# TravisWheelerLab/BATH

Hardware: AMD Instinct MI355X
Metric: DP Gcells/s + residues/s through bathsearch pipeline at 1/2/4/8 MI355X (higher is better)
Workload: dtype u8/i16 integer scores (SSV: exact binary16), f32 Forward

## Files before the change

### bath_amd/__init__.py

```python
import ctypes as C
import os
import subprocess

import numpy as np

_HERE = os.path.dirname(os.path.abspath(__file__))
_ROOT = os.path.dirname(_HERE)
LIB_PATH = os.environ.get("BATH_HIP_LIBRARY") or os.path.join(_HERE, "libbathhip.so")

OK, EINVAL, ERANGE, ENORESULT = 0, 11, 16, 19
KP, K, NEVPARAM = 29, 20, 8
LOGSUM_TABLE, LOGSUM_EXACT, LOGSUM_TABLE_SERIAL, LOGSUM_CONTEXT = 0, 1, 2, 3
LOGSUM_ODDS = 4
ENSEMBLE_SERIAL, ENSEMBLE_STREAMS_HOST, ENSEMBLE_STREAMS_DEVICE = 0, 1, 2
ENSEMBLE_MODES = {"serial": ENSEMBLE_SERIAL, "streams": ENSEMBLE_STREAMS_HOST, "device": ENSEMBLE_STREAMS_DEVICE}
ENS_SAMPLES = 200
ARITH_STRICT, ARITH_ODDS3, ARITH_ODDS = 0, 1, 2
ARITH_MODES = {"strict": ARITH_STRICT, "odds3": ARITH_ODDS3, "odds": ARITH_ODDS}
ENS_OK, ENS_IMPOSSIBLE, ENS_STEP_CAP, ENS_SEG_OVERFLOW = 0, 1, 2, 3
ENS_REGION_OK, ENS_REGION_NO_TRACES = 0, 1

DNA_SYMS = "ACGT-RYMKSWHBVDN*~"
AMINO_SYMS = "ACDEFGHIKLMNPQRSTVWY-BJZOUX*~"

# ... 28 lines not shown
class _FsProfile(C.Structure):
    _fields_ = [("M", C.c_int32), ("L", C.c_int32), ("max_length", C.c_int32), ("codon_lengths", C.c_int32),
                ("maxcodons", C.c_int32), ("nj", C.c_float), ("fsprob", C.c_float),
                ("tsc", C.POINTER(C.c_float)), ("rsc", C.POINTER(C.c_float)),
                ("codons", C.POINTER(C.c_uint8)), ("indel_pos", C.POINTER(C.c_uint8)),
                ("xsc", (C.c_float * 2) * 4), ("evparam", C.c_float * NEVPARAM), ("compo", C.c_float * K)]


class OProfileScalars(C.Structure):
    _fields_ = [("tbm_b", C.c_uint8), ("tec_b", C.c_uint8), ("tjb_b", C.c_uint8), ("base_b", C.c_uint8), ("bias_b", C.c_uint8),
                ("scale_b", C.c_float), ("xw", (C.c_int16 * 2) * 4), ("scale_w", C.c_float),
                ("base_w", C.c_int16), ("ddbound_w", C.c_int16), ("xf", (C.c_float * 2) * 4)]


class PipelineParams(C.Structure):
    _fields_ = [("F1", C.c_double), ("F2", C.c_double), ("F3", C.c_double), ("F4", C.c_double),
                ("do_biasfilter", C.c_int32), ("fs_pipe", C.c_int32), ("min_orf_len", C.c_int32), ("ncbi_table", C.c_int32),
                ("nres_before", C.c_int64),
                ("do_null2", C.c_int32), ("std_pipe", C.c_int32), ("strands", C.c_int32), ("initiator", C.c_int32),
                ("inc_by_E", C.c_int32), ("seed", C.c_int32), ("T", C.c_double)]


STRAND_BOTH, STRAND_TOPONLY, STRAND_BOTTOMONLY = 0, 1, 2
INIT_ANY, INIT_TABLE, INIT_AUG = 0, 1, 2


class OrfResult(C.Structure):
    _fields_ = [("window", C.c_int64), ("strand", C.c_int32), ("frame", C.c_int32), ("start", C.c_int32), ("end", C.c_int32),
                ("n", C.c_int32), ("stage", C.c_int32), ("msv_status", C.c_int32), ("vit_status", C.c_int32),
                ("usc", C.c_float), ("nullsc", C.c_float), ("filtersc", C.c_float), ("vfsc", C.c_float), ("fwdsc", C.c_float),
                ("P", C.c_double)]


ORF_RESULT_DTYPE = np.dtype([("window", "<i8"), ("strand", "<i4"), ("frame", "<i4"), ("start", "<i4"), ("end", "<i4"),
                             ("n", "<i4"), ("stage", "<i4"), ("msv_status", "<i4"), ("vit_status", "<i4"),
                             ("usc", "<f4"), ("nullsc", "<f4"), ("filtersc", "<f4"), ("vfsc", "<f4"), ("fwdsc", "<f4"),
                             ("P", "<f8")], align=True)


class PipelineStats(C.Structure):
    _fields_ = [(n, C.c_int64) for n in ("nres", "n_orfs", "n_past_msv", "n_past_bias", "n_past_vit", "n_past_fwd",
                                          "pos_past_msv", "pos_past_bias", "pos_past_vit", "pos_past_fwd",
                                          "cells_msv", "cells_vit", "cells_fwd")]


class Orf(C.Structure):
    _fields_ = [("window", C.c_int64), ("strand", C.c_int32), ("frame", C.c_int32), ("start", C.c_int32), ("end", C.c_int32),
                ("n", C.c_int32), ("aa_off", C.c_int64)]


class FsWindow(C.Structure):
    _fields_ = [("window", C.c_int64), ("strand", C.c_int32), ("n", C.c_int32), ("length", C.c_int32),
                ("orf_cnt", C.c_int32), ("k_min", C.c_int32), ("k_max", C.c_int32),
                ("tot_orfsc", C.c_float), ("nullsc", C.c_float), ("filtersc", C.c_float), ("fwdsc", C.c_float),
                ("P_tot", C.c_double), ("P_min", C.c_double), ("P_fs", C.c_double), ("P_null", C.c_double),
                ("branch", C.c_int32)]


class FsDomain(C.Structure):
    _fields_ = [("window", C.c_int64), ("strand", C.c_int32), ("fs_window", C.c_int32),
                ("ienv", C.c_int32), ("jenv", C.c_int32), ("iali", C.c_int32), ("jali", C.c_int32), ("ihmm", C.c_int32), ("jhmm", C.c_int32),
                ("envsc", C.c_float), ("oasc", C.c_float), ("domcorrection", C.c_float), ("dombias", C.c_float),
                ("bitscore", C.c_float), ("pre_score", C.c_float), ("lnP", C.c_double), ("reported", C.c_int32), ("n_shifted_codons", C.c_int32),
                ("n_stops", C.c_int32), ("pid", C.c_float), ("ali_columns", C.c_int32), ("cigar_off", C.c_int64)]
    cigar = ""


_DTYPES = {}


class DomainTrace(C.Structure):
    _fields_ = [("off", C.c_int64), ("N", C.c_int32), ("win_start", C.c_int32), ("orf_start", C.c_int32), ("frameshift", C.c_int32)]


class AliDisplayOpts(C.Structure):
    _fields_ = [("hmm_name", C.c_char_p), ("seq_name", C.c_char_p), ("consensus", C.c_char_p), ("rf", C.c_char_p), ("cs", C.c_char_p),
                ("M", C.c_int32), ("sqfrom", C.c_int64), ("sqto", C.c_int64), ("textw", C.c_int32), ("show_frameline", C.c_int32),
                ("initiator", C.c_int32)]


class FsRow(C.Structure):
    _fields_ = [("type", C.c_char), ("length", C.c_int32), ("ali_start", C.c_int32), ("seq_start", C.c_int64)]


class DistItem(C.Structure):
    _fields_ = [("query", C.c_int32), ("lo", C.c_int64), ("hi", C.c_int64)]


T_M, T_D, T_I = 1, 2, 3


def _np_dtype(T):
    d = _DTYPES.get(T)
    if d is None:
        d = _DTYPES[T] = np.dtype(T)
    return d


FS_DOMAIN_DTYPE = _np_dtype(FsDomain)


class KernelTime(C.Structure):
    _fields_ = [("name", C.c_char_p), ("ms", C.c_float), ("launches", C.c_int64), ("cells", C.c_double), ("bytes", C.c_double)]


class HmmWindow(C.Structure):
    _fields_ = [("target", C.c_int64), ("n", C.c_int32), ("k", C.c_int32), ("length", C.c_int32), ("score", C.c_float)]


class StdResult(C.Structure):
    _fields_ = [("fwdsc", C.c_float), ("bcksc", C.c_float), ("oasc", C.c_float), ("fwd_status", C.c_int32), ("bck_status", C.c_int32),
                ("ok", C.c_int32), ("null2", C.c_float * KP)]


class Fs5Result(C.Structure):
    _fields_ = [("fwdsc", C.c_float), ("bcksc", C.c_float), ("oasc", C.c_float), ("null2", C.c_float * KP)]


_CALIB_SCORE_FN = C.CFUNCTYPE(C.c_int, C.c_void_p, C.POINTER(C.c_uint8), C.c_int, C.c_int, C.POINTER(C.c_float))

_vp, _u8p, _f32p, _i32p, _i64p = C.c_void_p, C.POINTER(C.c_uint8), C.POINTER(C.c_float), C.POINTER(C.c_int32), C.POINTER(C.c_int64)
ABI = {
    "bath_hmmfile_count": (C.c_int, [C.c_char_p]),
    "bath_hmmfile_read": (C.c_int, [C.c_char_p, C.c_int, C.POINTER(C.POINTER(_Hmm))]),
    "bath_hmm_destroy": (None, [C.POINTER(_Hmm)]),
    "bath_gencode_basic": (C.c_int, [C.c_int, _u8p]),
    "bath_profile_config": (C.c_int, [C.POINTER(_Hmm), C.c_int, C.POINTER(C.POINTER(_Profile))]),
    "bath_profile_destroy": (None, [C.POINTER(_Profile)]),
    "bath_fs_profile_config": (C.c_int, [C.POINTER(_Hmm), _u8p, C.c_int, C.c_int, C.POINTER(C.POINTER(_FsProfile))]),
    "bath_fs_profile_destroy": (None, [C.POINTER(_FsProfile)]),
    "bath_hip_init": (C.c_int, [C.c_int, C.POINTER(_vp)]),
    "bath_hip_finalize": (None, [_vp]),
    "bath_hip_last_error": (C.c_char_p, [_vp]),
    "bath_hip_synchronize": (C.c_int, [_vp]),
    "bath_hip_stream": (_vp, [_vp]),
    "bath_hip_set_fs_strict": (C.c_int, [_vp, C.c_int]),
    "bath_hip_set_fs_serial": (C.c_int, [_vp, C.c_int]),
    "bath_hip_set_fs_odds": (C.c_int, [_vp, C.c_int]),
    "bath_hip_set_fs5_odds": (C.c_int, [_vp, C.c_int]),
    "bath_hip_set_fs_ensemble": (C.c_int, [_vp, C.c_int]),
    "bath_hip_fs_ensemble_counters": (C.c_int, [_vp, _i64p, _i64p, _i64p]),
    "bath_hip_set_std_ensemble": (C.c_int, [_vp, C.c_int]),
    "bath_hip_std_ensemble_counters": (C.c_int, [_vp, _i64p, _i64p, _i64p]),
    "bath_hip_std_region_ensembles": (C.c_int, [_vp, _vp, _vp, _i32p, C.c_uint32, _i32p, _i32p, _i32p, C.c_int64, _i64p, _i32p, _f32p, C.c_int64, _i64p]),
    "bath_selftest_std_ensemble": (C.c_int, [C.c_int, C.c_int, _f32p, _f32p, C.c_float, C.c_float, C.c_float, _u8p, C.c_int, _f32p, _f32p, C.c_uint32, _i32p, _i32p,
                                             _i32p, C.c_int, _i32p, _f32p, _i32p, C.c_int, _i32p]),
    "bath_selftest_std_ens_walk": (C.c_int, [C.c_int, _f32p, C.c_float, C.c_float, C.c_float, C.c_int, _f32p, _f32p, C.c_uint32, _i32p, _i32p, C.c_int, _i32p]),
    "bath_hip_fs5_region_ensembles": (C.c_int, [_vp, _vp, _vp, C.c_uint32, _i32p, _i32p, _i32p, C.c_int64, _i64p, _i32p, C.c_int64, _i64p]),
    "bath_selftest_fs_ensemble_seeded": (C.c_int, [C.c_int, _f32p, C.c_float, C.c_float, C.c_float, C.c_int, C.c_int, _f32p, _f32p, C.c_uint32, _i32p, C.c_int, _i32p]),
    "bath_selftest_fs_ensemble_streams": (C.c_int, [C.c_int, _f32p, C.c_float, C.c_float, C.c_float, C.c_int, C.c_int, _f32p, _f32p, C.c_uint32,
                                                    _i32p, _i32p, _i32p, C.c_int, _i32p, _i32p, C.c_int, _i32p]),
    "bath_selftest_rng_jump": (C.c_int, [C.c_uint32, C.c_uint64, C.POINTER(C.c_uint32)]),
    "bath_selftest_ens_explog": (C.c_int, [C.c_int, _f32p, _f32p, _f32p]),
    "bath_hip_trim": (C.c_int, [_vp]),
    "bath_hip_kernel_times": (C.c_int, [_vp, C.c_int, C.POINTER(KernelTime)]),
    "bath_hip_oprofile_convert": (C.c_int, [_vp, C.POINTER(_Profile), C.POINTER(_vp)]),
    "bath_hip_oprofile_destroy": (None, [_vp]),
    "bath_hip_oprofile_M": (C.c_int, [_vp]),
    "bath_hip_oprofile_scalars": (C.c_int, [_vp, C.c_int, C.POINTER(OProfileScalars)]),
    "bath_hip_oprofile_get_ssv_scores": (C.c_int, [_vp, _u8p]),
    "bath_hip_oprofile_get_vit": (C.c_int, [_vp, C.POINTER(C.c_int16), C.POINTER(C.c_int16)]),
    "bath_hip_oprofile_get_fwd": (C.c_int, [_vp, _f32p, _f32p]),
    "bath_hip_seqs_create": (C.c_int, [_vp, _u8p, _i64p, C.c_int64, C.POINTER(_vp)]),
    "bath_hip_seqs_destroy": (None, [_vp]),
    "bath_hip_seqs_count": (C.c_int64, [_vp]),
    "bath_hip_seqs_read": (C.c_int64, [_vp, _u8p, C.c_int64, _i64p, _i32p, _i32p]),
    "bath_hip_seqs_set_context": (C.c_int, [_vp, C.POINTER(C.c_int32)]),
    "bath_hip_host_alloc": (C.c_void_p, [C.c_size_t]),
    "bath_hip_host_free": (None, [C.c_void_p]),
    "bath_hip_seqs_create_packed": (C.c_int, [_vp, _i64p, C.c_int64, C.POINTER(_vp)]),
    "bath_hip_seqs_upload_packed": (C.c_int, [_vp, C.c_void_p, _i64p, _i32p, _u8p, C.c_int64]),
    "bath_hip_seqs_upload_wait": (C.c_int, [_vp]),
    "bath_hip_fasta_create": (C.c_int, [_vp, C.POINTER(_vp)]),
    "bath_hip_fasta_destroy": (None, [_vp]),
    "bath_hip_fasta_feed": (C.c_int, [_vp, C.c_void_p, C.c_int64]),
    "bath_hip_fasta_finish": (C.c_int, [_vp]),
    "bath_hip_fasta_count": (C.c_int64, [_vp]),
    "bath_hip_fasta_symbols": (C.c_int64, [_vp]),
    "bath_hip_fasta_records": (C.c_int, [_vp, C.c_int64, C.c_int64, C.c_void_p]),
    "bath_hip_fasta_error": (C.c_int, [_vp, _i64p, _i64p, _i64p, _i32p]),
    "bath_hip_fasta_windows": (C.c_int64, [_vp, C.c_int64, C.c_int64, C.c_int32, C.c_int32, C.c_void_p, C.c_int64]),
    "bath_hip_fasta_seqs": (C.c_int, [_vp, C.c_void_p, C.c_int64, C.POINTER(_vp)]),
    "bath_hip_fasta_seqs_for": (C.c_int, [_vp, _vp, C.c_void_p, C.c_int64, C.POINTER(_vp)]),
    "bath_hip_fasta_codes": (C.c_int, [_vp, C.c_int64, C.c_int64, C.c_int64, _u8p]),
    "bath_hip_fasta_release": (C.c_int, [_vp, C.c_int64]),
    "bath_hip_ssvfilter": (C.c_int, [_vp, _vp, _vp, _f32p, _i32p]),
    "bath_hip_msvfilter": (C.c_int, [_vp, _vp, _vp, _f32p, _i32p]),
    "bath_hip_vitfilter": (C.c_int, [_vp, _vp, _vp, _f32p, _i32p]),
    "bath_hip_forward_parser": (C.c_int, [_vp, _vp, _vp, _f32p, _i32p]),
    "bath_hip_bias_filter": (C.c_int, [_vp, _vp, _vp, _f32p, _f32p]),
    "bath_hip_fwdback_parser": (C.c_int, [_vp, _vp, _vp, _i64p, _f32p, _f32p, _i32p, _i32p, _f32p, _f32p]),
    "bath_hip_translate_orfs": (C.c_int, [_vp, _vp, C.c_int, C.c_int, C.POINTER(C.POINTER(Orf)), _i64p, C.POINTER(_u8p)]),
    "bath_hip_translate_orfs_opts": (C.c_int, [_vp, _vp, C.c_int, C.c_int, C.c_int, C.c_int, C.POINTER(C.POINTER(Orf)), _i64p, C.POINTER(_u8p)]),
    "bath_hip_orf_worklist": (C.c_int, [_vp, C.c_void_p, _i64p]),
    "bath_gencode_initiators": (C.c_int, [C.c_int, C.c_int, _u8p]),
    "bath_tophits_set_score_thresholds": (None, [_vp, C.c_int, C.c_double, C.c_int, C.c_double]),
    "bath_search_space_residues": (C.c_int64, [C.c_int, C.c_double, C.c_int, C.c_int64]),
    "bath_pipeline_params_default": (None, [C.POINTER(PipelineParams), C.c_int]),
    "bath_hip_pipeline_filters": (C.c_int, [_vp, _vp, _vp, C.POINTER(PipelineParams), C.POINTER(PipelineStats),
                                            C.POINTER(C.POINTER(OrfResult)), _i64p]),
    "bath_hip_pipeline_frameshift": (C.c_int, [_vp, _vp, _vp, _vp, C.POINTER(PipelineParams), C.POINTER(PipelineStats),
                                              C.POINTER(C.POINTER(OrfResult)), _i64p, C.POINTER(C.POINTER(FsWindow)), _i64p]),
    "bath_hip_oprofile_set_consensus": (C.c_int, [_vp, C.c_char_p]),
    "bath_hip_domain_cigars": (C.c_void_p, [_vp]),
    "bath_hip_domain_traces": (C.c_int, [_vp, C.POINTER(C.POINTER(DomainTrace)), _i64p, C.POINTER(C.POINTER(C.c_int8)), C.POINTER(_i32p),
                                         C.POINTER(_i32p), C.POINTER(C.POINTER(C.c_int8)), C.POINTER(_f32p)]),
    "bath_alidisplay_print": (C.c_int64, [C.POINTER(DomainTrace), C.POINTER(C.c_int8), _i32p, _i32p, C.POINTER(C.c_int8), _f32p,
                                          _u8p, C.c_int32, C.POINTER(_FsProfile), C.POINTER(_Profile), _u8p, C.POINTER(AliDisplayOpts),
                                          C.c_char_p, C.c_int64]),
    "bath_selftest_rng_stream": (C.c_int, [C.c_uint32, C.c_int, C.POINTER(C.c_double)]),
    "bath_selftest_fchoose": (C.c_int, [C.c_uint32, _f32p, C.c_int, C.c_int, _i32p]),
    "bath_hits_serialize": (C.c_int64, [C.c_void_p, C.c_int64, C.c_char_p, C.POINTER(DomainTrace), C.POINTER(C.c_int8), _i32p, _i32p, C.POINTER(C.c_int8), _f32p,
                                        C.c_void_p, C.c_int64]),
    "bath_hits_deserialize": (C.c_int, [C.c_void_p, C.c_int64, C.POINTER(_vp)]),
    "bath_hits_stream_size": (C.c_int64, [C.c_void_p, C.c_int64]),
    "bath_hits_destroy": (None, [_vp]),
    "bath_hits_count": (C.c_int64, [_vp]),
    "bath_hits_domains": (C.POINTER(FsDomain), [_vp]),
    "bath_hits_cigars": (C.c_void_p, [_vp, _i64p]),
    "bath_hits_traces": (C.c_int, [_vp, C.POINTER(C.POINTER(DomainTrace)), C.POINTER(C.POINTER(C.c_int8)), C.POINTER(_i32p), C.POINTER(_i32p),
                                   C.POINTER(C.POINTER(C.c_int8)), C.POINTER(_f32p)]),
    "bath_tophits_add_serialized": (C.c_int, [_vp, C.c_void_p, C.c_int64, C.c_int64, C.c_int64, C.c_int64, C.POINTER(C.c_char_p), C.POINTER(C.c_char_p),
                                              C.POINTER(C.c_char_p), C.POINTER(C.c_int64)]),
    "bath_dist_shard_range": (None, [C.c_int64, C.c_int, C.c_int, _i64p, _i64p]),
    "bath_dist_items": (C.c_int64, [_i64p, C.POINTER(C.c_double), C.c_int, C.c_int, C.c_int, C.POINTER(DistItem), C.c_int64]),
    "bath_dist_deal": (C.c_int, [C.POINTER(C.c_double), C.c_int64, C.c_int, _i32p]),
    "bath_selftest_cluster_segments": (C.c_int, [C.c_int, _i32p, _i32p, _i32p, _i32p, _i32p, C.c_int, C.c_int, _i32p, C.c_int, _i32p]),
    "bath_selftest_fs_ensemble": (C.c_int, [C.c_int, _f32p, C.c_float, C.c_float, C.c_float, C.c_int, C.c_int, _f32p, _f32p, _i32p, C.c_int, _i32p]),
    "bath_tophits_create": (_vp, []),
    "bath_tophits_destroy": (None, [_vp]),
    "bath_tophits_add": (C.c_int, [_vp, C.POINTER(FsDomain), C.c_int64, C.c_void_p, C.c_int64, C.POINTER(C.c_char_p), C.POINTER(C.c_char_p),
                                   C.POINTER(C.c_char_p), C.POINTER(C.c_int64)]),
    "bath_tophits_finalize": (C.c_int, [_vp, C.c_int64, C.c_int, C.c_double]),
    "bath_tophits_count": (C.c_int64, [_vp]),
    "bath_tophits_reported": (C.c_int64, [_vp]),
    "bath_tophits_get": (C.c_int, [_vp, C.c_int64, C.POINTER(FsDomain), C.POINTER(C.c_int64), C.POINTER(C.c_int32)]),
    "bath_tophits_targets": (C.c_int64, [_vp, C.c_int, C.c_int, C.c_char_p, C.c_int64]),
    "bath_tophits_domain_annotation": (C.c_int64, [_vp, C.c_int64, C.c_int, C.c_int, C.c_char_p, C.c_int64]),
    "bath_tophits_pipeline_statistics": (C.c_int64, [_vp, C.POINTER(PipelineStats), C.POINTER(PipelineParams), C.c_int64, C.c_int64, C.c_int64, C.c_char_p, C.c_int64]),
    "bath_tophits_set_inclusion": (None, [_vp, C.c_double]),
    "bath_tophits_tabular_targets": (C.c_int64, [_vp, C.c_char_p, C.c_char_p, C.c_int, C.c_int, C.c_int, C.c_int, C.c_char_p, C.c_int64]),
    "bath_trace_frameshift_rows": (C.c_int64, [C.POINTER(DomainTrace), C.POINTER(C.c_int8), _i32p, _i32p, C.POINTER(C.c_int8), _u8p, C.c_int32,
                                               C.POINTER(_FsProfile), C.c_int64, C.c_int64, C.POINTER(FsRow), C.c_int64]),
    "bath_tophits_tabular_frameshifts": (C.c_int64, [_vp, C.c_char_p, C.c_char_p, C.POINTER(FsRow), _i64p, C.c_int64, C.c_int, C.c_char_p, C.c_int64]),
    "bath_hip_pipeline_hits": (C.c_int, [_vp, _vp, _vp, C.POINTER(PipelineParams), C.c_double, C.POINTER(PipelineStats),
                                         C.POINTER(C.POINTER(FsDomain)), C.POINTER(C.c_int64), C.POINTER(C.c_int64)]),
    "bath_hip_pipeline_frameshift_domains": (C.c_int, [_vp, _vp, _vp, _vp, _vp, C.POINTER(PipelineParams), C.c_double, C.POINTER(PipelineStats),
                                                      C.POINTER(C.POINTER(FsWindow)), _i64p, C.POINTER(C.POINTER(FsDomain)), _i64p, _i64p]),
    "bath_hip_pipeline_timings": (C.c_int, [_vp, C.c_int, C.POINTER(C.c_char_p), _f32p, _i64p]),
    "bath_hip_fsprofile_convert": (C.c_int, [_vp, C.POINTER(_FsProfile), C.POINTER(_vp)]),
    "bath_hip_fsprofile_destroy": (None, [_vp]),
    "bath_hip_fs3_forward_parser": (C.c_int, [_vp, _vp, _vp, C.c_int, _f32p, _f32p, _i64p]),
    "bath_hip_fs3_backward_parser": (C.c_int, [_vp, _vp, _vp, C.c_int, _f32p, _f32p, _i64p]),
    "bath_hip_vitfilter_bath": (C.c_int, [_vp, _vp, _vp, _f32p, C.c_double, _f32p, _i32p, C.POINTER(C.POINTER(HmmWindow)), _i64p]),
    "bath_hip_ssvfilter_bath": (C.c_int, [_vp, _vp, _vp, C.c_double, C.POINTER(C.POINTER(HmmWindow)), _i64p]),
    "bath_hip_forward_full": (C.c_int, [_vp, _vp, _vp, _i32p, C.c_int, _f32p, _i32p, _f32p, _f32p]),
    "bath_hip_std_envelopes": (C.c_int, [_vp, _vp, _vp, C.POINTER(StdResult), _f32p, _f32p, _f32p, _f32p]),
    "bath_hip_std_envelopes_fill": (C.c_int, [_vp, _vp, _vp, C.POINTER(StdResult), _f32p, _f32p, _f32p, _f32p, C.c_int]),
    "bath_hip_fs5_envelopes_x": (C.c_int, [_vp, _vp, _vp, C.c_int, C.c_int, C.POINTER(Fs5Result), _f32p, _f32p, _f32p, _f32p]),
    "bath_hip_fs5_forward_full": (C.c_int, [_vp, _vp, _vp, C.c_int, _f32p, _f32p, _f32p]),
    "bath_hip_fs5_envelopes": (C.c_int, [_vp, _vp, _vp, C.c_int, C.c_int, C.POINTER(Fs5Result), _f32p, _i64p, _f32p, _i64p]),
    "bath_hip_fs5_forward_parser": (C.c_int, [_vp, _vp, _vp, C.c_int, _f32p]),
    "bath_hip_fs5_forward_parser_odds": (C.c_int, [_vp, _vp, _vp, C.c_int, _f32p]),
    "bath_calib_fit_scores": (C.c_int, [C.POINTER(C.c_uint32), _f32p, C.c_int, C.c_int, C.c_int, _CALIB_SCORE_FN, C.c_void_p, C.c_float,
                                        C.POINTER(C.c_double), C.POINTER(C.c_int)]),
    "bath_hip_calibrate_fs_arith": (C.c_int, [_vp, C.POINTER(_Hmm), C.c_int, C.POINTER(C.c_uint32), C.c_int, C.c_int, C.c_double,
                                              C.POINTER(C.c_double), C.POINTER(C.c_double), C.POINTER(C.c_double), C.POINTER(C.c_double),
                                              C.c_int, C.POINTER(C.c_int)]),
    "bath_calib_sample": (C.c_int, [C.POINTER(C.c_uint32), _f32p, C.c_int, C.c_int, C.c_int, _u8p]),
    "bath_gumbel_fit_complete": (C.c_int, [C.POINTER(C.c_double), C.c_int, C.POINTER(C.c_double), C.POINTER(C.c_double)]),
    "bath_gumbel_invcdf": (C.c_double, [C.c_double, C.c_double, C.c_double]),
    "bath_calib_tau": (C.c_int, [C.POINTER(C.c_double), C.c_int, C.c_double, C.c_double, C.POINTER(C.c_double)]),
    "bath_bg_fs_nullone": (C.c_float, [C.c_int]),
    "bath_hmm_max_length": (C.c_int, [C.POINTER(_Hmm), C.c_double]),
    "bath_hip_calibrate_fs": (C.c_int, [_vp, C.POINTER(_Hmm), C.c_int, C.POINTER(C.c_uint32), C.c_int, C.c_int, C.c_double,
                                        C.POINTER(C.c_double), C.POINTER(C.c_double), C.POINTER(C.c_double), C.POINTER(C.c_double)]),
    "bath_scorematrix_builtin": (C.c_char_p, [C.c_char_p]),
    "bath_scoresystem_create": (C.c_int, [C.c_char_p, C.c_char_p, C.c_double, C.c_double, C.POINTER(_vp), C.c_char_p, C.c_int]),
    "bath_scoresystem_destroy": (None, [_vp]),
    "bath_scoresystem_lambda": (C.c_double, [_vp]),
    "bath_scoresystem_conditionals": (C.c_int, [_vp, C.POINTER(C.c_double)]),
    "bath_hmm_from_sequence": (C.c_int, [_vp, _u8p, C.c_int, C.c_char_p, C.c_int, C.POINTER(C.POINTER(_Hmm))]),
    "bath_hmm_mean_match_relent": (C.c_double, [C.POINTER(_Hmm)]),
    "bath_hmm_lambda": (C.c_double, [C.POINTER(_Hmm)]),
    "bath_hmm_write_ascii": (C.c_int64, [C.POINTER(_Hmm), C.c_int, C.c_double, C.c_char_p, C.c_char_p, C.c_char_p, C.c_char_p, C.c_int64]),
    "bath_calib_sample_amino": (C.c_int, [C.POINTER(C.c_uint32), _f32p, C.c_int, C.c_int, _u8p]),
    "bath_gumbel_fit_complete_loc": (C.c_int, [C.POINTER(C.c_double), C.c_int, C.c_double, C.POINTER(C.c_double)]),
    "bath_hip_calib_samples_create": (C.c_int, [_vp, C.POINTER(C.c_uint32), C.c_int, C.c_int, C.c_int, C.c_int, C.c_int, C.c_int, C.POINTER(_vp)]),
    "bath_hip_calib_samples_destroy": (None, [_vp]),
    "bath_hip_calibrate": (C.c_int, [_vp, C.POINTER(_Hmm), C.c_int, C.POINTER(C.c_uint32), _vp, C.c_int, C.c_int, C.c_int, C.c_int, C.c_int, C.c_int,
                                     C.c_double, C.c_int, C.POINTER(C.c_double), C.POINTER(C.c_int)]),
}

_lib = None


def lib():
    global _lib
    if _lib is None:
        if not os.path.exists(LIB_PATH):
            raise BathError("libbathhip.so not built: run `python -c 'import __graft_entry__ as g; g.build()'` "
                            "(or `make -C bath_amd/csrc`). There is no CPU fallback.")
        L = C.CDLL(LIB_PATH)
        for name, (res, args) in ABI.items():
            fn = getattr(L, name)
            fn.restype, fn.argtypes = res, args
# ... 1359 lines not shown
```

### bath_amd/csrc/bath_common.hpp

```cpp
#pragma once
#include <set>
#include <atomic>
#include <hip/hip_runtime.h>

#include <cstdint>
#include <chrono>
#include <cstdio>
#include <cstdlib>
#include <cstring>
#include <condition_variable>
#include <functional>
#include <mutex>
#include <string>
#include <thread>
#include <vector>

#include "bath_hip.h"
#include "bath_tilings.hpp"

namespace bath {

inline hipError_t allow_max_lds(const void *fn) {
  static std::mutex mu;
  static std::set<std::pair<int, const void *>> done;
// ... 151 lines not shown
    if (hipMemcpyAsync(dst, stage[slot].p, n * sizeof(T), hipMemcpyHostToDevice, s) != hipSuccess) { set_error("staging upload failed"); return BATH_EFAIL; }
    return BATH_OK;
  }
  bath::HostBuf pinned[4];
  bath::HostBuf results_pinned;
  bath_orf_result *d_records = nullptr;
  int64_t n_records = 0;
  std::vector<bath_orf> orfs;
  std::vector<bath_fs_window> fs_windows;
  bool keep_fwd_rows = false;
  const float *fwd_rows_kept = nullptr;
  const int64_t *fwd_rows_off = nullptr;
  bool fs_want_regions = false;
  std::vector<int64_t> fs_keep_xoff;
  std::vector<int32_t> fs_regions_all;
  std::vector<bath_fs_domain> fs_domains;
  std::string cigars;
  struct TraceRec { int64_t col_off; int32_t ncol, k1, i_first, win_start, orf_start, frameshift, d_i; };
  std::vector<TraceRec> tr_recs;
  std::vector<uint16_t> tr_codes;
  std::vector<float> tr_pp;
  void traces_clear() { tr_recs.clear(); tr_codes.clear(); tr_pp.clear(); tr_valid = false; }
  void trace_push(const uint16_t *codes, const float *pp, int ncol, int k1, int i_first, int win_start, int orf_start, int frameshift, int d_i) {
    tr_recs.push_back(TraceRec{(int64_t)tr_codes.size(), ncol, k1, i_first, win_start, orf_start, frameshift, d_i});
    tr_codes.insert(tr_codes.end(), codes, codes + ncol);
    if (pp) tr_pp.insert(tr_pp.end(), pp, pp + ncol); else tr_pp.insert(tr_pp.end(), (size_t)ncol, 0.0f);
    tr_valid = false;
  }
  bool tr_valid = false;
  std::vector<bath_domain_trace> tr_out;
  std::vector<int8_t> tr_st, tr_c;
  std::vector<int32_t> tr_k, tr_i;
  std::vector<bath::PipelineSurvivor> fs_std_orfs;
  const uint8_t *fs_std_pool = nullptr;
  std::vector<uint8_t> orf_aa;
  std::vector<bath_orf_work> orf_work;
  std::vector<bath_hmm_window> hmm_windows;
  std::vector<bath::StageTiming> timings;
  std::vector<hipEvent_t> ev_pool;
  std::vector<bath::KernelSpan> spans;
  std::vector<hipEvent_t> span_events;
  size_t span_events_used = 0;
  void spans_reset() { spans.clear(); span_events_used = 0; }
  int span_begin(const char *name, hipStream_t s, double cells, double bytes) {
    auto get = [&]() -> hipEvent_t {
      if (span_events_used == span_events.size()) { hipEvent_t e; if (hipEventCreate(&e) != hipSuccess) return nullptr; span_events.push_back(e); }
      return span_events[span_events_used++];
    };
    bath::KernelSpan k{name, get(), get(), cells, bytes};
    if (!k.a || !k.b) return -1;
    (void)hipEventRecord(k.a, s);
    spans.push_back(k);
    return (int)spans.size() - 1;
  }
  void span_end(int idx, hipStream_t s) { if (idx >= 0) (void)hipEventRecord(spans[(size_t)idx].b, s); }
  std::vector<bath_hip_ctx *> lanes;
  bath::LanePool *lane_pool = nullptr;
  hipEvent_t ev_lanes = nullptr;
  bath_hip_ctx *aux = nullptr;
  bath_hip_ctx *aux2 = nullptr;
  bath_hip_ctx *aux3 = nullptr;
  bool internal = false;
};

namespace bath {
inline void mark_internal(bath_hip_ctx *c) { if (c && !c->internal) { c->internal = true; g_ctx_internal.fetch_add(1); } }
}

struct SeqView {
  const uint8_t *data;
  const int64_t *off;
  const int32_t *len;
  int64_t n;
  const int32_t *context;
};

struct bath_hip_seqs {
  bath_hip_ctx *ctx = nullptr;
  int64_t n = 0;
  int64_t total = 0;
  int64_t total_aligned = 0;
  mutable int64_t cache_minlen = -1, cache_nres = 0, cache_max_orfs = 0;
  mutable int64_t ntiles = -1;
  mutable void *d_tile_desc = nullptr;
  mutable int32_t *d_tile_first = nullptr;
  bool is_part = false;
  int64_t first_window = 0;
  mutable std::vector<bath_hip_seqs *> parts;
  int32_t maxlen = 0;
  uint8_t *d_data = nullptr;
  int64_t *d_off = nullptr;
  int32_t *d_len = nullptr;
  int32_t *d_context = nullptr;
  uint8_t *d_packed = nullptr;
  int64_t *d_poff = nullptr;
  int64_t packed_bytes = 0;
  void *d_exc = nullptr;
  int64_t exc_cap = 0, n_exc = 0;
  hipEvent_t ev_upload = nullptr;
  bool upload_pending = false;
  std::vector<int64_t> h_off;
  std::vector<int32_t> h_len;
  std::vector<int32_t> h_context;
  SeqView view() const { return SeqView{d_data, d_off, d_len, n, d_context}; }
};

struct LenTables {
  int32_t maxL = -1;
  uint8_t *d_tjb = nullptr;
  int16_t *d_xwmove = nullptr;
  float   *d_pmove = nullptr;
  float   *d_nullsc = nullptr;
  float   *d_lt1 = nullptr;
  float   *d_lt2 = nullptr;
  float   *d_p1 = nullptr;
  std::vector<uint8_t> h_tjb;
  std::vector<int16_t> h_xwmove;
  std::vector<float> h_pmove, h_nullsc;
};

struct bath_hip_oprofile {
  bath_hip_ctx *ctx = nullptr;
  uint64_t uid = 0;
  int M = 0, max_length = 0, L0 = 0;
  float nj = 1.f;
  float evparam[BATH_NEVPARAM];
  float compo[BATH_K_AMINO];
  std::vector<uint8_t> rb;
  std::vector<int16_t> rw;
  std::vector<int16_t> tw;
  std::vector<float> rf, tf;
  uint8_t tbm_b = 0, tec_b = 0, base_b = 0, bias_b = 0;
  float scale_b = 0;
  int16_t xw_E[2] = {0, 0};
  float scale_w = 0;
  int16_t base_w = 0, ddbound_w = 0;
  float xf_E[2] = {0, 0};
  std::string consensus;
  std::vector<uint8_t> cons_digital;
  uint8_t *d_cons = nullptr;
  std::vector<float> prefix_lengths, suffix_lengths;
  int NR = 0, G = 1;
  int ssv_row_bytes = 0;
  int16_t *d_ssv = nullptr;
  int16_t *d_msv = nullptr;
  uint8_t *d_rb = nullptr;
  int rb_stride = 0;
  int16_t *d_rw = nullptr;
  int16_t *d_tw = nullptr;
  float *d_rf = nullptr, *d_tf = nullptr;
  float *d_rfb = nullptr, *d_tfb = nullptr;
  float *d_msc = nullptr, *d_tsc = nullptr;
  float *d_bias_eo = nullptr;
  int vit_NR = 0, vit_rw_pitch = 0;
  int16_t *d_vit_rw = nullptr; uint32_t *d_vit_tw2 = nullptr; int16_t *d_vit_rank = nullptr;
  mutable LenTables lt;
  mutable std::mutex grow_mu;
  mutable std::vector<void *> retired;
  mutable int16_t *d_emit = nullptr;
  mutable double emit_F1 = -1.0;
  mutable int emit_maxlen = -1;
  int ensure_len_tables(int maxL) const;
};

namespace bath {
int build_len_tables(const bath_hip_oprofile *om, int maxL);
void bias_filter_eo(const float *compo, float eo[kKp][2]);
double gumbel_surv(double x, double mu, double lambda);
double gumbel_invsurv(double p, double mu, double lambda);
double exp_surv(double x, double mu, double lambda);
struct StageClock {
  bool on; std::chrono::steady_clock::time_point t;
  StageClock() { const char *e = std::getenv("BATH_HIP_TIMING"); on = e && e[0] == '1'; t = std::chrono::steady_clock::now(); }
  void lap(const char *what) {
    if (!on) return;
    const auto n = std::chrono::steady_clock::now();
    std::fprintf(stderr, "[bath timing] %-34s %8.2f ms\n", what, std::chrono::duration<double, std::milli>(n - t).count());
    t = n;
  }
};

}
```

### bath_amd/csrc/bath_pipeline.hip

```cpp
#include <algorithm>
#include <cmath>
#include <cstring>
#include <cstdlib>
#include <map>
#include <thread>

#include "bath_common.hpp"
#include "bath_kernels.hpp"
#include "bath_launch.hpp"
#include "host_model.hpp"

using namespace bath;

namespace bath {

static const double kLog2 = 0.69314718055994529;

enum { FLAG_VIT_RUN = 1, FLAG_HAS_WIN = 2 };

struct Counters {
  int cand_count, todo_msv, todo_vit, todo_ssvb, todo_vit2, todo_fwd, win_count, overflow;
  int todo_lb, pad_;
  unsigned long long n_orfs, orf_res;
  unsigned long long n_past_msv, n_past_bias, n_past_vit, n_past_fwd;
  unsigned long long pos_past_msv, pos_past_bias, pos_past_vit, pos_past_fwd;
  unsigned long long res_vit, res_fwd;
  unsigned long long res_seen;
};

struct Params {
  double F1, F2, F3, F4;
  int do_bias, fs_pipe, minlen;
  float evparam[BATH_NEVPARAM];
};

template <int NR, int G>
__global__ __launch_bounds__(256, NR <= 76 ? 4 : 1) void ssv_orf_kernel(const uint8_t *__restrict__ aa, const OrfRec *__restrict__ orfs, const int *__restrict__ n_orfs_dev,
                                                      SeqView dna, const int16_t *__restrict__ cost_tab, int row_bytes,
                                                      const int16_t *__restrict__ emit_thresh, int thresh_max,
                                                      Cand cand, int cand_cap, Counters *__restrict__ ctr, int chunk) {
  extern __shared__ __attribute__((aligned(16))) char lds[];
  if (chunk > 0 && (int64_t)blockIdx.x * (blockDim.x >> 6) * chunk * (64 / G) >= (int64_t)*n_orfs_dev) return;
  {
    const int n32 = kSsvRows * row_bytes / 4;
    const uint32_t *src = reinterpret_cast<const uint32_t *>(cost_tab);
    uint32_t *dst = reinterpret_cast<uint32_t *>(lds);
    for (int i = threadIdx.x; i < n32; i += blockDim.x) dst[i] = src[i];
  }
  __syncthreads();
  constexpr int TPW = 64 / G;
  const int64_t n_orfs = *n_orfs_dev;
  const int lane = threadIdx.x & 63;
  const int grank = SsvGroups<G>::rank(lane);
  const char *tile = lds + grank * (4 * NR);
  const unsigned tile_addr = (unsigned)(size_t)(__attribute__((address_space(3))) const char *)tile;
  const int64_t wave0 = ((int64_t)blockIdx.x * blockDim.x + threadIdx.x) >> 6;
  const int64_t nwaves = ((int64_t)gridDim.x * blockDim.x) >> 6;
  const s16x2 fl = {0, 0};
  const int64_t tb_first = chunk > 0 ? wave0 * chunk * TPW : wave0 * TPW, tb_step = chunk > 0 ? TPW : nwaves * TPW;
  const int64_t tb_end = chunk > 0 ? (tb_first + (int64_t)chunk * TPW < n_orfs ? tb_first + (int64_t)chunk * TPW : n_orfs) : n_orfs;
  for (int64_t tb = tb_first; tb < tb_end; tb += tb_step) {
    const int64_t t = tb + SsvGroups<G>::slot(lane);
    const bool live = t < n_orfs;
    OrfRec rec{0, 0, 0};
    if (live) rec = orfs[t];
    const int L = rec.len_sf & 0x0fffffff;
#ifdef BATH_SSV_POOL_PROBE
    const uint8_t *s = aa + ((size_t)(tb / TPW) * 8192) % ((size_t)1 << 27) + (size_t)lane * 8;
#define BATH_SSV_RES(i8) (s + (size_t)(i8) * 64)
#else
    const uint8_t *s = aa + rec.aa_off;
#define BATH_SSV_RES(i8) (s + (i8))
#endif
    const int Lw = wave_max_i32(L);
    s16x2 reg[NR];
#pragma unroll
    for (int r = 0; r < NR; r++) reg[r] = fl;
    s16x2 xE = fl, xE2 = fl;
    uint64_t qnext = (0 < L) ? *reinterpret_cast<const uint64_t *>(BATH_SSV_RES(0)) : 0x1d1d1d1d1d1d1d1dull;
    for (int i0 = 0; i0 < Lw; i0 += 8) {
      const uint64_t q = qnext;
      qnext = (i0 + 8 < L) ? *reinterpret_cast<const uint64_t *>(BATH_SSV_RES(i0 + 8)) : 0x1d1d1d1d1d1d1d1dull;
      const int nrow = min(8, Lw - i0);
      for (int h = 0; h < 2; h++) {
        const uint32_t qh = h ? (uint32_t)(q >> 32) : (uint32_t)q;
        const int nh = min(4, nrow - 4 * h);
        for (int j = 0; j < nh; j++) {
          int x = (int)__builtin_amdgcn_ubfe(qh, 8 * j, 8);
          x = (i0 + 4 * h + j < L) ? x : kRowReset;
          const unsigned carry = ssv_carry<NR, G>(reg, grank);
          ssv_row_pipe<NR, 3>(reg, xE, xE2, tile_addr + __umul24((unsigned)x, (unsigned)row_bytes), carry);
        }
      }
    }
    xE = ssv_max3(xE, xE2, xE2);
    const int v = ssv_group_max<G>(xE);
    if (dna.context) {
      unsigned long long r = 0;
      if (live && grank == 0) {
        const int sf = (int)((unsigned)rec.len_sf >> 28);
        const int64_t w = rec.w;
        const int startj = (int32_t)(rec.aa_off - (2 * dna.off[w] + 96 * w + (int64_t)sf * orf_stream_pitch(dna.len[w])));
        const int C = dna.context[w], start_s = sf % 3 + 3 * startj + 1;
        if (sf < 3 ? (start_s + 3 * L - 1 < C) : (dna.len[w] - start_s + 1 < C)) r = (unsigned long long)L;
      }
      if (__ballot(r != 0)) { for (int d = 32; d >= 1; d >>= 1) r += __shfl_xor(r, d, 64); if (lane == 0) atomicAdd(&ctr->res_seen, r); }
    }
    if (live && grank == 0 && v >= (int)emit_thresh[min(L, thresh_max)]) {
      const int sf = (int)((unsigned)rec.len_sf >> 28);
      const int64_t w = rec.w;
      const int64_t stream = 2 * dna.off[w] + 96 * w + (int64_t)sf * orf_stream_pitch(dna.len[w]);
      const int startj = (int32_t)(rec.aa_off - stream);
      bool seen = false;
      if (dna.context) {
        const int C = dna.context[w], start_s = sf % 3 + 3 * startj + 1;
        seen = sf < 3 ? (start_s + 3 * L - 1 < C) : (dna.len[w] - start_s + 1 < C);
      }
      const int slot = seen ? cand_cap + 1 : atomicAdd(&ctr->cand_count, 1);
      if (seen) {
      } else if (slot < cand_cap) {
        cand.window[slot] = w; cand.sf[slot] = sf; cand.startj[slot] = startj; cand.len[slot] = L;
        cand.v[slot] = (int16_t)min(v, 32767); cand.off[slot] = rec.aa_off;
      } else atomicOr(&ctr->overflow, 1);
    }
  }
}

__device__ __forceinline__ double d_gumbel_surv(double x, double mu, double lambda) {
  const double ey = -exp(-lambda * (x - mu));
  if (fabs(ey) < 5e-9) return -ey;
  return 1.0 - exp(ey);
}
__device__ __forceinline__ double d_exp_surv(double x, double mu, double lambda) { return (x < mu) ? 1.0 : exp(-lambda * (x - mu)); }

__device__ __forceinline__ int cand_classify(const Cand &cand, int c, int tjb, const MsvConsts &mc) {
  float sc = 0.f;
  const int st = ssv_classify(cand.v[c], tjb, mc, &sc);
  cand.usc[c] = sc; cand.msv_status[c] = st; cand.stage[c] = 0; cand.flags[c] = 0;
  cand.vfsc[c] = -INFINITY; cand.fwdsc[c] = -INFINITY; cand.vit_status[c] = 0; cand.filtersc[c] = 0.f; cand.P[c] = 1.0;
  cand.kminmax[2 * c] = 1 << 30; cand.kminmax[2 * c + 1] = 0;
  return st;
}

__global__ void classify_kernel(Cand cand, int cand_cap, Counters *__restrict__ ctr, const uint8_t *__restrict__ tjb_tab, MsvConsts mc,
                                int32_t *__restrict__ todo_msv) {
  const int ncand = min(ctr->cand_count, cand_cap);
  for (int c = blockIdx.x * blockDim.x + threadIdx.x; c < ncand; c += gridDim.x * blockDim.x) {
    if (cand_classify(cand, c, tjb_tab[cand.len[c]], mc) == BATH_ENORESULT) todo_msv[atomicAdd(&ctr->todo_msv, 1)] = c;
  }
}

struct F1Tables { const float *eo, *nullsc, *p1, *lt1, *lt2; };
__device__ __forceinline__ void cand_f1_bias(const Cand &cand, int c, Counters *__restrict__ ctr, const Params &p, const uint8_t *__restrict__ pool, int M,
                                             const float *s_eo , const F1Tables &t,
                                             int32_t *__restrict__ todo_vit, int32_t *__restrict__ todo_ssvb) {
  const int L = cand.len[c];
  const float usc = cand.usc[c];
  const float nullsc = t.nullsc[L];
  cand.nullsc[c] = nullsc;
  float seqsc = (float)((double)(usc - nullsc) / kLog2);
  double P = d_gumbel_surv(seqsc, p.evparam[0], p.evparam[1]);
  cand.P[c] = P;
  if (P > p.F1) return;
  atomicAdd(&ctr->n_past_msv, 1ull); atomicAdd(&ctr->pos_past_msv, (unsigned long long)L * 3ull);
  cand.stage[c] = 1;
  float filtersc = nullsc;
  if (p.do_bias) {
    filtersc = bias_forward(pool + cand.off[c], L, M, s_eo, t.p1[L]);
    filtersc = (filtersc + t.lt1[L]) + t.lt2[L];
    seqsc = (float)((double)(usc - filtersc) / kLog2);
    P = d_gumbel_surv(seqsc, p.evparam[0], p.evparam[1]);
    cand.P[c] = P; cand.filtersc[c] = filtersc;
    if (P > p.F1) return;
  }
  cand.filtersc[c] = filtersc;
  atomicAdd(&ctr->n_past_bias, 1ull); atomicAdd(&ctr->pos_past_bias, (unsigned long long)L * 3ull);
  cand.stage[c] = 2;
  if (P > p.F2) { cand.flags[c] |= FLAG_VIT_RUN; todo_vit[atomicAdd(&ctr->todo_vit, 1)] = c; atomicAdd(&ctr->res_vit, (unsigned long long)L); }
  else todo_ssvb[atomicAdd(&ctr->todo_ssvb, 1)] = c;
}

__global__ void f1_bias_kernel(Cand cand, int cand_cap, Counters *__restrict__ ctr, Params p, const uint8_t *__restrict__ pool, int M, F1Tables t,
                               int32_t *__restrict__ todo_vit, int32_t *__restrict__ todo_ssvb) {
  __shared__ float s_eo[kKp * 2];
  for (int i = threadIdx.x; i < kKp * 2; i += blockDim.x) s_eo[i] = t.eo[i];
  __syncthreads();
  const int ncand = min(ctr->cand_count, cand_cap);
  for (int c = blockIdx.x * blockDim.x + threadIdx.x; c < ncand; c += gridDim.x * blockDim.x) cand_f1_bias(cand, c, ctr, p, pool, M, s_eo, t, todo_vit, todo_ssvb);
}

template <int NR>
__global__ __launch_bounds__(256, 4) void msv_stage_kernel(Cand cand, int cand_cap, Counters *__restrict__ ctr,
                                                           const int16_t *__restrict__ cost_tab , int row_bytes,
                                                           const uint8_t *__restrict__ tjb_tab, MsvConsts mc, Params p, const uint8_t *__restrict__ pool, int M,
                                                           F1Tables t, int32_t *__restrict__ todo_vit, int32_t *__restrict__ todo_ssvb) {
  extern __shared__ __attribute__((aligned(16))) char lds[];
  __shared__ float s_eo[kKp * 2];
  const int ncand = min(ctr->cand_count, cand_cap);
  if ((int64_t)blockIdx.x * blockDim.x >= ncand) return;
  {
    const int n32 = kSsvRows * row_bytes / 4;
    const uint32_t *src = reinterpret_cast<const uint32_t *>(cost_tab);
    uint32_t *dst = reinterpret_cast<uint32_t *>(lds);
    for (int i = threadIdx.x; i < n32; i += blockDim.x) dst[i] = src[i];
    for (int i = threadIdx.x; i < kKp * 2; i += blockDim.x) s_eo[i] = t.eo[i];
  }
  __syncthreads();
  const int64_t job = (int64_t)blockIdx.x * blockDim.x + threadIdx.x;
  const bool live = job < ncand;
  const int c = live ? (int)job : 0;
  const int L = live ? cand.len[c] : 0;
  const int tjb = tjb_tab[L];
  const bool rescore = live && cand_classify(cand, c, tjb, mc) == BATH_ENORESULT;
  const int Lr = rescore ? L : 0;
  const uint8_t *s = pool + (rescore ? cand.off[c] : 0);
  bool overflow = false;
  const int xJ = msv_lane_rows<NR>(lds, row_bytes, s, Lr, wave_max_i32(Lr), (uint8_t)((int8_t)tjb + (int8_t)mc.tbm), mc, &overflow);
  if (rescore) {
    if (overflow) { cand.usc[c] = INFINITY; cand.msv_status[c] = BATH_ERANGE; }
    else { cand.usc[c] = msv_lane_score(xJ, tjb, mc); cand.msv_status[c] = BATH_OK; }
  }
  if (live) cand_f1_bias(cand, c, ctr, p, pool, M, s_eo, t, todo_vit, todo_ssvb);
}

template <int C>
__global__ __launch_bounds__(256) void ssv_bath_kernel(Cand cand, const Counters *__restrict__ ctr, const int32_t *__restrict__ todo,
                                                       const uint8_t *__restrict__ pool, int M, const uint8_t *__restrict__ rb, int rb_stride,
                                                       const uint8_t *__restrict__ ssv_scores, const uint8_t *__restrict__ tjb_tab,
                                                       const float *__restrict__ nullsc_tab, MsvConsts mc, double invP_f1,
                                                       WindowRec *__restrict__ wins, int win_cap, Counters *__restrict__ ctrw) {
  const int lane = threadIdx.x & 63;
  const int64_t wid = ((int64_t)blockIdx.x * blockDim.x + threadIdx.x) >> 6;
  const int64_t nw = ((int64_t)gridDim.x * blockDim.x) >> 6;
  const int ntodo = ctr->todo_ssvb;
  const int Q = max(2, ((M - 1) / 16) + 1);
  for (int64_t job = wid; job < ntodo; job += nw) {
    const int c = todo[job];
    const int L = cand.len[c];
    const uint8_t *s = pool + cand.off[c];
    const int tjb = tjb_tab[L];
    const float nullsc = nullsc_tab[L];
    const int sc_thresh = (uint8_t)(int)ceil((((double)nullsc + ((double)(float)invP_f1 * kLog2) + 3.0) * (double)mc.scale_b) + mc.base + mc.tec + tjb);
    const int tjbm = (uint8_t)((int8_t)tjb + (int8_t)mc.tbm);
    const int xB = satu8(mc.base - tjbm);
    int kmin = 1 << 30, kmax = 0;
    int dp[C];
#pragma unroll
    for (int k = 0; k < C; k++) dp[k] = 0;
    const int ph = threadIdx.x & 63;
    int rbuf = (ph < L) ? (int)s[ph] : 0, rnext = 0;
    for (int i = 1; i <= L; i++) {
      const int j = (i - 1) & 63;
      if (j == 0) { const int q = i - 1 + 64 + ph; rnext = (q < L) ? (int)s[q] : 0; }
      const int x = min(__builtin_amdgcn_readlane(rbuf, j), kKp - 1);
      if (j == 63) rbuf = rnext;
      const uint8_t *row = rb + (size_t)x * rb_stride;
      int prev = wave_shr1_i32(dp[C - 1], 0);
      int xE = 0;
#pragma unroll
      for (int k = 0; k < C; k++) {
        const int node = lane * C + k + 1;
        const int cost = (node <= M) ? (int)row[node] : 255;
        int sv = max(prev, xB);
        sv = satu8(sv + mc.bias);
        sv = satu8(sv - cost);
        prev = dp[k];
        dp[k] = sv;
        xE = max(xE, sv);
      }
      xE = wave_max_i32(xE);
      if (xE >= sc_thresh) {
        int rank = 1 << 30;
#pragma unroll
        for (int k = 0; k < C; k++) {
          const int node = lane * C + k + 1;
          if (node <= M && dp[k] == xE) rank = min(rank, ((node - 1) % Q) * 16 + (node - 1) / Q);
        }
        rank = wave_min_i32(rank);
        int end = (rank / 16) + Q * (rank % 16) + 1;
        int rem_sc = xE;
#pragma unroll
        for (int k = 0; k < C; k++) dp[k] = 0;
        int start = end, target_end = i, target_start = i;
        int sc = rem_sc;
        while (rem_sc > mc.base - tjb - mc.tbm && start >= 1 && target_start >= 1) {
          rem_sc -= mc.bias - (int)ssv_scores[(size_t)start * kKp + min((int)s[target_start - 1], kKp - 1)];
          --start; --target_start;
        }
        start++; target_start++;
        int k = end + 1, n = target_end + 1, max_end = target_end, max_sc = sc, since = 0;
        while (k < M && n <= L) {
          sc += mc.bias - (int)ssv_scores[(size_t)k * kKp + min((int)s[n - 1], kKp - 1)];
          if (sc >= max_sc) { max_sc = sc; max_end = n; since = 0; }
          else { since++; if (since == 5) break; }
          k++; n++;
        }
        end += (max_end - target_end);
        target_end = max_end;
        float ret = ((float)(max_sc - tjb) - (float)mc.base);
        ret /= mc.scale_b;
        ret = (float)((double)ret - 3.0);
        if (lane == 0) {
          const int slot = atomicAdd(&ctrw->win_count, 1);
          if (slot < win_cap) wins[slot] = WindowRec{c, target_start, end, end - start + 1, ret};
        }
        kmin = min(kmin, start); kmax = max(kmax, end);
        i = target_end;
        { const int base = i & ~63; rbuf = (base + ph < L) ? (int)s[base + ph] : 0; rnext = (base + 64 + ph < L) ? (int)s[base + 64 + ph] : 0; }
      }
    }
    if (lane == 0) { cand.kminmax[2 * c] = kmin; cand.kminmax[2 * c + 1] = kmax; }
  }
}

__device__ __forceinline__ float local_compo_x(const uint8_t *ssv_scores, int M, int base_b, float scale_b, const float *bgf, int k_start, int k_end, int x) {
  const int k_len = k_end - k_start + 1;
  if (k_len < 20) { k_start -= (20 - k_len) / 2; k_end += (20 - k_len) / 2; }
  k_start = max(1, k_start); k_end = min(M, k_end);
  float acc = 0.0f;
  for (int k = k_start; k <= k_end; k++) {
    const float lo = ((float)base_b - (float)ssv_scores[(size_t)k * kKp + x]) / scale_b;
    acc += bgf[x] * expf(lo);
  }
  return acc;
}
__device__ void local_compo_finish(float *compo , const float *bgf, float *eo );
__device__ void local_compo_eo(const uint8_t *ssv_scores, int M, int base_b, float scale_b, const float *bgf, int k_start, int k_end, float *eo ) {
  float compo[20];
  for (int x = 0; x < 20; x++) compo[x] = local_compo_x(ssv_scores, M, base_b, scale_b, bgf, k_start, k_end, x);
  local_compo_finish(compo, bgf, eo);
}
__device__ void local_compo_finish(float *compo, const float *bgf, float *eo) {
  float sum = 0.f, cc = 0.f;
  for (int x = 0; x < 20; x++) { const float y = compo[x] - cc; const float t = sum + y; cc = (t - sum) - y; sum = t; }
  if (sum != 0.0f) for (int x = 0; x < 20; x++) compo[x] /= sum;
  else for (int x = 0; x < 20; x++) compo[x] = 1.0f / 20.0f;
  for (int x = 0; x < 20; x++) { eo[2 * x] = bgf[x] / bgf[x]; eo[2 * x + 1] = compo[x] / bgf[x]; }
  eo[2 * 20] = eo[2 * 20 + 1] = 1.0f; eo[2 * 27] = eo[2 * 27 + 1] = 1.0f; eo[2 * 28] = eo[2 * 28 + 1] = 1.0f;
  const int mem[6][2] = {{2, 11}, {7, 9}, {3, 13}, {8, 8}, {1, 1}, {-1, -1}};
  for (int dx = 0; dx < 6; dx++) {
    float n0 = 0.f, n1 = 0.f, den = 0.f;
    if (dx == 5) { for (int y = 0; y < 20; y++) { n0 += bgf[y]; n1 += compo[y]; den += bgf[y]; } }
    else {
      const int a = min(mem[dx][0], mem[dx][1]), b = max(mem[dx][0], mem[dx][1]);
      n0 += bgf[a]; n1 += compo[a]; den += bgf[a];
      if (b != a) { n0 += bgf[b]; n1 += compo[b]; den += bgf[b]; }
    }
    eo[2 * (21 + dx)] = den > 0.f ? n0 / den : 0.f;
    eo[2 * (21 + dx) + 1] = den > 0.f ? n1 / den : 0.f;
  }
}

__global__ void post_vit_kernel(Cand cand, int cand_cap, Counters *__restrict__ ctr, Params p, int32_t *__restrict__ todo_lb, int32_t *__restrict__ todo_fwd) {
  const int ncand = min(ctr->cand_count, cand_cap);
  for (int c = blockIdx.x * blockDim.x + threadIdx.x; c < ncand; c += gridDim.x * blockDim.x) {
    if (cand.stage[c] != 2) continue;
    const int L = cand.len[c];
    if (cand.flags[c] & FLAG_VIT_RUN) {
      const float seqsc = (float)((double)(cand.vfsc[c] - cand.filtersc[c]) / kLog2);
      const double P = d_gumbel_surv(seqsc, p.evparam[2], p.evparam[3]);
      cand.P[c] = P;
      if (P > p.F2) { cand.kminmax[2 * c] = 1 << 30; cand.kminmax[2 * c + 1] = 0; continue; }
    }
    atomicAdd(&ctr->n_past_vit, 1ull); atomicAdd(&ctr->pos_past_vit, (unsigned long long)L * 3ull);
    if (p.do_bias && cand.kminmax[2 * c] <= cand.kminmax[2 * c + 1]) {
      cand.flags[c] |= FLAG_HAS_WIN;
      todo_lb[atomicAdd(&ctr->todo_lb, 1)] = c;
      continue;
    }
    cand.stage[c] = 3;
    todo_fwd[atomicAdd(&ctr->todo_fwd, 1)] = c; atomicAdd(&ctr->res_fwd, (unsigned long long)L);
  }
}

__global__ void compo_terms_kernel(const float *__restrict__ bgf, int base_b, float scale_b, float *__restrict__ terms ) {
  const int x = blockIdx.x, sc = threadIdx.x;
  const float lo = ((float)base_b - (float)sc) / scale_b;
  terms[x * 256 + sc] = bgf[x] * expf(lo);
}

__global__ __launch_bounds__(64) void local_compo_kernel(Cand cand, const Counters *__restrict__ ctr, int M, const uint8_t *__restrict__ ssv_scores,
                                                         const float *__restrict__ terms, const int32_t *__restrict__ todo_lb, float *__restrict__ compo_out ) {
  const int lane = threadIdx.x, g = lane / 20, x = lane % 20;
  const int ntodo = ctr->todo_lb;
  for (int base = blockIdx.x * 3; base < ntodo; base += gridDim.x * 3) {
    const int job = base + g;
    if (g >= 3 || job >= ntodo) continue;
    const int c = todo_lb[job];
    int k_start = cand.kminmax[2 * c], k_end = cand.kminmax[2 * c + 1];
    const int k_len = k_end - k_start + 1;
    if (k_len < 20) { k_start -= (20 - k_len) / 2; k_end += (20 - k_len) / 2; }
    k_start = max(1, k_start); k_end = min(M, k_end);
    const float *tx = terms + x * 256;
    float acc = 0.0f;
    for (int k = k_start; k <= k_end; k++) acc += tx[ssv_scores[(size_t)k * kKp + x]];
    compo_out[(size_t)job * 20 + x] = acc;
  }
}

__global__ __launch_bounds__(64) void post_vit_local_kernel(Cand cand, Counters *__restrict__ ctr, Params p, const uint8_t *__restrict__ pool, int M,
                                                            const float *__restrict__ bgf, const float *__restrict__ compo_in,
                                                            const float *__restrict__ p1_tab, const float *__restrict__ lt1_tab, const float *__restrict__ lt2_tab,
                                                            const int32_t *__restrict__ todo_lb, int32_t *__restrict__ todo_vit2, int32_t *__restrict__ todo_fwd) {
  __shared__ float s_eo[64][kKp * 2 + 1];
  const int ntodo = ctr->todo_lb;
  for (int job = blockIdx.x * blockDim.x + threadIdx.x; job < ntodo; job += gridDim.x * blockDim.x) {
    const int c = todo_lb[job];
    const int L = cand.len[c];
    const float usc = cand.usc[c];
    float filtersc = cand.filtersc[c];
    const float vfsc = (cand.flags[c] & FLAG_VIT_RUN) ? cand.vfsc[c] : -INFINITY;
    float compo[20];
    for (int y = 0; y < 20; y++) compo[y] = compo_in[(size_t)job * 20 + y];
    float *eo = s_eo[threadIdx.x];
    local_compo_finish(compo, bgf, eo);
    float lf = bias_forward(pool + cand.off[c], L, M, eo, p1_tab[L]);
    lf = (lf + lt1_tab[L]) + lt2_tab[L];
    bool to_fwd = true;
    if (lf > filtersc) {
      filtersc = lf;
      cand.filtersc[c] = filtersc;
      if (vfsc == -INFINITY) {
        const float seqsc = (float)((double)(usc - filtersc) / kLog2);
        const double P = d_gumbel_surv(seqsc, p.evparam[0], p.evparam[1]);
        cand.P[c] = P;
        if (P > p.F2) { cand.stage[c] = 5; todo_vit2[atomicAdd(&ctr->todo_vit2, 1)] = c; atomicAdd(&ctr->res_vit, (unsigned long long)L); to_fwd = false; }
      } else {
        const float seqsc = (float)((double)(vfsc - filtersc) / kLog2);
        const double P = d_gumbel_surv(seqsc, p.evparam[2], p.evparam[3]);
        cand.P[c] = P;
        if (P > p.F2) to_fwd = false;
      }
    }
    if (to_fwd) { cand.stage[c] = 3; todo_fwd[atomicAdd(&ctr->todo_fwd, 1)] = c; atomicAdd(&ctr->res_fwd, (unsigned long long)L); }
  }
}

__global__ void post_vit2_kernel(Cand cand, Counters *__restrict__ ctr, Params p, const int32_t *__restrict__ todo_vit2, int32_t *__restrict__ todo_fwd) {
  const int ntodo = ctr->todo_vit2;
  for (int job = blockIdx.x * blockDim.x + threadIdx.x; job < ntodo; job += gridDim.x * blockDim.x) {
    const int c = todo_vit2[job];
    const float seqsc = (float)((double)(cand.vfsc[c] - cand.filtersc[c]) / kLog2);
    const double P = d_gumbel_surv(seqsc, p.evparam[2], p.evparam[3]);
    cand.P[c] = P;
    if (P > p.F2) { cand.stage[c] = 2; continue; }
    cand.stage[c] = 3;
    todo_fwd[atomicAdd(&ctr->todo_fwd, 1)] = c; atomicAdd(&ctr->res_fwd, (unsigned long long)cand.len[c]);
  }
}

__global__ void final_kernel(Cand cand, Counters *__restrict__ ctr, Params p, const int32_t *__restrict__ todo_fwd) {
  const int ntodo = ctr->todo_fwd;
  for (int job = blockIdx.x * blockDim.x + threadIdx.x; job < ntodo; job += gridDim.x * blockDim.x) {
    const int c = todo_fwd[job];
    const float seqsc = (float)((double)(cand.fwdsc[c] - cand.filtersc[c]) / kLog2);
    const double P = d_exp_surv(seqsc, p.evparam[4], p.evparam[5]);
    cand.P[c] = P;
    if (P > (p.fs_pipe ? p.F4 : p.F3)) continue;
    cand.stage[c] = 4;
    atomicAdd(&ctr->n_past_fwd, 1ull);
    if (!p.fs_pipe) atomicAdd(&ctr->pos_past_fwd, (unsigned long long)cand.len[c] * 3ull);
  }
}

__global__ void copy_count_kernel(const int *src, int64_t *dst) { *dst = *src; }

}


namespace bath {

static int ssv_classify_host(int v, int tjb, const MsvConsts &c, float *sc) {
  if (tjb + c.tbm + c.tec + c.bias >= 127) return BATH_ENORESULT;
  unsigned xE = (v >= -1 - c.bias) ? 255u : (unsigned)(v + 256);
  if ((int)xE >= 255 - c.bias) { *sc = INFINITY; return (c.base - tjb - c.tbm < 128) ? BATH_ENORESULT : BATH_ERANGE; }
  xE = (xE + (unsigned)(c.base - tjb - c.tbm) - 128u) & 0xffffu;
  if ((int)xE >= 255 - c.bias) { *sc = INFINITY; return BATH_ERANGE; }
  unsigned xJ = (xE - (unsigned)c.tec) & 0xffffu;
  if ((int)xJ > c.base) return BATH_ENORESULT;
  float r = ((float)((int)xJ - tjb) - (float)c.base);
  r /= c.scale_b;
  r = (float)((double)r - 3.0);
  *sc = r;
  return BATH_OK;
}

static void build_emit_table(const bath_hip_oprofile *om, double F1, int maxlen, std::vector<int16_t> &tab) {
  const MsvConsts mc = msv_consts(om);
  tab.assign((size_t)maxlen + 1, (int16_t)32767);
  for (int len = 0; len <= maxlen; len++) {
    const int tjb = om->lt.h_tjb[len];
    const float nullsc = om->lt.h_nullsc[len];
    auto keep = [&](int v) {
      float usc = 0.f;
      if (ssv_classify_host(v, tjb, mc, &usc) != BATH_OK) return true;
      const float seqsc = (float)((double)(usc - nullsc) / kLog2);
      return !(gumbel_surv(seqsc, om->evparam[0], om->evparam[1]) > F1);
    };
    if (!keep(127)) continue;
    int lo = -128, hi = 127;
    while (lo < hi) { const int mid = lo + (hi - lo) / 2; if (keep(mid)) hi = mid; else lo = mid + 1; }
    tab[(size_t)len] = (int16_t)lo;
  }
}

static int ensure_emit_table(bath_hip_ctx *ctx, const bath_hip_oprofile *om, double F1, int maxlen) {
  std::lock_guard<std::mutex> lock(om->grow_mu);
  if (om->emit_F1 == F1 && om->emit_maxlen >= maxlen && om->d_emit) return BATH_OK;
  std::vector<int16_t> tab;
  build_emit_table(om, F1, maxlen, tab);
  if (om->d_emit) om->retired.push_back(om->d_emit);
  om->d_emit = nullptr;
  BATH_HIP_TRY(ctx, hipMalloc((void **)&om->d_emit, tab.size() * sizeof(int16_t) + 64));
  BATH_HIP_TRY(ctx, hipMemcpy(om->d_emit, tab.data(), tab.size() * sizeof(int16_t), hipMemcpyHostToDevice));
  om->emit_F1 = F1; om->emit_maxlen = maxlen;
  return BATH_OK;
}

static int wave_grid_blocks(bath_hip_ctx *ctx) { return ctx->prop.multiProcessorCount * 8; }

struct PipelineWork {
  Cand cand;
  int cand_cap = 0;
  uint8_t *pool = nullptr;
  int32_t *todo_msv = nullptr, *todo_vit = nullptr, *todo_ssvb = nullptr, *todo_vit2 = nullptr, *todo_fwd = nullptr, *todo_sorted = nullptr;
  int *len_bins = nullptr;
  WindowRec *wins = nullptr;
  int win_cap = 0;
  Counters *ctr = nullptr;
};

template <class T>
static T *carve(char *&p, size_t n) {
  T *r = reinterpret_cast<T *>(p);
  p += (n * sizeof(T) + 255) / 256 * 256;
  return r;
}

static size_t layout(PipelineWork &w, char *base, int cap, int win_cap) {
  char *p = base;
  const size_t n = (size_t)cap;
  w.cand_cap = cap; w.win_cap = std::max(2 * cap, win_cap);
  if (win_cap == 0) {
    static const int forced = [] { const char *e = std::getenv("BATH_HIP_TEST_WINCAP"); return e ? std::atoi(e) : 0; }();
    if (forced > 0) w.win_cap = forced;
  }
  w.ctr = carve<Counters>(p, 1);
  w.cand.window = carve<int64_t>(p, n); w.cand.off = carve<int64_t>(p, n); w.cand.P = carve<double>(p, n);
  w.cand.sf = carve<int32_t>(p, n); w.cand.startj = carve<int32_t>(p, n); w.cand.len = carve<int32_t>(p, n);
  w.cand.msv_status = carve<int32_t>(p, n); w.cand.vit_status = carve<int32_t>(p, n); w.cand.fwd_status = carve<int32_t>(p, n); w.cand.stage = carve<int32_t>(p, n);
  w.cand.flags = carve<int32_t>(p, n); w.cand.kminmax = carve<int32_t>(p, 2 * n);
  w.cand.usc = carve<float>(p, n); w.cand.nullsc = carve<float>(p, n); w.cand.filtersc = carve<float>(p, n);
  w.cand.vfsc = carve<float>(p, n); w.cand.fwdsc = carve<float>(p, n);
  w.cand.v = carve<int16_t>(p, n);
  w.todo_msv = carve<int32_t>(p, n); w.todo_vit = carve<int32_t>(p, n); w.todo_ssvb = carve<int32_t>(p, n);
  w.todo_vit2 = carve<int32_t>(p, n); w.todo_fwd = carve<int32_t>(p, n); w.todo_sorted = carve<int32_t>(p, n);
  w.len_bins = carve<int>(p, 2048);
  w.wins = carve<WindowRec>(p, (size_t)w.win_cap);
  return (size_t)(p - base);
}

}

extern "C" void bath_pipeline_params_default(bath_pipeline_params *p, int fs_pipe) {
  p->F1 = 0.02; p->F2 = 1e-3; p->F3 = 1e-5; p->F4 = 5e-4;
  p->do_biasfilter = 1; p->fs_pipe = fs_pipe; p->min_orf_len = 20; p->ncbi_table = 1;
  p->nres_before = 0;
  p->do_null2 = 1; p->std_pipe = 1; p->strands = BATH_STRAND_BOTH; p->initiator = BATH_INIT_ANY;
  p->inc_by_E = 1; p->seed = 42; p->T = 0.0;
}

extern "C" int bath_hip_pipeline_timings(const bath_hip_ctx *ctx, int max, const char **names, float *ms, int64_t *launches) {
  int n = std::min<int>(max, (int)ctx->timings.size());
  for (int i = 0; i < n; i++) { names[i] = ctx->timings[i].name; ms[i] = ctx->timings[i].ms; launches[i] = ctx->timings[i].launches; }
  return n;
}

namespace bath {
struct FilterState {
  PipelineWork W;
  Counters hc{};
  const uint8_t *d_ssvsc = nullptr;
  const float *d_bgf = nullptr;
  OrfTablesDev tt{};
};
}

__global__ __launch_bounds__(64) void fwd_keep_offsets_kernel(const int32_t *__restrict__ todo, const int *__restrict__ ntodo_dev, const int32_t *__restrict__ len,
                                                              int64_t *__restrict__ off, int64_t cap) {
  const int lane = threadIdx.x, n = *ntodo_dev;
  int64_t base = 0;
  for (int j0 = 0; j0 < n; j0 += 64) {
    const int j = j0 + lane;
    const int sid = j < n ? todo[j] : -1;
    const int64_t v = sid >= 0 ? ((int64_t)len[sid] + 1) * 6 : 0;
    int64_t incl = v;
    for (int d = 1; d < 64; d <<= 1) { const int64_t u = __shfl_up(incl, d, 64); if (lane >= d) incl += u; }
    if (sid >= 0) off[sid] = (base + incl <= cap) ? base + incl - v : (int64_t)-1;
    base += __shfl(incl, 63, 64);
  }
}

static int cascade_model_ok(bath_hip_ctx *ctx, const bath_hip_oprofile *om) {
  if (om->M <= kCascadeMaxNodes) return BATH_OK;
  ctx->set_error("the filter cascade supports models up to " + std::to_string(kCascadeMaxNodes) + " nodes (this one has " + std::to_string(om->M) + ")");
  return BATH_EINVAL;
}

static int launch_ssv_bath(bath_hip_ctx *ctx, hipStream_t stream, const bath_hip_oprofile *om, const Cand &cand, Counters *ctr, const int32_t *todo, const uint8_t *pool,
                           const uint8_t *ssv_scores, const MsvConsts &mc, double invP, WindowRec *wins, int win_cap);

static int run_filters(bath_hip_ctx *ctx, const bath_hip_oprofile *om, const bath_hip_seqs *dna,
                       const bath_pipeline_params *prm, bath_pipeline_stats *stats,
                       const bath_orf_result **results, int64_t *n_results, FilterState *state) {
  if (!ctx || !om || !dna || !prm) return BATH_EINVAL;
  if (cascade_model_ok(ctx, om) != BATH_OK) return BATH_EINVAL;
  BATH_HIP_TRY(ctx, hipSetDevice(ctx->device));
  if (n_results) *n_results = 0;
  if (results) *results = nullptr;
  if (stats) std::memset(stats, 0, sizeof *stats);
  const int64_t nwin = dna->n;
  if (nwin == 0) return BATH_OK;
  const int M = om->M;
  const int max_orf = dna->maxlen / 3 + 1;
  int st = om->ensure_len_tables(max_orf);
  if (st != BATH_OK) return st;

  OrfTablesDev tt{};
  if (prm->strands < 0 || prm->strands > 2 || prm->initiator < 0 || prm->initiator > 2) { ctx->set_error("bath_pipeline_params: strands / initiator out of range"); return BATH_EINVAL; }
  if ((st = orf_tables_upload(ctx, prm->ncbi_table, &tt, prm->initiator)) != BATH_OK) return st;
  if ((st = ensure_emit_table(ctx, om, prm->F1, max_orf)) != BATH_OK) return st;
  DevBuf &b_tabs = ctx->scratch[8], &b_work = ctx->scratch[9];
  const size_t ssv_bytes = (size_t)(M + 1) * kKp;
  const size_t tabs_bytes = 8192 + ssv_bytes + 256 + 20 * 4 + 256;
  if (tabs_bytes > b_tabs.cap) ctx->tabs_uid = 0;
  BATH_HIP_TRY(ctx, b_tabs.reserve(tabs_bytes));
  char *tp = b_tabs.as<char>();
  const int16_t *d_emit = om->d_emit;
  uint8_t *d_ssvsc = reinterpret_cast<uint8_t *>(tp); tp += (ssv_bytes + 255) / 256 * 256;
  float *d_bgf = reinterpret_cast<float *>(tp);
  if (ctx->tabs_uid != om->uid || ctx->tabs_ptr != b_tabs.p) {
    std::vector<uint8_t> ssv_scores(ssv_bytes, 0);
    bath_hip_oprofile_get_ssv_scores(om, ssv_scores.data());
    BATH_HIP_TRY(ctx, hipMemcpyAsync(d_ssvsc, ssv_scores.data(), ssv_scores.size(), hipMemcpyHostToDevice, ctx->stream));
    BATH_HIP_TRY(ctx, hipMemcpyAsync(d_bgf, kAminoBg, 20 * sizeof(float), hipMemcpyHostToDevice, ctx->stream));
    BATH_HIP_TRY(ctx, hipStreamSynchronize(ctx->stream));
    ctx->tabs_uid = om->uid; ctx->tabs_ptr = b_tabs.p;
  }

  Params P{};
  P.F1 = prm->F1; P.F2 = prm->F2; P.F3 = prm->F3; P.F4 = prm->F4;
  P.do_bias = prm->do_biasfilter; P.fs_pipe = prm->fs_pipe; P.minlen = prm->min_orf_len;
  std::memcpy(P.evparam, om->evparam, sizeof P.evparam);
  const MsvConsts mc = msv_consts(om);
  const double invP_f1 = gumbel_invsurv(prm->F1, om->evparam[0], om->evparam[1]);
  VitWindowArgs wa{};
  wa.invP_vit = (double)(float)gumbel_invsurv(prm->F2, om->evparam[2], om->evparam[3]);
  wa.invP_msv = (double)(float)gumbel_invsurv(prm->F2, om->evparam[0], om->evparam[1]);

  if (dna->cache_minlen != prm->min_orf_len) {
    int64_t nres_c = 0, max_orfs_c = 0;
    for (int64_t i = 0; i < nwin; i++) {
      const int n = dna->h_len[i];
      if (n < 15) continue;
      nres_c += 2 * (int64_t)(n - (dna->h_context.empty() ? 0 : dna->h_context[(size_t)i]));
      max_orfs_c += 6 * (int64_t)((n / 3 + 1) / (prm->min_orf_len + 1) + 1);
    }
    dna->cache_minlen = prm->min_orf_len; dna->cache_nres = nres_c; dna->cache_max_orfs = max_orfs_c;
  }
  const int64_t nres = prm->strands == BATH_STRAND_BOTH ? dna->cache_nres : dna->cache_nres / 2;
  const int64_t max_orfs = dna->cache_max_orfs;
  if (max_orfs >= (int64_t)INT32_MAX) { ctx->set_error("DNA block too large for one pipeline call (ORF list indices are 32-bit): split it"); return BATH_EINVAL; }
  int64_t cap = std::max<int64_t>(4096, (int64_t)((double)max_orfs * std::min(1.0, prm->F1 * 4.0 + 0.01)));
  cap = std::min<int64_t>(cap, std::max<int64_t>(max_orfs, 4096));
  {
    static const int forced = [] { const char *e = std::getenv("BATH_HIP_TEST_CANDCAP"); return e ? std::atoi(e) : 0; }();
    if (forced > 0) cap = forced;
  }

  if ((st = orf_tiles_ensure(ctx, dna)) != BATH_OK) return st;
  const size_t nent = (size_t)dna->ntiles * 6;
  DevBuf &b_aa = ctx->scratch[24], &b_slots = ctx->scratch[25], &b_orfs = ctx->scratch[26], &b_misc = ctx->scratch[27];
  BATH_HIP_TRY(ctx, b_aa.reserve(orf_aa_bytes(dna)));
  BATH_HIP_TRY(ctx, b_slots.reserve(((size_t)dna->ntiles * (size_t)orf_slot_cap(prm->min_orf_len) + 64) * 8));
  BATH_HIP_TRY(ctx, b_orfs.reserve((size_t)(max_orfs + 64) * sizeof(OrfRec)));
  BATH_HIP_TRY(ctx, b_misc.reserve((5 * nent + kOrfMiscInts) * sizeof(int32_t)));
  OrfBuffers ob{};
  orf_buffers_carve(&ob, b_aa.p, b_slots.p, b_orfs.p, b_misc.p, nent);

  const int NRk = om->NR;
  const size_t ssv_shmem = (size_t)kSsvRows * om->ssv_row_bytes;
  if ((st = ssv_table_fits(ctx, om)) != BATH_OK) return st;
  const int dec_blocks = ctx->prop.multiProcessorCount * 4;

  std::vector<hipEvent_t> &ev = ctx->ev_pool;
  while (ev.size() < 12) { hipEvent_t e; BATH_HIP_TRY(ctx, hipEventCreate(&e)); ev.push_back(e); }

  PipelineWork W;
  Counters hc{};
  int win_need = 0;
  for (int attempt = 0;; attempt++) {
    size_t need = layout(W, nullptr, (int)cap, win_need);
    BATH_HIP_TRY(ctx, b_work.reserve(need + 4096));
    layout(W, b_work.as<char>(), (int)cap, win_need);
    W.pool = b_aa.as<uint8_t>();
    BATH_HIP_TRY(ctx, hipMemsetAsync(W.ctr, 0, sizeof(Counters), ctx->stream));
    SeqView cv{W.pool, W.cand.off, W.cand.len, cap};

    int e = 0;
    BATH_HIP_TRY(ctx, hipEventRecord(ev[e++], ctx->stream));
    if ((st = launch_orf_scan(ctx, dna, tt, prm->min_orf_len, ob, &W.ctr->n_orfs, &W.ctr->orf_res, prm->strands)) != BATH_OK) return st;
    BATH_HIP_TRY(ctx, hipEventRecord(ev[e++], ctx->stream));
    {
      static const int ssv_chunk = [] { const char *e = std::getenv("BATH_HIP_SSV_CHUNK"); return e ? std::atoi(e) : 0; }();
      int blocks = ctx->prop.multiProcessorCount * 4;
      const int ssv_threads = 256;
      const int wpb = ssv_threads / 64;
      if (ssv_chunk > 0) blocks = (int)std::min<int64_t>((max_orfs + (int64_t)wpb * (64 / om->G) * ssv_chunk - 1) / ((int64_t)wpb * (64 / om->G) * ssv_chunk), 1 << 30);
      bool launched = false;
#define BATH_ORF_CASE(N, GG)                                                                                                     \
  if (!launched && NRk == N && om->G == GG) {                                                                                    \
    if (ssv_shmem > 64 * 1024) (void)bath::allow_max_lds((const void *)ssv_orf_kernel<N, GG>); \
    hipLaunchKernelGGL((ssv_orf_kernel<N, GG>), dim3(blocks), dim3(ssv_threads), ssv_shmem, ctx->stream, W.pool, ob.sorted, ob.ntotal,                  \
                       dna->view(), om->d_ssv, om->ssv_row_bytes, d_emit, max_orf, W.cand, W.cand_cap, W.ctr, ssv_chunk);        \
    launched = true;                                                                                                             \
  }
      BATH_SSV_SHAPES(BATH_ORF_CASE)
#undef BATH_ORF_CASE
      if (!launched) { ctx->set_error("SSV kernel: no tile shape for this model length"); return BATH_EINVAL; }
      BATH_HIP_TRY(ctx, hipGetLastError());
    }
    BATH_HIP_TRY(ctx, hipEventRecord(ev[e++], ctx->stream));
    hipStream_t bulk_stream = ctx->stream;
    struct StreamRestore { bath_hip_ctx *c; hipStream_t s; ~StreamRestore() { c->stream = s; } } stream_restore{ctx, bulk_stream};
    if (ctx->tail_stream) {
      BATH_HIP_TRY(ctx, hipStreamWaitEvent(ctx->tail_stream, ev[e - 1], 0));
      ctx->stream = ctx->tail_stream;
    }
    const bool few_cands = dna->total < lane_min_nt(), few_msv = dna->total < 2 * lane_min_nt();
    const F1Tables f1t{om->d_bias_eo, om->lt.d_nullsc, om->lt.d_p1, om->lt.d_lt1, om->lt.d_lt2};
    const bool msv_stage = !few_msv && msv_stage_supported(om);
    if (msv_stage) {
      bool launched = false;
#define BATH_MSV_STAGE_CASE(N, ...)                                                                                                         \
  if (!launched && NRk == N) {                                                                                                              \
    hipLaunchKernelGGL((msv_stage_kernel<N>), dim3((unsigned)((W.cand_cap + 255) / 256)), dim3(256), ssv_shmem, ctx->stream, W.cand, W.cand_cap, W.ctr, om->d_msv, \
                       om->ssv_row_bytes, om->lt.d_tjb, mc, P, W.pool, M, f1t, W.todo_vit, W.todo_ssvb);                                      \
    launched = true;                                                                                                                        \
  }
      BATH_MSV_LANE_NR(BATH_MSV_STAGE_CASE)
#undef BATH_MSV_STAGE_CASE
      if (!launched) { ctx->set_error("MSV stage kernel: no tile shape for this model length"); return BATH_EINVAL; }
      BATH_HIP_TRY(ctx, hipGetLastError());
      BATH_HIP_TRY(ctx, hipEventRecord(ev[e++], ctx->stream));
      BATH_HIP_TRY(ctx, hipEventRecord(ev[e++], ctx->stream));
    } else {
      hipLaunchKernelGGL(classify_kernel, dim3(dec_blocks), dim3(256), 0, ctx->stream, W.cand, W.cand_cap, W.ctr, om->lt.d_tjb, mc, W.todo_msv);
      BATH_HIP_TRY(ctx, hipGetLastError());
      if ((st = launch_msv_wave(ctx, om, cv, W.todo_msv, cap, W.cand.usc, W.cand.msv_status, &W.ctr->todo_msv, !few_msv)) != BATH_OK) return st;
      BATH_HIP_TRY(ctx, hipEventRecord(ev[e++], ctx->stream));
      hipLaunchKernelGGL(f1_bias_kernel, dim3(dec_blocks), dim3(256), 0, ctx->stream, W.cand, W.cand_cap, W.ctr, P, W.pool, M, f1t, W.todo_vit, W.todo_ssvb);
      BATH_HIP_TRY(ctx, hipGetLastError());
      BATH_HIP_TRY(ctx, hipEventRecord(ev[e++], ctx->stream));
    }
    wa.d_filtersc = W.cand.filtersc; wa.d_ssv_scores = d_ssvsc; wa.d_wins = W.wins; wa.d_win_count = &W.ctr->win_count; wa.win_cap = W.win_cap;
    wa.d_kminmax = W.cand.kminmax;
    auto launch_ssvb = [&](hipStream_t stream) -> int {
      return launch_ssv_bath(ctx, stream, om, W.cand, W.ctr, W.todo_ssvb, W.pool, d_ssvsc, mc, invP_f1, W.wins, W.win_cap);
    };
    bool ssvb_done = false;
    if (vit_lane_supported(om) && !few_cands) {
      if ((st = launch_vit_sorted(ctx, om, cv, W.todo_vit, cap, &W.ctr->todo_vit, W.cand.len, W.len_bins, W.todo_sorted, W.cand.vfsc, W.cand.vit_status, &wa,
                                  launch_ssvb)) != BATH_OK) return st;
      ssvb_done = true;
    } else if ((st = launch_vit_wave(ctx, om, cv, W.todo_vit, cap, W.cand.vfsc, W.cand.vit_status, &wa, &W.ctr->todo_vit)) != BATH_OK) return st;
    BATH_HIP_TRY(ctx, hipEventRecord(ev[e++], ctx->stream));
    if (!ssvb_done && (st = launch_ssvb(ctx->stream)) != BATH_OK) return st;
    BATH_HIP_TRY(ctx, hipGetLastError());
    BATH_HIP_TRY(ctx, hipEventRecord(ev[e++], ctx->stream));
    hipLaunchKernelGGL(post_vit_kernel, dim3(dec_blocks), dim3(256), 0, ctx->stream, W.cand, W.cand_cap, W.ctr, P, W.todo_msv , W.todo_fwd);
    if (P.do_bias) {
      DevBuf &b_compo = ctx->scratch[36];
      BATH_HIP_TRY(ctx, b_compo.reserve((size_t)20 * 256 * 4 + (size_t)W.cand_cap * 20 * 4 + 256));
      float *d_terms = b_compo.as<float>(), *d_compo = d_terms + 20 * 256;
      hipLaunchKernelGGL(compo_terms_kernel, dim3(20), dim3(256), 0, ctx->stream, d_bgf, (int)om->base_b, om->scale_b, d_terms);
      hipLaunchKernelGGL(local_compo_kernel, dim3(16384), dim3(64), 0, ctx->stream, W.cand, W.ctr, M, d_ssvsc, d_terms, W.todo_msv, d_compo);
      hipLaunchKernelGGL(post_vit_local_kernel, dim3(std::max(1, dec_blocks)), dim3(64), 0, ctx->stream, W.cand, W.ctr, P, W.pool, M, d_bgf, d_compo,
                         om->lt.d_p1, om->lt.d_lt1, om->lt.d_lt2, W.todo_msv, W.todo_vit2, W.todo_fwd);
    }
    BATH_HIP_TRY(ctx, hipGetLastError());
    if ((st = launch_vit_wave(ctx, om, cv, W.todo_vit2, cap, W.cand.vfsc, W.cand.vit_status, nullptr, &W.ctr->todo_vit2)) != BATH_OK) return st;
    hipLaunchKernelGGL(post_vit2_kernel, dim3(64), dim3(256), 0, ctx->stream, W.cand, W.ctr, P, W.todo_vit2, W.todo_fwd);
    BATH_HIP_TRY(ctx, hipGetLastError());
    BATH_HIP_TRY(ctx, hipEventRecord(ev[e++], ctx->stream));
    ctx->fwd_rows_kept = nullptr; ctx->fwd_rows_off = nullptr;
    float *d_keep = nullptr; int64_t *d_keep_off = nullptr;
    if (ctx->keep_fwd_rows) {
      constexpr int64_t kKeepFloats = (int64_t)8 << 20;
      DevBuf &b_rows = ctx->scratch[38], &b_roff = ctx->scratch[39];
      BATH_HIP_TRY(ctx, b_rows.reserve((size_t)kKeepFloats * sizeof(float) + 64)); BATH_HIP_TRY(ctx, b_roff.reserve((size_t)cap * sizeof(int64_t) + 64));
      d_keep = b_rows.as<float>(); d_keep_off = b_roff.as<int64_t>();
      hipLaunchKernelGGL(fwd_keep_offsets_kernel, dim3(1), dim3(64), 0, ctx->stream, W.todo_fwd, &W.ctr->todo_fwd, W.cand.len, d_keep_off, kKeepFloats);
      BATH_HIP_TRY(ctx, hipGetLastError());
    }
    if ((st = launch_fwd_wave(ctx, om, cv, W.todo_fwd, cap, W.cand.fwdsc, W.cand.fwd_status, &W.ctr->todo_fwd, d_keep, d_keep_off)) != BATH_OK) return st;
    if (d_keep) { ctx->fwd_rows_kept = d_keep; ctx->fwd_rows_off = d_keep_off; }
    hipLaunchKernelGGL(final_kernel, dim3(dec_blocks), dim3(256), 0, ctx->stream, W.cand, W.ctr, P, W.todo_fwd);
    BATH_HIP_TRY(ctx, hipGetLastError());
    BATH_HIP_TRY(ctx, hipEventRecord(ev[e++], ctx->stream));

    BATH_HIP_TRY(ctx, hipMemcpyAsync(&hc, W.ctr, sizeof(Counters), hipMemcpyDeviceToHost, ctx->stream));
    BATH_HIP_TRY(ctx, hipStreamSynchronize(ctx->stream));
    if (hc.overflow || hc.cand_count > cap || hc.win_count > W.win_cap) {
      if (attempt >= 4) { ctx->set_error("candidate / window buffers overflowed repeatedly"); return BATH_EMEM; }
      if (hc.overflow || hc.cand_count > cap) cap = std::max<int64_t>(cap * 2, (int64_t)hc.cand_count + 1024);
      if (hc.win_count > W.win_cap) win_need = hc.win_count + hc.win_count / 4 + 1024;
      continue;
    }
    static const char *names[] = {"translate_orfs", "ssv_f1", "classify_msv", "f1_bias", "viterbi_windows", "ssv_windows", "post_vit", "forward_final"};
    const int64_t launches[] = {4, 1, msv_stage ? 1 : 2, msv_stage ? 0 : 1, 4, 1, 3, 2};
    ctx->timings.clear();
    for (int i = 0; i + 1 < e; i++) {
      float ms = 0.f;
      BATH_HIP_TRY(ctx, hipEventElapsedTime(&ms, ev[i], ev[i + 1]));
      ctx->timings.push_back(StageTiming{names[i], ms, launches[i]});
    }
    break;
  }

  if (stats) {
    stats->nres = nres; stats->n_orfs = (int64_t)hc.n_orfs;
    stats->n_past_msv = (int64_t)hc.n_past_msv; stats->n_past_bias = (int64_t)hc.n_past_bias;
    stats->n_past_vit = (int64_t)hc.n_past_vit; stats->n_past_fwd = (int64_t)hc.n_past_fwd;
    stats->pos_past_msv = (int64_t)hc.pos_past_msv; stats->pos_past_bias = (int64_t)hc.pos_past_bias;
    stats->pos_past_vit = (int64_t)hc.pos_past_vit; stats->pos_past_fwd = (int64_t)hc.pos_past_fwd;
    stats->cells_msv = (int64_t)(hc.orf_res - hc.res_seen) * M; stats->cells_vit = (int64_t)hc.res_vit * M; stats->cells_fwd = (int64_t)hc.res_fwd * M;
  }

  if (results) {
    bath_orf_result *d_rec = nullptr;
    int64_t nrec = 0;
    if (dna->n > (int64_t)UINT32_MAX || dna->maxlen / 3 >= (1 << 28)) { ctx->set_error("block too large for the ORF records' sort key (2^32 windows, 805 Mnt per window)"); return BATH_ERANGE; }
    if ((st = build_orf_records(ctx, W.cand, hc.cand_count, dna->is_part ? dna->first_window : 0, &d_rec, &nrec)) != BATH_OK) return st;
    ctx->d_records = d_rec; ctx->n_records = nrec;
    if (!dna->is_part) {
      BATH_HIP_TRY(ctx, ctx->results_pinned.reserve((size_t)std::max<int64_t>(nrec, 1) * sizeof(bath_orf_result)));
      if (nrec > 0) BATH_HIP_TRY(ctx, hipMemcpyAsync(ctx->results_pinned.p, d_rec, (size_t)nrec * sizeof(bath_orf_result), hipMemcpyDeviceToHost, ctx->stream));
      BATH_HIP_TRY(ctx, hipStreamSynchronize(ctx->stream));
      *results = ctx->results_pinned.as<bath_orf_result>();
    } else *results = nullptr;
    if (n_results) *n_results = nrec;
  } else if (n_results) *n_results = (int64_t)hc.n_past_msv;
  if (state) { state->W = W; state->hc = hc; state->d_ssvsc = d_ssvsc; state->d_bgf = d_bgf; state->tt = tt; }
  return BATH_OK;
}

static int pipeline_lane_count(const bath_hip_seqs *dna) {
  const char *e = std::getenv("BATH_HIP_LANES");
  const int forced = e ? std::atoi(e) : 0;
  if (forced > 0) return (int)std::min<int64_t>(forced, std::max<int64_t>(dna->n, 1));
  if (dna->is_part || dna->n < 8) return 1;
  int K = (dna->total >= ((int64_t)1 << 28)) ? 2 : 1;
  const int64_t by_size = (dna->total + ((int64_t)1 << 34) - 1) >> 34;
  if (by_size > K) K = (int)std::min<int64_t>(by_size, std::max<int64_t>(dna->n, 1));
  return K;
}

static int ensure_parts(bath_hip_ctx *ctx, const bath_hip_seqs *dna, int K) {
  if ((int)dna->parts.size() == K) return BATH_OK;
  for (bath_hip_seqs *p : dna->parts) bath_hip_seqs_destroy(p);
  dna->parts.clear();
  int64_t w0 = 0;
  for (int k = 0; k < K; k++) {
    static const double split2 = [] { const char *e = std::getenv("BATH_HIP_LANE_SPLIT"); const double v = e ? std::atof(e) : 0.0; return (v > 0.05 && v < 0.95) ? v : 0.5; }();
    int64_t w1 = w0;
    if (k == K - 1) w1 = dna->n;
    else {
      const int64_t target = (K == 2) ? (int64_t)((double)dna->total_aligned * split2) : dna->total_aligned / K * (k + 1);
      w1 = std::lower_bound(dna->h_off.begin() + w0, dna->h_off.end(), target) - dna->h_off.begin();
      w1 = std::max(w1, std::min(w0 + 1, dna->n));
    }
    bath_hip_seqs *p = new bath_hip_seqs();
    p->ctx = ctx; p->is_part = true; p->first_window = w0; p->n = w1 - w0;
    const int64_t base = w0 < dna->n ? dna->h_off[(size_t)w0] : dna->total_aligned;
    p->h_off.resize((size_t)p->n); p->h_len.assign(dna->h_len.begin() + w0, dna->h_len.begin() + w1);
    for (int64_t i = 0; i < p->n; i++) {
      p->h_off[(size_t)i] = dna->h_off[(size_t)(w0 + i)] - base;
      p->maxlen = std::max(p->maxlen, p->h_len[(size_t)i]);
      p->total += p->h_len[(size_t)i];
    }
    p->total_aligned = (w1 < dna->n ? dna->h_off[(size_t)w1] : dna->total_aligned) - base;
    p->d_data = dna->d_data + base;
    p->d_len = dna->d_len + w0;
    if (dna->d_context) { p->d_context = dna->d_context + w0; p->h_context.assign(dna->h_context.begin() + w0, dna->h_context.begin() + w1); }
    dna->parts.push_back(p);
    if (hipMalloc((void **)&p->d_off, (size_t)std::max<int64_t>(p->n, 1) * sizeof(int64_t)) != hipSuccess) { ctx->set_error("hipMalloc (block parts)"); return BATH_EMEM; }
    if (p->n > 0 && hipMemcpy(p->d_off, p->h_off.data(), (size_t)p->n * sizeof(int64_t), hipMemcpyHostToDevice) != hipSuccess) { ctx->set_error("hipMemcpy (block parts)"); return BATH_EFAIL; }
    w0 = w1;
  }
  return BATH_OK;
}

template <class After>
static int run_filters_lanes(bath_hip_ctx *ctx, const bath_hip_oprofile *om, const bath_hip_seqs *dna,
                             const bath_pipeline_params *prm, bath_pipeline_stats *stats,
                             const bath_orf_result **results, int64_t *n_results, std::vector<FilterState> *states, After after) {
  if (!ctx || !om || !dna || !prm) return BATH_EINVAL;
  if (cascade_model_ok(ctx, om) != BATH_OK) return BATH_EINVAL;
  const int K = pipeline_lane_count(dna);
  if (K <= 1) {
    states->assign(1, FilterState{});
    int st = run_filters(ctx, om, dna, prm, stats, results, n_results, &(*states)[0]);
    if (st != BATH_OK) return st;
    return after(0, ctx, dna, (*states)[0]);
  }
  BATH_HIP_TRY(ctx, hipSetDevice(ctx->device));
  int st = om->ensure_len_tables(dna->maxlen / 3 + 1);
  if (st != BATH_OK) return st;
  if ((st = ensure_emit_table(ctx, om, prm->F1, dna->maxlen / 3 + 1)) != BATH_OK) return st;
  while ((int)ctx->lanes.size() < K) {
    bath_hip_ctx *lane = nullptr;
    if ((st = bath_hip_init(ctx->device, &lane)) != BATH_OK) { ctx->set_error("cannot create a pipeline lane"); return st; }
    mark_internal(lane);
    const char *pe = std::getenv("BATH_HIP_LANE_PRIO");
    if (!(pe && pe[0] == '0')) {
      int lo = 0, hi = 0;
      if (hipDeviceGetStreamPriorityRange(&lo, &hi) == hipSuccess && lo != hi) {
        (void)hipStreamDestroy(lane->stream);
        const char *te = std::getenv("BATH_HIP_TAIL_PRIO");
        const bool tails = te && te[0] == '1';
        const int prio = tails ? (ctx->lanes.empty() ? std::min(lo, hi + 1) : lo) : (ctx->lanes.empty() ? hi : lo);
        if (hipStreamCreateWithPriority(&lane->stream, hipStreamNonBlocking, prio) != hipSuccess) { ctx->set_error("hipStreamCreateWithPriority"); return BATH_EFAIL; }
        if (tails && hipStreamCreateWithPriority(&lane->tail_stream, hipStreamNonBlocking, hi) != hipSuccess) { ctx->set_error("hipStreamCreateWithPriority"); return BATH_EFAIL; }
      }
    }
    ctx->lanes.push_back(lane);
  }
  for (bath_hip_ctx *lane : ctx->lanes) { lane->fs_strict = ctx->fs_strict; lane->fs_odds = ctx->fs_odds; lane->fs5_odds = ctx->fs5_odds; }
  if ((st = ensure_parts(ctx, dna, K)) != BATH_OK) return st;
// ... 531 lines not shown
```

### bath_amd/csrc/bath_profile.hip

```cpp
#include <atomic>
#include <cctype>
#include <cmath>
#include <cstring>

#include "bath_common.hpp"
#include "host_model.hpp"

using namespace bath;

namespace bath {

static const double kLog2 = 0.69314718055994529;

double gumbel_surv(double x, double mu, double lambda) {
  double ey = -std::exp(-lambda * (x - mu));
  if (std::fabs(ey) < 5e-9) return -ey;
  return 1.0 - std::exp(ey);
}
double gumbel_invsurv(double p, double mu, double lambda) {
  double lp = (p < 5e-9) ? (std::pow(p, p) - 1) / p : std::log(-1. * std::log(1 - p));
  return mu - lp / lambda;
}
double exp_surv(double x, double mu, double lambda) { return (x < mu) ? 1.0 : std::exp(-lambda * (x - mu)); }

// ... 94 lines not shown
    return BATH_ENODEVICE;
  }
  bath::g_ctx_total.fetch_add(1);
  *out = ctx;
  return BATH_OK;
}

extern "C" void bath_hip_finalize(bath_hip_ctx *ctx) {
  if (!ctx) return;
  bath::g_ctx_total.fetch_sub(1);
  if (ctx->internal) bath::g_ctx_internal.fetch_sub(1);
  (void)hipSetDevice(ctx->device);
  (void)hipStreamSynchronize(ctx->stream);
  delete ctx->lane_pool; ctx->lane_pool = nullptr;
  for (bath_hip_ctx *lane : ctx->lanes) bath_hip_finalize(lane);
  ctx->lanes.clear();
  if (ctx->ev_lanes) (void)hipEventDestroy(ctx->ev_lanes);
  if (ctx->tail_stream) (void)hipStreamDestroy(ctx->tail_stream);
  if (ctx->aux) { bath_hip_finalize(ctx->aux); ctx->aux = nullptr; }
  if (ctx->aux2) { bath_hip_finalize(ctx->aux2); ctx->aux2 = nullptr; }
  if (ctx->aux3) { bath_hip_finalize(ctx->aux3); ctx->aux3 = nullptr; }
  for (auto &b : ctx->scratch) b.release();
  for (auto &b : ctx->pinned) b.release();
  for (auto &b : ctx->stage) b.release();
  ctx->results_pinned.release();
  for (auto e : ctx->ev_pool) (void)hipEventDestroy(e);
  for (auto e : ctx->span_events) (void)hipEventDestroy(e);
  if (ctx->ev_fork) (void)hipEventDestroy(ctx->ev_fork);
  if (ctx->ev_join) (void)hipEventDestroy(ctx->ev_join);
  if (ctx->copy_stream) (void)hipStreamDestroy(ctx->copy_stream);
  if (ctx->side_stream) (void)hipStreamDestroy(ctx->side_stream);
  (void)hipStreamDestroy(ctx->stream);
  delete ctx;
}

extern "C" int bath_hip_trim(bath_hip_ctx *ctx) {
  if (!ctx) return BATH_EINVAL;
  BATH_HIP_TRY(ctx, hipSetDevice(ctx->device));
  BATH_HIP_TRY(ctx, hipStreamSynchronize(ctx->stream));
  delete ctx->lane_pool; ctx->lane_pool = nullptr;
  for (bath_hip_ctx *lane : ctx->lanes) bath_hip_finalize(lane);
  ctx->lanes.clear();
  if (ctx->aux) { bath_hip_finalize(ctx->aux); ctx->aux = nullptr; }
  if (ctx->aux2) { bath_hip_finalize(ctx->aux2); ctx->aux2 = nullptr; }
  if (ctx->aux3) { bath_hip_finalize(ctx->aux3); ctx->aux3 = nullptr; }
  if (ctx->tail_stream) { (void)hipStreamDestroy(ctx->tail_stream); ctx->tail_stream = nullptr; }
  if (ctx->copy_stream) { (void)hipStreamSynchronize(ctx->copy_stream); (void)hipStreamDestroy(ctx->copy_stream); ctx->copy_stream = nullptr; }
  if (ctx->side_stream) {
    (void)hipStreamSynchronize(ctx->side_stream); (void)hipStreamDestroy(ctx->side_stream); ctx->side_stream = nullptr;
    if (ctx->ev_fork) { (void)hipEventDestroy(ctx->ev_fork); ctx->ev_fork = nullptr; }
    if (ctx->ev_join) { (void)hipEventDestroy(ctx->ev_join); ctx->ev_join = nullptr; }
  }
  ctx->fs_std_orfs.clear(); ctx->fs_std_pool = nullptr; ctx->fs_keep_xoff.clear(); ctx->fs_regions_all.clear();
  ctx->d_records = nullptr; ctx->n_records = 0;
  return BATH_OK;
}

extern "C" const char *bath_hip_last_error(const bath_hip_ctx *ctx) { return ctx ? ctx->err.c_str() : "no context"; }

extern "C" int bath_hip_synchronize(bath_hip_ctx *ctx) {
  BATH_HIP_TRY(ctx, hipSetDevice(ctx->device));
  BATH_HIP_TRY(ctx, hipStreamSynchronize(ctx->stream));
  return BATH_OK;
}

extern "C" void *bath_hip_stream(bath_hip_ctx *ctx) { return (void *)ctx->stream; }
extern "C" int bath_hip_kernel_times(bath_hip_ctx *ctx, int max, bath_kernel_time *out) {
  if (!ctx || !out) return 0;
  int n = 0;
  for (const bath_hip_ctx *c : {(const bath_hip_ctx *)ctx, (const bath_hip_ctx *)ctx->aux, (const bath_hip_ctx *)ctx->aux2, (const bath_hip_ctx *)ctx->aux3}) {
    if (!c) continue;
    for (const bath::KernelSpan &k : c->spans) {
      float ms = 0.f;
      if (hipEventSynchronize(k.b) != hipSuccess || hipEventElapsedTime(&ms, k.a, k.b) != hipSuccess) continue;
      int i = 0;
      while (i < n && out[i].name != k.name) i++;
      if (i == n) { if (n == max) continue; out[n++] = bath_kernel_time{k.name, 0.f, 0, 0.0, 0.0}; }
      out[i].ms += ms; out[i].launches++; out[i].cells += k.cells; out[i].bytes += k.bytes;
    }
  }
  return n;
}
extern "C" int bath_hip_set_fs_serial(bath_hip_ctx *ctx, int on) {
  if (!ctx) return BATH_EINVAL;
  ctx->fs_serial = on < 0 ? -1 : (on ? 1 : 0);
  return BATH_OK;
}

extern "C" int bath_hip_set_fs_strict(bath_hip_ctx *ctx, int on) {
  if (!ctx) return BATH_EINVAL;
  ctx->fs_strict = on ? 1 : 0;
  if (!on && ctx->aux3) { bath_hip_finalize(ctx->aux3); ctx->aux3 = nullptr; }
  for (bath_hip_ctx *l : ctx->lanes) l->fs_strict = ctx->fs_strict;
  return BATH_OK;
}

extern "C" int bath_hip_set_fs_odds(bath_hip_ctx *ctx, int on) {
  if (!ctx) return BATH_EINVAL;
  ctx->fs_odds = on ? 1 : 0;
  for (bath_hip_ctx *l : ctx->lanes) l->fs_odds = ctx->fs_odds;
  return BATH_OK;
}

extern "C" int bath_hip_set_fs5_odds(bath_hip_ctx *ctx, int on) {
  if (!ctx) return BATH_EINVAL;
  ctx->fs5_odds = on ? 1 : 0;
  for (bath_hip_ctx *l : ctx->lanes) l->fs5_odds = ctx->fs5_odds;
  return BATH_OK;
}

extern "C" int bath_hip_set_fs_ensemble(bath_hip_ctx *ctx, int mode) {
  if (!ctx) return BATH_EINVAL;
  if (mode != BATH_ENSEMBLE_SERIAL && mode != BATH_ENSEMBLE_STREAMS_HOST && mode != BATH_ENSEMBLE_STREAMS_DEVICE) { ctx->set_error("bath_hip_set_fs_ensemble: unknown mode " + std::to_string(mode)); return BATH_EINVAL; }
  ctx->fs_ensemble = mode;
  for (bath_hip_ctx *l : ctx->lanes) l->fs_ensemble = mode;
  return BATH_OK;
}

extern "C" int bath_hip_set_std_ensemble(bath_hip_ctx *ctx, int mode) {
  if (!ctx) return BATH_EINVAL;
  if (mode != BATH_ENSEMBLE_SERIAL && mode != BATH_ENSEMBLE_STREAMS_HOST && mode != BATH_ENSEMBLE_STREAMS_DEVICE) { ctx->set_error("bath_hip_set_std_ensemble: unknown mode " + std::to_string(mode)); return BATH_EINVAL; }
  ctx->std_ensemble = mode;
  for (bath_hip_ctx *l : ctx->lanes) l->std_ensemble = mode;
  if (ctx->aux) ctx->aux->std_ensemble = mode;
  return BATH_OK;
}

extern "C" int bath_hip_std_ensemble_counters(bath_hip_ctx *ctx, int64_t *serial_fallbacks, int64_t *twin_fallbacks, int64_t *kernel_regions) {
  if (!ctx) return BATH_EINVAL;
  int64_t s = 0, t = 0, k = 0;
  for (const bath_hip_ctx *c : {(const bath_hip_ctx *)ctx, (const bath_hip_ctx *)ctx->aux}) {
    if (!c) continue;
    s += c->std_ens_serial_fallbacks.load(); t += c->std_ens_twin_fallbacks.load(); k += c->std_ens_kernel_regions.load();
  }
  if (serial_fallbacks) *serial_fallbacks = s;
  if (twin_fallbacks) *twin_fallbacks = t;
  if (kernel_regions) *kernel_regions = k;
  return BATH_OK;
}

extern "C" int bath_hip_fs_ensemble_counters(bath_hip_ctx *ctx, int64_t *bound_fallbacks, int64_t *overflow_fallbacks, int64_t *matrix_bytes_kept) {
  if (!ctx) return BATH_EINVAL;
  int64_t b = 0, o = 0, k = 0;
  for (const bath_hip_ctx *c : {(const bath_hip_ctx *)ctx, (const bath_hip_ctx *)ctx->aux2}) {
    if (!c) continue;
    b += c->fs_ens_bound_fallbacks.load(); o += c->fs_ens_overflow_fallbacks.load(); k += c->fs_ens_bytes_kept.load();
  }
  if (bound_fallbacks) *bound_fallbacks = b;
  if (overflow_fallbacks) *overflow_fallbacks = o;
  if (matrix_bytes_kept) *matrix_bytes_kept = k;
  return BATH_OK;
}


extern "C" void bath_hip_oprofile_destroy(bath_hip_oprofile *om) {
  if (!om) return;
  for (void *p : {(void *)om->d_emit, (void *)om->d_ssv, (void *)om->d_msv, (void *)om->d_rb, (void *)om->d_rw, (void *)om->d_tw, (void *)om->d_rf, (void *)om->d_tf,
                  (void *)om->d_bias_eo, (void *)om->d_vit_rw, (void *)om->d_vit_tw2, (void *)om->d_vit_rank, (void *)om->lt.d_tjb, (void *)om->lt.d_xwmove, (void *)om->lt.d_pmove,
                  (void *)om->lt.d_nullsc, (void *)om->lt.d_lt1, (void *)om->lt.d_lt2, (void *)om->lt.d_p1, (void *)om->d_cons, (void *)om->d_msc, (void *)om->d_tsc, (void *)om->d_rfb, (void *)om->d_tfb})
    if (p) (void)hipFree(p);
  for (void *p : om->retired) (void)hipFree(p);
  delete om;
}

extern "C" int bath_hip_oprofile_set_consensus(bath_hip_oprofile *om, const char *consensus) {
  if (!om || !consensus) return BATH_EINVAL;
  bath_hip_ctx *ctx = om->ctx;
  static const char syms[] = "ACDEFGHIKLMNPQRSTVWY-BJZOUX*~";
  om->consensus.assign((size_t)om->M + 2, ' ');
  om->cons_digital.assign((size_t)om->M + 1, 255);
  for (int k = 1; k <= om->M && consensus[k]; k++) {
    om->consensus[(size_t)k] = consensus[k];
    const char *q = std::strchr(syms, std::toupper((unsigned char)consensus[k]));
    if (q) om->cons_digital[(size_t)k] = (uint8_t)(q - syms);
  }
  if (!om->d_cons) BATH_HIP_TRY(ctx, hipMalloc(&om->d_cons, (size_t)om->M + 1));
  BATH_HIP_TRY(ctx, hipMemcpy(om->d_cons, om->cons_digital.data(), (size_t)om->M + 1, hipMemcpyHostToDevice));
  return BATH_OK;
}

extern "C" int bath_hip_oprofile_M(const bath_hip_oprofile *om) { return om->M; }

extern "C" int bath_hip_oprofile_convert(bath_hip_ctx *ctx, const bath_profile *gm, bath_hip_oprofile **ret) {
  *ret = nullptr;
  const int M = gm->M;
  if (M < 1) { ctx->set_error("profile has no nodes"); return BATH_EINVAL; }
  BATH_HIP_TRY(ctx, hipSetDevice(ctx->device));
  const size_t W = (size_t)M + 1;
  auto msc = [&](int k, int x) { return gm->rsc[(size_t)x * W * 2 + 2 * k]; };
  auto tsc = [&](int k, int s) { return gm->tsc[(size_t)k * 8 + s]; };
  enum { MM, IM, DM, BM, MD, DD, MI, II };

  bath_hip_oprofile *om = new bath_hip_oprofile();
  { static std::atomic<uint64_t> next_uid{1}; om->uid = next_uid.fetch_add(1); }
  om->ctx = ctx; om->M = M; om->max_length = gm->max_length; om->nj = gm->nj; om->L0 = gm->L;
  std::memcpy(om->evparam, gm->evparam, sizeof om->evparam);
  std::memcpy(om->compo, gm->compo, sizeof om->compo);

  float maxsc = 0.0f;
  for (int x = 0; x < 20; x++)
    for (size_t i = 0; i < W * 2; i++) maxsc = std::max(maxsc, gm->rsc[(size_t)x * W * 2 + i]);
  om->scale_b = (float)(3.0 / kLog2);
  om->base_b = 190;
  om->bias_b = cost_u8(om->scale_b, (float)(-1.0 * maxsc));
  om->rb.assign((size_t)kKp * W, 255);
  for (int x = 0; x < kKp; x++)
    for (int k = 1; k <= M; k++) om->rb[x * W + k] = cost_u8_biased(om->scale_b, om->bias_b, msc(k, x));
  om->tbm_b = cost_u8(om->scale_b, logf(2.0f / ((float)M * (float)(M + 1))));
  om->tec_b = cost_u8(om->scale_b, logf(0.5f));

  om->scale_w = (float)(500.0 / kLog2);
  om->base_w = 12000;
  om->rw.assign((size_t)kKp * W, -32768);
  for (int x = 0; x < kKp; x++)
    for (int k = 1; k <= M; k++) om->rw[x * W + k] = score_i16(om->scale_w, msc(k, x));
  om->tw.assign(W * 8, -32768);
  for (int k = 1; k <= M; k++) {
    int16_t *t = &om->tw[(size_t)k * 8];
    for (int s : {BM, MM, IM, DM}) t[s] = std::min<int16_t>(score_i16(om->scale_w, tsc(k - 1, s)), 0);
    for (int s : {MD, MI}) t[s] = (k < M) ? std::min<int16_t>(score_i16(om->scale_w, tsc(k, s)), 0) : (int16_t)-32768;
    t[II] = (k < M) ? std::min<int16_t>(score_i16(om->scale_w, tsc(k, II)), -1) : (int16_t)-32768;
    t[DD] = (k < M) ? score_i16(om->scale_w, tsc(k, DD)) : (int16_t)-32768;
  }
  om->xw_E[0] = score_i16(om->scale_w, gm->xsc[0][0]);
  om->xw_E[1] = score_i16(om->scale_w, gm->xsc[0][1]);
  int ddb = -32768;
  for (int k = 2; k < M - 1; k++)
    ddb = std::max(ddb, (int)score_i16(om->scale_w, tsc(k, DD)) + (int)score_i16(om->scale_w, tsc(k + 1, DM)) -
                            (int)score_i16(om->scale_w, tsc(k + 1, BM)));
  om->ddbound_w = (int16_t)ddb;

  om->rf.assign((size_t)kKp * W, 0.f);
  for (int x = 0; x < kKp; x++)
    for (int k = 1; k <= M; k++) om->rf[x * W + k] = expf(msc(k, x));
  om->tf.assign(W * 8, 0.f);
  for (int k = 1; k <= M; k++) {
    float *t = &om->tf[(size_t)k * 8];
    for (int s : {BM, MM, IM, DM}) t[s] = expf(tsc(k - 1, s));
    for (int s : {MD, MI, II, DD}) t[s] = (k < M) ? expf(tsc(k, s)) : 0.f;
  }
  om->xf_E[0] = expf(gm->xsc[0][0]);
  om->xf_E[1] = expf(gm->xsc[0][1]);

  {
    std::vector<float> &pre = om->prefix_lengths, &suf = om->suffix_lengths;
    pre.assign(W, 0.f); suf.assign(W, 0.f);
    float total = 0;
    for (int k = 1; k < M; k++) {
      const float t_mi = om->tf[(size_t)k * 8 + MI], t_ii = om->tf[(size_t)k * 8 + II];
      pre[k] = (t_mi == 0) ? 1.f : (float)(1 + (int)(std::log(1e-7 / t_mi) / std::log((double)t_ii)));
      total += pre[k];
    }
    pre[0] = pre[M] = 0;
    for (int k = 1; k < M; k++) pre[k] /= total;
    suf[M] = pre[M - 1];
    for (int k = M - 1; k >= 1; k--) suf[k] = suf[k + 1] + pre[k - 1];
    for (int k = 2; k < M; k++) pre[k] += pre[k - 1];
  }

  static const bool wide = [] { const char *e = std::getenv("BATH_HIP_SSV_WIDE"); return e && e[0] == '1'; }();
  static const int g2max = [] { const char *e = std::getenv("BATH_HIP_SSV_G2_MAX"); return e ? std::atoi(e) : 304; }();
  int G = (!wide && M > 152 && M <= g2max) ? 2 : 1;
  while (G < 8 && M > 416 * G) G *= 2;
  if (M > 416 * G) { ctx->set_error("model longer than 3328 nodes"); delete om; return BATH_EINVAL; }
  int NR = ((M + G - 1) / G + 1) / 2;
  if (G == 1 && NR <= 112) NR = (NR + 3) / 4 * 4;
  else if (G == 2 && NR <= 76) NR = NR <= 40 ? 40 : (NR <= 72 ? (NR + 7) / 8 * 8 : 76);
  else NR = std::max((NR + 15) / 16 * 16, G > 1 ? 112 : 16);
  NR = std::max(NR, 16);
  om->NR = NR; om->G = G;
  om->ssv_row_bytes = 16 * ((NR * G / 4 + 1) | 1);
  {
    size_t rowsz = (size_t)om->ssv_row_bytes / 2;
    auto half_bits = [](float v) { const _Float16 h = (_Float16)v; int16_t b; std::memcpy(&b, &h, 2); return b; };
    std::vector<int16_t> tab((size_t)kSsvRows * rowsz, half_bits(-1.0f));
    for (int x = 0; x < kKp; x++)
      for (int k = 1; k <= M; k++) {
        const int g = (k - 1) / (2 * NR), q = (k - 1) - g * 2 * NR;
        const int cost = std::min((int)om->rb[x * W + k] - (int)om->bias_b, 127);
        tab[x * rowsz + (size_t)g * 2 * NR + 2 * (q % NR) + q / NR] = half_bits(-(float)cost / 2048.0f);
      }
    BATH_HIP_TRY(ctx, upload(&om->d_ssv, tab.data(), tab.size(), ctx->stream));
    if (G == 1 && NR <= 76) {
      std::vector<int16_t> mtab((size_t)kSsvRows * rowsz, half_bits(-1.0f));
      for (int x = 0; x < kKp; x++)
        for (int k = 1; k <= M; k++) {
          const int q = k - 1;
          const int inc = (int)om->bias_b - (int)om->rb[x * W + k];
          mtab[x * rowsz + 2 * (q % NR) + q / NR] = half_bits((float)inc / 2048.0f);
        }
      BATH_HIP_TRY(ctx, upload(&om->d_msv, mtab.data(), mtab.size(), ctx->stream));
    }
  }
  {
    int NRv = ((M + 1) / 2 + 15) / 16 * 16;
    if (NRv == 80) NRv = std::max(68, ((M + 1) / 2 + 3) / 4 * 4);
    if (NRv <= BATH_TILING_MAX(BATH_VIT_LANE_NR)) {
      om->vit_NR = NRv;
      om->vit_rw_pitch = 4 * NRv + 16;
      const size_t rowsz = (size_t)om->vit_rw_pitch / 2;
      std::vector<int16_t> rwt((size_t)30 * rowsz, (int16_t)-32768);
      auto slot = [&](int node) { return node <= NRv ? 2 * (node - 1) : 2 * (node - NRv - 1) + 1; };
      for (int x = 0; x < kKp; x++)
        for (int k = 1; k <= M; k++) rwt[x * rowsz + slot(k)] = om->rw[x * W + k];
      std::vector<uint32_t> tw2((size_t)NRv * 8);
      std::vector<int16_t> rank((size_t)2 * NRv, (int16_t)32767);
      const int Q8 = std::max(2, ((M - 1) / 8) + 1);
      auto twv = [&](int node, int s) -> int { return node <= M ? (int)om->tw[(size_t)node * 8 + s] : -32768; };
      for (int r = 0; r < NRv; r++)
        for (int s = 0; s < 8; s++) tw2[(size_t)r * 8 + s] = ((uint32_t)(uint16_t)twv(r + 1, s)) | ((uint32_t)(uint16_t)twv(NRv + r + 1, s) << 16);
      for (int node = 1; node <= M; node++) rank[(size_t)slot(node)] = (int16_t)(((node - 1) % Q8) * 8 + (node - 1) / Q8);
      BATH_HIP_TRY(ctx, upload(&om->d_vit_rw, rwt.data(), rwt.size(), ctx->stream));
      BATH_HIP_TRY(ctx, upload(&om->d_vit_tw2, tw2.data(), tw2.size(), ctx->stream));
      BATH_HIP_TRY(ctx, upload(&om->d_vit_rank, rank.data(), rank.size(), ctx->stream));
    }
  }
  om->rb_stride = (int)W;
  BATH_HIP_TRY(ctx, upload(&om->d_rb, om->rb.data(), om->rb.size(), ctx->stream));
  BATH_HIP_TRY(ctx, upload(&om->d_rw, om->rw.data(), om->rw.size(), ctx->stream));
  BATH_HIP_TRY(ctx, upload(&om->d_tw, om->tw.data(), om->tw.size(), ctx->stream));
  BATH_HIP_TRY(ctx, upload(&om->d_rf, om->rf.data(), om->rf.size(), ctx->stream));
  BATH_HIP_TRY(ctx, upload(&om->d_tf, om->tf.data(), om->tf.size(), ctx->stream));
  {
    std::vector<float> tfb((size_t)(M + 2) * 8, 0.f), rfb((size_t)kKp * (M + 2), 0.f);
    std::memcpy(tfb.data(), om->tf.data(), sizeof(float) * (size_t)(M + 1) * 8);
    for (int x = 0; x < kKp; x++) std::memcpy(&rfb[(size_t)x * (M + 2)], &om->rf[(size_t)x * W], sizeof(float) * W);
    BATH_HIP_TRY(ctx, upload(&om->d_tfb, tfb.data(), tfb.size(), ctx->stream));
    BATH_HIP_TRY(ctx, upload(&om->d_rfb, rfb.data(), rfb.size(), ctx->stream));
    BATH_HIP_TRY(ctx, hipStreamSynchronize(ctx->stream));
  }
  {
    std::vector<float> lm((size_t)kKp * W, -INFINITY);
    for (int x = 0; x < kKp; x++)
      for (int k = 1; k <= M; k++) lm[(size_t)x * W + k] = msc(k, x);
    BATH_HIP_TRY(ctx, upload(&om->d_msc, lm.data(), lm.size(), ctx->stream));
    BATH_HIP_TRY(ctx, upload(&om->d_tsc, gm->tsc, (size_t)M * 8, ctx->stream));
    BATH_HIP_TRY(ctx, hipStreamSynchronize(ctx->stream));
  }
  {
    float eo[kKp][2];
    bias_filter_eo(om->compo, eo);
    BATH_HIP_TRY(ctx, upload(&om->d_bias_eo, &eo[0][0], (size_t)kKp * 2, ctx->stream));
  }
  BATH_HIP_TRY(ctx, hipStreamSynchronize(ctx->stream));
  int st = om->ensure_len_tables(4096);
  if (st != BATH_OK) { bath_hip_oprofile_destroy(om); return st; }
  *ret = om;
  return BATH_OK;
}

extern "C" int bath_hip_oprofile_scalars(const bath_hip_oprofile *om, int L, bath_oprofile_scalars *o) {
  int st = om->ensure_len_tables(L);
  if (st != BATH_OK) return st;
  o->tbm_b = om->tbm_b; o->tec_b = om->tec_b; o->tjb_b = om->lt.h_tjb[L]; o->base_b = om->base_b; o->bias_b = om->bias_b;
  o->scale_b = om->scale_b;
  o->xw[0][0] = om->xw_E[0]; o->xw[0][1] = om->xw_E[1];
  for (int s = 1; s < 4; s++) { o->xw[s][0] = 0; o->xw[s][1] = om->lt.h_xwmove[L]; }
  o->scale_w = om->scale_w; o->base_w = om->base_w; o->ddbound_w = om->ddbound_w;
  o->xf[0][0] = om->xf_E[0]; o->xf[0][1] = om->xf_E[1];
  for (int s = 1; s < 4; s++) { o->xf[s][1] = om->lt.h_pmove[L]; o->xf[s][0] = 1.0f - om->lt.h_pmove[L]; }
  return BATH_OK;
}

extern "C" int bath_hip_oprofile_get_ssv_scores(const bath_hip_oprofile *om, uint8_t *arr) {
  const size_t W = (size_t)om->M + 1;
  std::memset(arr, 0, W * kKp);
  for (int k = 1; k <= om->M; k++)
    for (int x = 0; x < kKp; x++) arr[(size_t)k * kKp + x] = om->rb[x * W + k];
  return BATH_OK;
}
extern "C" int bath_hip_oprofile_get_vit(const bath_hip_oprofile *om, int16_t *rw, int16_t *tw) {
  std::memcpy(rw, om->rw.data(), om->rw.size() * sizeof(int16_t));
  std::memcpy(tw, om->tw.data(), om->tw.size() * sizeof(int16_t));
  return BATH_OK;
}
extern "C" int bath_hip_oprofile_get_fwd(const bath_hip_oprofile *om, float *rf, float *tf) {
  std::memcpy(rf, om->rf.data(), om->rf.size() * sizeof(float));
  std::memcpy(tf, om->tf.data(), om->tf.size() * sizeof(float));
  return BATH_OK;
}


extern "C" void bath_hip_seqs_destroy(bath_hip_seqs *sq) {
  if (!sq) return;
  for (bath_hip_seqs *part : sq->parts) bath_hip_seqs_destroy(part);
  sq->parts.clear();
  if (sq->is_part) { sq->d_data = nullptr; sq->d_len = nullptr; sq->d_context = nullptr; }
  for (void *p : {(void *)sq->d_data, (void *)sq->d_off, (void *)sq->d_len, (void *)sq->d_context, (void *)sq->d_tile_desc, (void *)sq->d_tile_first,
                  (void *)sq->d_packed, (void *)sq->d_poff, sq->d_exc})
    if (p) (void)hipFree(p);
  if (sq->ev_upload) (void)hipEventDestroy(sq->ev_upload);
  delete sq;
}

extern "C" int64_t bath_hip_seqs_count(const bath_hip_seqs *sq) { return sq->n; }

extern "C" int64_t bath_hip_seqs_read(const bath_hip_seqs *sq, uint8_t *data, int64_t cap, int64_t *offsets, int32_t *lengths, int32_t *context) {
  if (!sq || cap < 0 || (cap > 0 && !data)) return -1;
  bath_hip_ctx *ctx = sq->ctx;
  const int64_t bytes = sq->total_aligned + 64;
  if (hipSetDevice(ctx->device) != hipSuccess || hipStreamSynchronize(ctx->stream) != hipSuccess) { ctx->set_error("seqs_read: the block's stream failed"); return -1; }
  auto get = [&](void *dst, const void *src, size_t n) { return n == 0 || !dst || hipMemcpy(dst, src, n, hipMemcpyDeviceToHost) == hipSuccess; };
  const bool ok = get(data, sq->d_data, (size_t)std::min(cap, bytes)) && get(offsets, sq->d_off, (size_t)sq->n * sizeof(int64_t)) &&
                  get(lengths, sq->d_len, (size_t)sq->n * sizeof(int32_t)) &&
                  (!context || (sq->d_context ? get(context, sq->d_context, (size_t)sq->n * sizeof(int32_t)) : (std::memset(context, 0, (size_t)sq->n * sizeof(int32_t)), true)));
  if (!ok) { ctx->set_error("seqs_read: copy to the host failed"); return -1; }
  return bytes;
}

extern "C" int bath_hip_seqs_set_context(bath_hip_seqs *sq, const int32_t *context) {
  if (!sq || sq->is_part) return BATH_EINVAL;
  bath_hip_ctx *ctx = sq->ctx;
  BATH_HIP_TRY(ctx, hipSetDevice(ctx->device));
  for (bath_hip_seqs *part : sq->parts) bath_hip_seqs_destroy(part);
  sq->parts.clear();
  sq->cache_minlen = -1;
  if (!context) { if (sq->d_context) (void)hipFree(sq->d_context); sq->d_context = nullptr; sq->h_context.clear(); return BATH_OK; }
  for (int64_t i = 0; i < sq->n; i++) if (context[i] < 0 || context[i] > sq->h_len[(size_t)i]) { ctx->set_error("context longer than its window"); return BATH_EINVAL; }
  sq->h_context.assign(context, context + sq->n);
  if (!sq->d_context) BATH_HIP_TRY(ctx, hipMalloc((void **)&sq->d_context, (size_t)std::max<int64_t>(sq->n, 1) * sizeof(int32_t)));
  if (sq->n > 0) BATH_HIP_TRY(ctx, hipMemcpy(sq->d_context, sq->h_context.data(), (size_t)sq->n * sizeof(int32_t), hipMemcpyHostToDevice));
  return BATH_OK;
}

extern "C" int bath_hip_seqs_create(bath_hip_ctx *ctx, const uint8_t *dsq, const int64_t *offsets, int64_t n, bath_hip_seqs **ret) {
  *ret = nullptr;
  if (n < 0) return BATH_EINVAL;
  BATH_HIP_TRY(ctx, hipSetDevice(ctx->device));
  bath_hip_seqs *sq = new bath_hip_seqs();
  sq->ctx = ctx; sq->n = n;
  sq->h_off.resize(n); sq->h_len.resize(n);
  int64_t pos = 0;
  bool contiguous_ok = true;
  for (int64_t i = 0; i < n; i++) {
    int64_t L = offsets[i + 1] - offsets[i];
    if (L < 0 || L > INT32_MAX) { delete sq; ctx->set_error("bad sequence offsets"); return BATH_EINVAL; }
    sq->h_off[i] = pos; sq->h_len[i] = (int32_t)L;
    if (pos != offsets[i] - offsets[0]) contiguous_ok = false;
    sq->maxlen = std::max(sq->maxlen, (int32_t)L);
    sq->total += L;
    pos += (L + 15) / 16 * 16;
  }
  sq->total_aligned = pos;
  size_t bytes = (size_t)pos + 64;
  BATH_HIP_TRY(ctx, hipMalloc((void **)&sq->d_data, bytes));
  BATH_HIP_TRY(ctx, hipMalloc((void **)&sq->d_off, (size_t)std::max<int64_t>(n, 1) * sizeof(int64_t)));
  BATH_HIP_TRY(ctx, hipMalloc((void **)&sq->d_len, (size_t)std::max<int64_t>(n, 1) * sizeof(int32_t)));
  BATH_HIP_TRY(ctx, hipMemsetAsync(sq->d_data, 0x1d, bytes, ctx->stream));
  std::vector<uint8_t> staged;
  if (n > 0) {
    if (contiguous_ok) {
      BATH_HIP_TRY(ctx, hipMemcpyAsync(sq->d_data, dsq + offsets[0], (size_t)(offsets[n] - offsets[0]), hipMemcpyHostToDevice, ctx->stream));
    } else {
      staged.assign((size_t)pos, 0x1d);
      for (int64_t i = 0; i < n; i++) std::memcpy(staged.data() + sq->h_off[i], dsq + offsets[i], (size_t)sq->h_len[i]);
      BATH_HIP_TRY(ctx, hipMemcpyAsync(sq->d_data, staged.data(), staged.size(), hipMemcpyHostToDevice, ctx->stream));
    }
    BATH_HIP_TRY(ctx, hipMemcpyAsync(sq->d_off, sq->h_off.data(), (size_t)n * sizeof(int64_t), hipMemcpyHostToDevice, ctx->stream));
    BATH_HIP_TRY(ctx, hipMemcpyAsync(sq->d_len, sq->h_len.data(), (size_t)n * sizeof(int32_t), hipMemcpyHostToDevice, ctx->stream));
  }
  BATH_HIP_TRY(ctx, hipStreamSynchronize(ctx->stream));
  *ret = sq;
  return BATH_OK;
}


namespace {
struct ExcRec { int64_t seq; int32_t pos, code; };

__global__ __launch_bounds__(256) void unpack2_kernel(const uint8_t *__restrict__ packed, const int64_t *__restrict__ poff, const int64_t *__restrict__ off,
                                                      const int32_t *__restrict__ len, uint8_t *__restrict__ data, int64_t n) {
  const int64_t s = (int64_t)blockIdx.x * 4 + (threadIdx.x >> 6);
  if (s >= n) return;
  const int lane = threadIdx.x & 63;
  const int L = len[s];
  const int nb = (L + 3) >> 2;
  const uint8_t *src = packed + poff[s];
  uint8_t *dst = data + off[s];
  const int j_lo = blockIdx.y * 4096, j_hi = min((nb + 3) >> 2, j_lo + 4096);
  for (int j = j_lo + lane; j < j_hi; j += 64) {
    uint32_t w;
    if (4 * j + 4 <= nb) w = *reinterpret_cast<const uint32_t *>(src + 4 * j);
    else { w = 0; for (int q = 0; 4 * j + q < nb; q++) w |= (uint32_t)src[4 * j + q] << (8 * q); }
    uint32_t v[4];
#pragma unroll
    for (int q = 0; q < 4; q++) {
      const unsigned b = (w >> (8 * q)) & 0xffu;
      v[q] = (b & 3u) | ((b >> 2) & 3u) << 8 | ((b >> 4) & 3u) << 16 | ((b >> 6) & 3u) << 24;
    }
    if (16 * j + 16 <= L) *reinterpret_cast<uint4 *>(dst + 16 * j) = make_uint4(v[0], v[1], v[2], v[3]);
    else for (int q = 0; 16 * j + q < L; q++) dst[16 * j + q] = (uint8_t)((v[q >> 2] >> (8 * (q & 3))) & 0xffu);
  }
}
__global__ void unpack_exceptions_kernel(const ExcRec *__restrict__ exc, int64_t n, const int64_t *__restrict__ off, uint8_t *__restrict__ data) {
  const int64_t i = (int64_t)blockIdx.x * blockDim.x + threadIdx.x;
  if (i < n) data[off[exc[i].seq] + exc[i].pos] = (uint8_t)exc[i].code;
}
}
// ... 78 lines not shown
```

### bath_amd/csrc/bath_viterbi.hip

```cpp
#include <algorithm>
#include <cstdlib>
#include <functional>

#include "bath_common.hpp"
#include "bath_kernels.hpp"
#include "bath_launch.hpp"

using namespace bath;

namespace bath {

__device__ __forceinline__ s16x2 pk_adds(s16x2 a, s16x2 b) { return __builtin_elementwise_add_sat(a, b); }
__device__ __forceinline__ s16x2 pk_max(s16x2 a, s16x2 b) { return __builtin_elementwise_max(a, b); }
__device__ __forceinline__ s16x2 as_s2(unsigned v) { return __builtin_bit_cast(s16x2, v); }
__device__ __forceinline__ unsigned as_u(s16x2 v) { return __builtin_bit_cast(unsigned, v); }

struct VitLaneTables {
  const int16_t *rw;
  int rw_pitch_bytes;
  const uint32_t *tw2;
  const int16_t *rank;
};

struct VitLaneConsts {
// ... 25 lines not shown
    for (int i = threadIdx.x; i < 2 * NR; i += blockDim.x) s_rank[i] = tb.rank[i];
  }
  __syncthreads();
  if (ntodo_dev) ntodo = *ntodo_dev;
  const int64_t t = (int64_t)blockIdx.x * blockDim.x + threadIdx.x + (skip_dev ? *skip_dev : 0);
  if (t - (threadIdx.x & 63) >= ntodo) return;
  const bool live = t < ntodo;
  const int64_t sid = live ? (todo ? (int64_t)todo[t] : t) : (todo ? (int64_t)todo[0] : 0);
  const int L = live ? sq.len[sid] : 0;
  const uint8_t *s = sq.data + sq.off[sid];
  const int Lw = wave_max_i32(L);
  const bool do_win = (wins != nullptr);
  const int M = c.M;

  const int xw_move = xwmove_tab[L];
  int sc_thresh = 0, sc_ext_thresh = 0, skip_until = 0, kmin = 1 << 30, kmax = 0;
  if (do_win && live) {
    const double fsc = (double)filtersc[sid];
    sc_thresh = (int)(int16_t)(int)ceil(((fsc + 0.69314718055994529 * c.invP_vit + 3.0) * (double)c.scale_w) -
                                        (double)(float)c.xwE_move - (double)(float)xw_move + (double)(float)c.base_w);
    sc_ext_thresh = (int)ceil(((fsc + 0.69314718055994529 * c.invP_msv + 3.0) * (double)c.scale_b) + c.base_b + c.tec_b + (int)tjb_tab[L]);
  }
  const s16x2 NEG = {-32768, -32768};
  s16x2 Mr[NR], Ir[NR], Dr[NR];
#pragma unroll
  for (int r = 0; r < NR; r++) Mr[r] = Ir[r] = Dr[r] = NEG;
  int xN = c.base_w;
  int xB = (int16_t)(xN + xw_move);
  int xJ = -32768, xC = -32768;
  bool overflow = false;
  short ePrev = -32768;

  uint32_t wnext = (0 < L) ? *reinterpret_cast<const uint32_t *>(s) : 0x1d1d1d1du;
  for (int i0 = 0; i0 < Lw; i0 += 4) {
    const uint32_t w = wnext;
    wnext = (i0 + 4 < L) ? *reinterpret_cast<const uint32_t *>(s + i0 + 4) : 0x1d1d1d1du;
#pragma unroll 1
    for (int j = 0; j < 4; j++) {
      const int i = i0 + j + 1;
      const bool on = (i <= L) && !overflow;
      int x = (w >> (8 * j)) & 0xff;
      x = (i <= L) ? min(x, kKp - 1) : 29;
      const char *rowbase = s_rw + x * tb.rw_pitch_bytes;
      const s16x2 xBv = {(short)xB, (short)xB};
      s16x2 xEv = NEG;
      unsigned pM = (as_u(Mr[NR - 1]) << 16) | 0x8000u, pI = (as_u(Ir[NR - 1]) << 16) | 0x8000u, pD = (as_u(Dr[NR - 1]) << 16) | 0x8000u;
      s16x2 dpk = NEG;
      s16x2 cpk = {(short)-32768, ePrev};
      int twz = 0;
      asm volatile("" : "+s"(twz));
      const uint32_t *tw = tw2g + twz;
      u32x16 t_c, t_n;
      int4 e_c = *reinterpret_cast<const int4 *>(rowbase), e_n = e_c;
      asm volatile("s_load_dwordx16 %0, %1, 0x0" : "=s"(t_c) : "s"(tw));
#pragma unroll
      for (int r = 0; r < NR; r += 2) {
        asm volatile("s_waitcnt lgkmcnt(0)" ::: "memory");
        __builtin_amdgcn_sched_barrier(0);
        if ((r & 3) == 0 && r + 4 < NR) e_n = *reinterpret_cast<const int4 *>(rowbase + 4 * (r + 4));
        if (r + 2 < NR) asm volatile("s_load_dwordx16 %0, %1, %2" : "=s"(t_n) : "s"(tw), "i"((r + 2) * 32));
        __builtin_amdgcn_sched_barrier(0);
        const unsigned em[2] = {(r & 3) ? (unsigned)e_c.z : (unsigned)e_c.x, (r & 3) ? (unsigned)e_c.w : (unsigned)e_c.y};
#pragma unroll
        for (int q = 0; q < 2; q++) {
          const int rr = r + q;
          const unsigned tMM = t_c[8 * q + 0], tIM = t_c[8 * q + 1], tDM = t_c[8 * q + 2], tBM = t_c[8 * q + 3];
          const unsigned tMD = t_c[8 * q + 4], tDD = t_c[8 * q + 5], tMI = t_c[8 * q + 6], tII = t_c[8 * q + 7];
          const unsigned oM = as_u(Mr[rr]), oI = as_u(Ir[rr]);
          const unsigned oD = as_u(pk_max(Dr[rr], cpk));
          cpk = pk_adds(cpk, as_s2(tDD));
          const s16x2 ms = as_s2(pM), is = as_s2(pI), ds = as_s2(pD);
          s16x2 sv = pk_adds(xBv, as_s2(tBM));
          sv = pk_max(sv, pk_adds(ms, as_s2(tMM)));
          sv = pk_max(sv, pk_adds(is, as_s2(tIM)));
          sv = pk_max(sv, pk_adds(ds, as_s2(tDM)));
          sv = pk_adds(sv, as_s2(em[q]));
          Ir[rr] = pk_max(pk_adds(as_s2(oM), as_s2(tMI)), pk_adds(as_s2(oI), as_s2(tII)));
          const s16x2 dcv = pk_adds(sv, as_s2(tMD));
          xEv = pk_max(xEv, sv);
          Mr[rr] = sv;
          Dr[rr] = dpk;
          dpk = pk_max(dcv, pk_adds(dpk, as_s2(tDD)));
          pM = oM; pI = oI; pD = oD;
        }
        if (r + 2 < NR) t_c = t_n;
        if ((r & 3) == 2 && r + 2 < NR) e_c = e_n;
        asm volatile("" : "+v"(Mr[r]), "+v"(Mr[r + 1]), "+v"(Ir[r]), "+v"(Ir[r + 1]), "+v"(Dr[r]), "+v"(Dr[r + 1]), "+v"(dpk), "+v"(cpk), "+v"(xEv));
        __builtin_amdgcn_sched_barrier(0);
      }
      ePrev = dpk.x;
      if (on) {
        const int xE = max((int)xEv.x, (int)xEv.y);
        if (xE >= 32767) overflow = true;
        else {
          xN = (int16_t)(xN + 0);
          xC = (int16_t)max(xC + 0, xE + c.xwE_move);
          xJ = (int16_t)max(xJ + 0, xE + c.xwE_loop);
          xB = (int16_t)max(xJ + xw_move, xN + xw_move);
          if (do_win && i > skip_until && xE >= sc_thresh) {
            int rank = 32767;
#pragma unroll
            for (int r = 0; r < NR; r++) {
              if ((int)Mr[r].x == xE) rank = min(rank, (int)s_rank[2 * r]);
              if ((int)Mr[r].y == xE) rank = min(rank, (int)s_rank[2 * r + 1]);
            }
            const int k_start = (rank / 8) + c.Q8 * (rank % 8) + 1;
            int max_k_end = k_start, max_i_end = i, sc_ext = sc_ext_thresh, max_sc_ext = sc_ext, since = 0;
            int kk = k_start + 1, nn = i + 1;
            while (kk <= M && nn <= L) {
              sc_ext += c.bias_b - (int)ssv_scores[(size_t)kk * kKp + min((int)s[nn - 1], kKp - 1)];
              if (sc_ext >= max_sc_ext) { max_sc_ext = sc_ext; max_k_end = kk; max_i_end = nn; since = 0; }
              else if (++since == 5) break;
              kk++; nn++;
            }
            const int slot = atomicAdd(win_count, 1);
            if (slot < win_cap) wins[slot] = WindowRec{(int32_t)sid, i, max_k_end, max_k_end - k_start + 1, 0.0f};
            kmax = max(kmax, max_k_end);
            kmin = min(kmin, k_start);
            skip_until = max_i_end;
          }
        }
      }
    }
  }
  if (live) {
    if (overflow) { sc[sid] = INFINITY; status[sid] = BATH_ERANGE; }
    else if (xC > -32768) {
      float r = (float)xC + (float)xw_move - (float)c.base_w;
      r /= c.scale_w;
      r = (float)((double)r - 3.0);
      sc[sid] = r; status[sid] = BATH_OK;
    } else { sc[sid] = -INFINITY; status[sid] = BATH_OK; }
    if (do_win && kminmax) { kminmax[2 * sid] = kmin; kminmax[2 * sid + 1] = kmax; }
  }
}

constexpr int kLenBins = 2048;
constexpr int kVitLongTarget = 128;
__device__ __forceinline__ void len_block_range(int n, int &lo, int &hi) {
  const int per = (n + (int)gridDim.x - 1) / (int)gridDim.x;
  lo = min(n, (int)blockIdx.x * per); hi = min(n, lo + per);
}
__global__ __launch_bounds__(256) void len_hist_kernel(const int32_t *__restrict__ todo, const int *__restrict__ ntodo_dev, const int32_t *__restrict__ len,
                                                       int *__restrict__ hist) {
  __shared__ int s_cnt[kLenBins];
  for (int i = threadIdx.x; i < kLenBins; i += blockDim.x) s_cnt[i] = 0;
  __syncthreads();
  int lo, hi;
  len_block_range(*ntodo_dev, lo, hi);
  for (int j = lo + threadIdx.x; j < hi; j += blockDim.x) atomicAdd(&s_cnt[min(len[todo[j]], kLenBins - 1)], 1);
  __syncthreads();
  for (int i = threadIdx.x; i < kLenBins; i += blockDim.x) if (s_cnt[i]) atomicAdd(&hist[i], s_cnt[i]);
}
__global__ void len_scan_kernel(int *__restrict__ hist ) {
  __shared__ int tmp[kLenBins];
  for (int i = threadIdx.x; i < kLenBins; i += blockDim.x) tmp[i] = hist[i];
  __syncthreads();
  if (threadIdx.x == 0) {
    int run = 0;
    for (int b = kLenBins - 1; b >= 0; b--) { const int cnt = tmp[b]; tmp[b] = run; run += cnt; }
  }
  __syncthreads();
  for (int i = threadIdx.x; i < kLenBins; i += blockDim.x) hist[i] = tmp[i];
}
__global__ __launch_bounds__(256) void len_scatter_kernel(const int32_t *__restrict__ todo, const int *__restrict__ ntodo_dev, const int32_t *__restrict__ len,
                                                          int *__restrict__ cursor, int32_t *__restrict__ sorted) {
  __shared__ int s_cnt[kLenBins];
  for (int i = threadIdx.x; i < kLenBins; i += blockDim.x) s_cnt[i] = 0;
  __syncthreads();
  int lo, hi;
  len_block_range(*ntodo_dev, lo, hi);
  for (int j = lo + threadIdx.x; j < hi; j += blockDim.x) atomicAdd(&s_cnt[min(len[todo[j]], kLenBins - 1)], 1);
  __syncthreads();
  for (int i = threadIdx.x; i < kLenBins; i += blockDim.x) { const int c = s_cnt[i]; if (c) s_cnt[i] = atomicAdd(&cursor[i], c); }
  __syncthreads();
  for (int j = lo + threadIdx.x; j < hi; j += blockDim.x) {
    const int cnd = todo[j];
    sorted[atomicAdd(&s_cnt[min(len[cnd], kLenBins - 1)], 1)] = cnd;
  }
}

int vit_lane_supported(const bath_hip_oprofile *om) { return om->vit_NR > 0; }

const int *len_sort_count_longer(const int *d_bins, int T) { return d_bins + std::min(T + 1, kLenBins - 1); }

int launch_len_sort(bath_hip_ctx *ctx, const int32_t *d_todo, const int *d_ntodo, const int32_t *d_len, int *d_bins, int32_t *d_sorted) {
  BATH_HIP_TRY(ctx, hipMemsetAsync(d_bins, 0, kLenBins * sizeof(int), ctx->stream));
  hipLaunchKernelGGL(len_hist_kernel, dim3(256), dim3(256), 0, ctx->stream, d_todo, d_ntodo, d_len, d_bins);
  hipLaunchKernelGGL(len_scan_kernel, dim3(1), dim3(256), 0, ctx->stream, d_bins);
  hipLaunchKernelGGL(len_scatter_kernel, dim3(256), dim3(256), 0, ctx->stream, d_todo, d_ntodo, d_len, d_bins, d_sorted);
  BATH_HIP_TRY(ctx, hipGetLastError());
  return BATH_OK;
}

int launch_vit_lane(bath_hip_ctx *ctx, const bath_hip_oprofile *om, SeqView v, const int32_t *d_todo, int64_t ntodo, const int *ntodo_dev,
                    float *d_sc, int32_t *d_status, const VitWindowArgs *wa, const int *skip_dev) {
  if (ntodo == 0) return BATH_OK;
  VitLaneTables tb{om->d_vit_rw, om->vit_rw_pitch, om->d_vit_tw2, om->d_vit_rank};
  VitLaneConsts c{};
  c.M = om->M; c.base_w = om->base_w; c.xwE_loop = om->xw_E[0]; c.xwE_move = om->xw_E[1]; c.Q8 = std::max(2, ((om->M - 1) / 8) + 1);
  c.scale_w = om->scale_w; c.scale_b = om->scale_b; c.base_b = om->base_b; c.tec_b = om->tec_b; c.bias_b = om->bias_b;
  const float *fsc = nullptr; const uint8_t *ssv = nullptr; WindowRec *wins = nullptr; int *wc = nullptr; int cap = 0; int32_t *kmm = nullptr;
  if (wa) { c.invP_vit = wa->invP_vit; c.invP_msv = wa->invP_msv; fsc = wa->d_filtersc; ssv = wa->d_ssv_scores; wins = (WindowRec *)wa->d_wins; wc = wa->d_win_count; cap = wa->win_cap; kmm = wa->d_kminmax; }
  const int NRv = om->vit_NR;
  const size_t shmem = (size_t)30 * om->vit_rw_pitch + (size_t)2 * NRv * 2 + 16;
  const int blocks = (int)((ntodo + 255) / 256);
  bool launched = false;
#define BATH_VITL_CASE(N, ...)                                                                                                         \
  if (!launched && NRv == N) {                                                                                                         \
    hipLaunchKernelGGL(vit_lane_kernel<N>, dim3(blocks), dim3(256), shmem, ctx->stream, v, tb, tb.tw2, c, om->lt.d_xwmove, om->lt.d_tjb, d_todo, ntodo, \
                       ntodo_dev, skip_dev, d_sc, d_status, fsc, ssv, wins, wc, cap, kmm);                                                       \
    launched = true;                                                                                                                   \
  }
  BATH_VIT_LANE_NR(BATH_VITL_CASE)
#undef BATH_VITL_CASE
  if (!launched) { ctx->set_error("lane-per-target Viterbi kernel: unsupported model length"); return BATH_EINVAL; }
  BATH_HIP_TRY(ctx, hipGetLastError());
  return BATH_OK;
}

int64_t lane_min_nt() {
  static const int64_t v = [] { const char *e = std::getenv("BATH_HIP_LANE_MIN_NT"); return e ? std::atoll(e) : (int64_t)150'000'000; }();
  return v;
}

const char *vit_lane_kernel_name(const bath_hip_oprofile *om) {
#define BATH_VITL_NAME(N, ...) if (om->vit_NR == N) return "vit_lane_kernel<" #N ">";
  BATH_VIT_LANE_NR(BATH_VITL_NAME)
#undef BATH_VITL_NAME
  return "vit_lane_kernel<?>";
}

int launch_vit_sorted(bath_hip_ctx *ctx, const bath_hip_oprofile *om, SeqView v, const int32_t *d_todo, int64_t cap, const int *d_ntodo, const int32_t *d_len,
                      int *d_bins, int32_t *d_sorted, float *d_sc, int32_t *d_status, const VitWindowArgs *wa, const std::function<int(hipStream_t)> &beside) {
  int st;
  if ((st = launch_len_sort(ctx, d_todo, d_ntodo, d_len, d_bins, d_sorted)) != BATH_OK) return st;
  if (!ctx->side_stream) {
    BATH_HIP_TRY(ctx, hipStreamCreateWithFlags(&ctx->side_stream, hipStreamNonBlocking));
    BATH_HIP_TRY(ctx, hipEventCreateWithFlags(&ctx->ev_fork, hipEventDisableTiming));
    BATH_HIP_TRY(ctx, hipEventCreateWithFlags(&ctx->ev_join, hipEventDisableTiming));
  }
  static const int long_orf = [] { const char *e = std::getenv("BATH_HIP_VIT_LONG"); return e ? std::atoi(e) : kVitLongTarget; }();
  const int *d_nlong = len_sort_count_longer(d_bins, long_orf);
  BATH_HIP_TRY(ctx, hipEventRecord(ctx->ev_fork, ctx->stream));
  BATH_HIP_TRY(ctx, hipStreamWaitEvent(ctx->side_stream, ctx->ev_fork, 0));
  {
    hipStream_t main_stream = ctx->stream;
    ctx->stream = ctx->side_stream;
    st = launch_vit_wave(ctx, om, v, d_sorted, cap, d_sc, d_status, wa, d_nlong);
    ctx->stream = main_stream;
    if (st != BATH_OK) return st;
    if (beside && (st = beside(ctx->side_stream)) != BATH_OK) return st;
  }
  BATH_HIP_TRY(ctx, hipEventRecord(ctx->ev_join, ctx->side_stream));
  if ((st = launch_vit_lane(ctx, om, v, d_sorted, cap, d_ntodo, d_sc, d_status, wa, d_nlong)) != BATH_OK) return st;
  BATH_HIP_TRY(ctx, hipStreamWaitEvent(ctx->stream, ctx->ev_join, 0));
  return BATH_OK;
}

}
```

### include/bath_hip.h

```cpp
#ifndef BATH_HIP_H
#define BATH_HIP_H

#include <stdint.h>
#include <stddef.h>

#ifdef __cplusplus
extern "C" {
#endif

#define BATH_OK          0
#define BATH_EFAIL       1
#define BATH_EMEM        5
#define BATH_EFORMAT     7
#define BATH_EINVAL     11
#define BATH_ERANGE     16
#define BATH_ENORESULT  19
#define BATH_ENODEVICE  40

#define BATH_KP_AMINO   29
#define BATH_K_AMINO    20
#define BATH_KP_DNA     18
#define BATH_NEVPARAM    8
#define BATH_FTAU        4
#define BATH_FLAMBDA     5
// ... 294 lines not shown
                           float *pp, float *oa, float *ppx, float *oax);
int bath_hip_std_envelopes_fill(bath_hip_ctx *ctx, const bath_hip_oprofile *om, const bath_hip_seqs *sq, bath_std_result *res,
                                float *pp, float *oa, float *ppx, float *oax, int fill);

typedef struct bath_tophits bath_tophits;
bath_tophits *bath_tophits_create(void);
void bath_tophits_destroy(bath_tophits *th);
int  bath_tophits_add(bath_tophits *th, const bath_fs_domain *dom, int64_t n, const char *cigars, int64_t seqidx0,
                      const char *const *seq_names, const char *const *seq_accs, const char *const *seq_descs, const int64_t *seq_lens);
int  bath_tophits_finalize(bath_tophits *th, int64_t nres, int max_length, double E);
void bath_tophits_set_score_thresholds(bath_tophits *th, int by_E, double T, int inc_by_E, double incT);
int64_t bath_search_space_residues(int Z_is_set, double Z_megabases, int strands, int64_t nres_searched);
int64_t bath_tophits_count(const bath_tophits *th);
int64_t bath_tophits_reported(const bath_tophits *th);
#define BATH_HIT_REPORTED  1
#define BATH_HIT_DUPLICATE 4
int  bath_tophits_get(const bath_tophits *th, int64_t rank, bath_fs_domain *dom, int64_t *seqidx, int32_t *flags);
int64_t bath_tophits_targets(const bath_tophits *th, int fs_pipe, int textw, char *buf, int64_t cap);
int64_t bath_tophits_domain_annotation(const bath_tophits *th, int64_t rank, int M, int fs_pipe, char *buf, int64_t cap);
int64_t bath_tophits_pipeline_statistics(const bath_tophits *th, const bath_pipeline_stats *stats, const bath_pipeline_params *params,
                                         int64_t nmodels, int64_t nnodes, int64_t nseqs, char *buf, int64_t cap);
void bath_tophits_set_inclusion(bath_tophits *th, double incE);
#define BATH_HIT_INCLUDED  2
int64_t bath_tophits_tabular_targets(const bath_tophits *th, const char *qname, const char *qacc, int M, int fs_pipe,
                                     int show_cigar, int show_header, char *buf, int64_t cap);

typedef struct {
  char    type;
  int32_t length;
  int32_t ali_start;
  int64_t seq_start;
} bath_fs_row;
int64_t bath_trace_frameshift_rows(const bath_domain_trace *tr, const int8_t *st, const int32_t *k, const int32_t *i, const int8_t *c,
                                   const uint8_t *window_dsq, int32_t window_len, const bath_fs_profile *gm_fs5, int64_t iali, int64_t jali,
                                   bath_fs_row *rows, int64_t cap);
int64_t bath_tophits_tabular_frameshifts(const bath_tophits *th, const char *qname, const char *qacc, const bath_fs_row *rows,
                                         const int64_t *row_off, int64_t n_reported, int show_header, char *buf, int64_t cap);

typedef struct bath_hits bath_hits;
int64_t bath_hits_serialize(const bath_fs_domain *dom, int64_t n, const char *cigars, const bath_domain_trace *tr,
                            const int8_t *st, const int32_t *k, const int32_t *i, const int8_t *c, const float *pp,
                            uint8_t *buf, int64_t cap);
int     bath_hits_deserialize(const uint8_t *buf, int64_t nbytes, bath_hits **ret);
int64_t bath_hits_stream_size(const uint8_t *buf, int64_t nbytes);
void    bath_hits_destroy(bath_hits *h);
int64_t bath_hits_count(const bath_hits *h);
bath_fs_domain *bath_hits_domains(bath_hits *h);
const char *bath_hits_cigars(const bath_hits *h, int64_t *nbytes);
int     bath_hits_traces(const bath_hits *h, const bath_domain_trace **tr, const int8_t **st, const int32_t **k, const int32_t **i,
                         const int8_t **c, const float **pp);
int     bath_tophits_add_serialized(bath_tophits *th, const uint8_t *buf, int64_t nbytes, int64_t window_shift, int64_t n_seqs, int64_t seqidx0,
                                    const char *const *seq_names, const char *const *seq_accs, const char *const *seq_descs, const int64_t *seq_lens);

typedef struct { int32_t query; int64_t lo, hi; } bath_dist_item;
void    bath_dist_shard_range(int64_t n, int rank, int world, int64_t *lo, int64_t *hi);
int64_t bath_dist_items(const int64_t *n_windows_by_query, const double *costs_by_query, int n_queries, int world, int items_per_rank,
                        bath_dist_item *items, int64_t cap);
int     bath_dist_deal(const double *costs, int64_t n_items, int world, int32_t *owner);

#define BATH_LOGSUM_TABLE 0
#define BATH_LOGSUM_EXACT 1
#define BATH_LOGSUM_TABLE_SERIAL 2
#define BATH_LOGSUM_CONTEXT 3
#define BATH_LOGSUM_ODDS 4

int  bath_hip_fsprofile_convert(bath_hip_ctx *ctx, const bath_fs_profile *gm_fs, bath_hip_fsprofile **ret);
void bath_hip_fsprofile_destroy(bath_hip_fsprofile *om);

int bath_hip_fs3_forward_parser(bath_hip_ctx *ctx, const bath_hip_fsprofile *om3, const bath_hip_seqs *dna, int logsum_mode,
                                float *sc, float *xmx, const int64_t *xmx_offsets);
int bath_hip_fs3_backward_parser(bath_hip_ctx *ctx, const bath_hip_fsprofile *om3, const bath_hip_seqs *dna, int logsum_mode,
                                 float *sc, float *xmx, const int64_t *xmx_offsets);

typedef struct {
  float fwdsc, bcksc, oasc;
  float null2[BATH_KP_AMINO];
} bath_fs5_result;
int bath_hip_fs5_envelopes(bath_hip_ctx *ctx, const bath_hip_fsprofile *om5, const bath_hip_seqs *dna, int logsum_mode, int c5_compat,
                           bath_fs5_result *res,
                           float *pp , const int64_t *pp_offsets,
                           float *oa , const int64_t *oa_offsets);

int bath_hip_fs5_envelopes_x(bath_hip_ctx *ctx, const bath_hip_fsprofile *om5, const bath_hip_seqs *dna, int logsum_mode, int c5_compat,
                             bath_fs5_result *res, float *pp, float *oa, float *ppx, float *oax);
int bath_hip_fs5_forward_full(bath_hip_ctx *ctx, const bath_hip_fsprofile *om5, const bath_hip_seqs *dna, int cfg_len_amino,
                              float *sc, float *fwd, float *xmx);

int bath_hip_fs5_forward_parser(bath_hip_ctx *ctx, const bath_hip_fsprofile *om5, const bath_hip_seqs *dna, int cfg_len_amino, float *sc);
int bath_hip_fs5_forward_parser_odds(bath_hip_ctx *ctx, const bath_hip_fsprofile *om5, const bath_hip_seqs *dna, int cfg_len_amino, float *sc);

int bath_calib_sample(uint32_t *rng_state, const float *f, int ncbi_table, int L, int N, uint8_t *dna);
int    bath_gumbel_fit_complete(const double *x, int n, double *mu, double *lambda);
double bath_gumbel_invcdf(double p, double mu, double lambda);
int    bath_calib_tau(const double *xv, int n, double lambda_model, double tailp, double *tau);
float  bath_bg_fs_nullone(int L_amino);
int    bath_hmm_max_length(const bath_hmm *hmm, double emit_thresh);
int bath_hip_calibrate_fs(bath_hip_ctx *ctx, const bath_hmm *hmm, int ncbi_table, uint32_t *rng_state, int L, int N, double tailp,
                          double *tau3, double *tau5, double *xv3, double *xv5);
typedef int (*bath_calib_score_fn)(void *user, const uint8_t *dna, int n, int L3, float *sc);
int bath_calib_fit_scores(uint32_t *rng_state, const float *f, int ncbi_table, int L, int N, bath_calib_score_fn score, void *user,
                          float nullsc, double *xv, int *n_redrawn);
#define BATH_ARITH_STRICT 0
#define BATH_ARITH_ODDS3  1
#define BATH_ARITH_ODDS   2
int bath_hip_calibrate_fs_arith(bath_hip_ctx *ctx, const bath_hmm *hmm, int ncbi_table, uint32_t *rng_state, int L, int N, double tailp,
                                double *tau3, double *tau5, double *xv3, double *xv5, int arith, int *redrawn);

typedef struct bath_scoresystem bath_scoresystem;
const char *bath_scorematrix_builtin(const char *name);
int    bath_scoresystem_create(const char *mx_name, const char *mxfile, double popen, double pextend, bath_scoresystem **ret,
                               char *errbuf, int errlen);
void   bath_scoresystem_destroy(bath_scoresystem *s);
double bath_scoresystem_lambda(const bath_scoresystem *s);
int    bath_scoresystem_conditionals(const bath_scoresystem *s, double *Q );
int    bath_hmm_from_sequence(const bath_scoresystem *s, const uint8_t *dsq, int n, const char *name, int ct, bath_hmm **ret);
double bath_hmm_mean_match_relent(const bath_hmm *hmm);
double bath_hmm_lambda(const bath_hmm *hmm);
int64_t bath_hmm_write_ascii(const bath_hmm *hmm, int nseq, double eff_nseq, const char *desc, const char *date, const char *comlog,
                             char *buf, int64_t cap);
int bath_calib_sample_amino(uint32_t *rng_state, const float *f, int L, int N, uint8_t *aa);
int bath_gumbel_fit_complete_loc(const double *x, int n, double lambda, double *mu);
typedef struct bath_hip_calib_samples bath_hip_calib_samples;
int  bath_hip_calib_samples_create(bath_hip_ctx *ctx, uint32_t *rng_state, int EmL, int EmN, int EvL, int EvN, int EfL, int EfN,
                                   bath_hip_calib_samples **ret);
void bath_hip_calib_samples_destroy(bath_hip_calib_samples *s);
int  bath_hip_calibrate(bath_hip_ctx *ctx, bath_hmm *hmm, int ncbi_table, uint32_t *rng_state, bath_hip_calib_samples *samples,
                        int EmL, int EmN, int EvL, int EvN, int EfL, int EfN, double Eft, int arith, double *xv, int *redrawn);

int bath_hip_fs5_region_ensembles(bath_hip_ctx *ctx, const bath_hip_fsprofile *om5, const bath_hip_seqs *regions, uint32_t seed,
                                  int32_t *region_status, int32_t *trace_status, int32_t *seg, int64_t max_seg, int64_t *seg_off,
                                  int32_t *env, int64_t max_env, int64_t *env_off);

int bath_hip_std_region_ensembles(bath_hip_ctx *ctx, const bath_hip_oprofile *om, const bath_hip_seqs *regions, const int32_t *cfg_len, uint32_t seed,
                                  int32_t *region_status, int32_t *trace_status, int32_t *seg, int64_t max_seg, int64_t *seg_off,
                                  int32_t *env, float *env_n2corr, int64_t max_env, int64_t *env_off);

int bath_selftest_rng_stream(uint32_t seed, int n, double *out);
int bath_selftest_fchoose(uint32_t seed, const float *p, int n, int draws, int32_t *out);
int bath_selftest_cluster_segments(int n, const int32_t *idx, const int32_t *i, const int32_t *j, const int32_t *k, const int32_t *m,
                                   int nsamples, int fs, int32_t *env, int max_env, int32_t *n_env);
int bath_selftest_fs_ensemble(int M, const float *tsc, float xNL, float xNM, float xE, int ireg, int Lr, const float *fwd, const float *fx,
                              int32_t *env, int max_env, int32_t *n_env);
int bath_selftest_fs_ensemble_seeded(int M, const float *tsc, float xNL, float xNM, float xE, int ireg, int Lr, const float *fwd, const float *fx,
                                     uint32_t seed, int32_t *env, int max_env, int32_t *n_env);
int bath_selftest_fs_ensemble_streams(int M, const float *tsc, float xNL, float xNM, float xE, int ireg, int Lr, const float *fwd, const float *fx,
                                      uint32_t seed, int32_t *region_status, int32_t *trace_status, int32_t *seg, int max_seg, int32_t *n_seg,
                                      int32_t *env, int max_env, int32_t *n_env);
int bath_selftest_std_ensemble(int mode, int M, const float *tf, const float *rf, float pmove, float tEL, float tEM, const uint8_t *res, int Lr,
                               const float *fwd, const float *fx, uint32_t seed, int32_t *region_status, int32_t *trace_status,
                               int32_t *seg, int max_seg, int32_t *n_seg, float *n2sc, int32_t *env, int max_env, int32_t *n_env);
int bath_selftest_std_ens_walk(int M, const float *tf, float pmove, float tEL, float tEM, int Lr, const float *fwd, const float *fx, uint32_t rng_state,
                               int32_t *status, int32_t *seg, int max_seg, int32_t *n_seg);
int bath_selftest_rng_jump(uint32_t seed, uint64_t n, uint32_t *state);
int bath_selftest_ens_explog(int n, const float *x, float *e, float *l);

#ifdef __cplusplus
}
#endif
#endif
```

Baseline: 201.1 billion.

## Aggregate pipeline stage counters and todo lists in LDS before global atomics

Replaces per-candidate global atomicAdds in the classify, f1/bias, post-Viterbi and final filter kernels with block-local LDS tallies. Each block collects its list entries and counter sums, reserves one global slot range per list, and flushes when its local buffer nears capacity. The change also precomputes the composition term table once per profile instead of launching it every pipeline batch, and parallelizes the length-bin scan with wave shuffles instead of a single thread. It adds extra __syncthreads and LDS use per block, and the order of entries in the todo lists changes.

```diff
diff --git a/bath_amd/__init__.py b/bath_amd/__init__.py
--- a/bath_amd/__init__.py
+++ b/bath_amd/__init__.py
@@ -204,6 +204,9 @@
                                                     _i32p, _i32p, _i32p, C.c_int, _i32p, _i32p, C.c_int, _i32p]),
     "bath_selftest_rng_jump": (C.c_int, [C.c_uint32, C.c_uint64, C.POINTER(C.c_uint32)]),
     "bath_selftest_ens_explog": (C.c_int, [C.c_int, _f32p, _f32p, _f32p]),
+    "bath_selftest_compute_units": (C.c_int, [_vp]),
+    "bath_selftest_compo_terms": (C.c_int, [C.c_int, C.c_float, _f32p]),
+    "bath_selftest_len_sort": (C.c_int, [_vp, C.c_int, _i32p, C.c_int, _i32p, _i32p]),
     "bath_hip_trim": (C.c_int, [_vp]),
     "bath_hip_kernel_times": (C.c_int, [_vp, C.c_int, C.POINTER(KernelTime)]),
     "bath_hip_oprofile_convert": (C.c_int, [_vp, C.POINTER(_Profile), C.POINTER(_vp)]),
diff --git a/bath_amd/csrc/bath_common.hpp b/bath_amd/csrc/bath_common.hpp
--- a/bath_amd/csrc/bath_common.hpp
+++ b/bath_amd/csrc/bath_common.hpp
@@ -327,6 +327,7 @@
   float *d_rfb = nullptr, *d_tfb = nullptr;
   float *d_msc = nullptr, *d_tsc = nullptr;
   float *d_bias_eo = nullptr;
+  float *d_compo_terms = nullptr;
   int vit_NR = 0, vit_rw_pitch = 0;
   int16_t *d_vit_rw = nullptr; uint32_t *d_vit_tw2 = nullptr; int16_t *d_vit_rank = nullptr;
   mutable LenTables lt;
@@ -340,6 +341,7 @@
 
 namespace bath {
 int build_len_tables(const bath_hip_oprofile *om, int maxL);
+int build_compo_terms(bath_hip_ctx *ctx, bath_hip_oprofile *om);
 void bias_filter_eo(const float *compo, float eo[kKp][2]);
 double gumbel_surv(double x, double mu, double lambda);
 double gumbel_invsurv(double p, double mu, double lambda);
diff --git a/bath_amd/csrc/bath_pipeline.hip b/bath_amd/csrc/bath_pipeline.hip
--- a/bath_amd/csrc/bath_pipeline.hip
+++ b/bath_amd/csrc/bath_pipeline.hip
@@ -142,18 +142,84 @@
   return st;
 }
 
-__global__ void classify_kernel(Cand cand, int cand_cap, Counters *__restrict__ ctr, const uint8_t *__restrict__ tjb_tab, MsvConsts mc,
-                                int32_t *__restrict__ todo_msv) {
+template <int NL, int NS, int CAP>
+struct BlockTally {
+  int n[NL > 0 ? NL : 1], base[NL > 0 ? NL : 1];
+  unsigned long long sum[NS > 0 ? NS : 1];
+  int32_t ids[NL > 0 ? NL : 1][NL > 0 ? CAP : 1];
+};
+template <int NL, int NS>
+struct TallyOut {
+  int32_t *list[NL > 0 ? NL : 1]; int *count[NL > 0 ? NL : 1];
+  unsigned long long *sum[NS > 0 ? NS : 1];
+};
+template <int NL, int NS, int CAP>
+__device__ __forceinline__ void tally_reset(BlockTally<NL, NS, CAP> &t) {
+  if ((int)threadIdx.x < NL) t.n[threadIdx.x] = 0;
+  if ((int)threadIdx.x < NS) t.sum[threadIdx.x] = 0ull;
+  __syncthreads();
+}
+template <int NL, int NS, int CAP>
+__device__ __forceinline__ void tally_add(BlockTally<NL, NS, CAP> &t, int k, unsigned long long v) { atomicAdd(&t.sum[k], v); }
+template <int NL, int NS, int CAP>
+__device__ __forceinline__ void tally_push(BlockTally<NL, NS, CAP> &t, int l, int32_t id) { t.ids[l][atomicAdd(&t.n[l], 1)] = id; }
+template <int NL, int NS, int CAP>
+__device__ __forceinline__ bool tally_lists_full(BlockTally<NL, NS, CAP> &t) {
+  bool full = false;
+  __syncthreads();
+#pragma unroll
+  for (int l = 0; l < NL; l++) full |= t.n[l] > CAP - (int)blockDim.x;
+  __syncthreads();
+  return full;
+}
+template <int NL, int NS, int CAP>
+__device__ __forceinline__ void tally_write_lists(BlockTally<NL, NS, CAP> &t, const TallyOut<NL, NS> &o) {
+  if (NL == 0) return;
+  __syncthreads();
+#pragma unroll
+  for (int l = 0; l < NL; l++) if ((int)threadIdx.x == l && t.n[l] > 0) t.base[l] = atomicAdd(o.count[l], t.n[l]);
+  __syncthreads();
+#pragma unroll
+  for (int l = 0; l < NL; l++) {
+    const int n = t.n[l], b = t.base[l];
+    for (int i = threadIdx.x; i < n; i += blockDim.x) o.list[l][b + i] = t.ids[l][i];
+  }
+  __syncthreads();
+  if ((int)threadIdx.x < NL) t.n[threadIdx.x] = 0;
+  __syncthreads();
+}
+template <int NL, int NS, int CAP>
+__device__ __forceinline__ void tally_finish(BlockTally<NL, NS, CAP> &t, const TallyOut<NL, NS> &o) {
+  tally_write_lists(t, o);
+  if (NL == 0) __syncthreads();
+#pragma unroll
+  for (int k = 0; k < NS; k++) if ((int)threadIdx.x == k && t.sum[k] != 0ull) atomicAdd(o.sum[k], t.sum[k]);
+}
+
+__global__ __launch_bounds__(256) void classify_kernel(Cand cand, int cand_cap, Counters *__restrict__ ctr, const uint8_t *__restrict__ tjb_tab, MsvConsts mc,
+                                                       int32_t *__restrict__ todo_msv) {
+  __shared__ BlockTally<1, 0, 512> tally;
+  tally_reset(tally);
+  const TallyOut<1, 0> out{{todo_msv}, {&ctr->todo_msv}, {nullptr}};
   const int ncand = min(ctr->cand_count, cand_cap);
-  for (int c = blockIdx.x * blockDim.x + threadIdx.x; c < ncand; c += gridDim.x * blockDim.x) {
-    if (cand_classify(cand, c, tjb_tab[cand.len[c]], mc) == BATH_ENORESULT) todo_msv[atomicAdd(&ctr->todo_msv, 1)] = c;
-  }
+  for (int c0 = blockIdx.x * blockDim.x; c0 < ncand; c0 += gridDim.x * blockDim.x) {
+    if (tally_lists_full(tally)) tally_write_lists(tally, out);
+    const int c = c0 + threadIdx.x;
+    if (c < ncand && cand_classify(cand, c, tjb_tab[cand.len[c]], mc) == BATH_ENORESULT) tally_push(tally, 0, c);
+  }
+  tally_finish(tally, out);
 }
 
 struct F1Tables { const float *eo, *nullsc, *p1, *lt1, *lt2; };
-__device__ __forceinline__ void cand_f1_bias(const Cand &cand, int c, Counters *__restrict__ ctr, const Params &p, const uint8_t *__restrict__ pool, int M,
-                                             const float *s_eo , const F1Tables &t,
-                                             int32_t *__restrict__ todo_vit, int32_t *__restrict__ todo_ssvb) {
+enum { F1_TODO_VIT = 0, F1_TODO_SSVB = 1, F1_NL = 2 };
+enum { F1_N_MSV = 0, F1_POS_MSV, F1_N_BIAS, F1_POS_BIAS, F1_RES_VIT, F1_NS };
+__device__ __forceinline__ TallyOut<F1_NL, F1_NS> f1_tally_out(Counters *__restrict__ ctr, int32_t *__restrict__ todo_vit, int32_t *__restrict__ todo_ssvb) {
+  return TallyOut<F1_NL, F1_NS>{{todo_vit, todo_ssvb}, {&ctr->todo_vit, &ctr->todo_ssvb},
+                                {&ctr->n_past_msv, &ctr->pos_past_msv, &ctr->n_past_bias, &ctr->pos_past_bias, &ctr->res_vit}};
+}
+template <int CAP>
+__device__ __forceinline__ void cand_f1_bias(const Cand &cand, int c, BlockTally<F1_NL, F1_NS, CAP> &tally, const Params &p, const uint8_t *__restrict__ pool, int M,
+                                             const float *s_eo , const F1Tables &t) {
   const int L = cand.len[c];
   const float usc = cand.usc[c];
   const float nullsc = t.nullsc[L];
@@ -162,7 +228,7 @@
   double P = d_gumbel_surv(seqsc, p.evparam[0], p.evparam[1]);
   cand.P[c] = P;
   if (P > p.F1) return;
-  atomicAdd(&ctr->n_past_msv, 1ull); atomicAdd(&ctr->pos_past_msv, (unsigned long long)L * 3ull);
+  tally_add(tally, F1_N_MSV, 1ull); tally_add(tally, F1_POS_MSV, (unsigned long long)L * 3ull);
   cand.stage[c] = 1;
   float filtersc = nullsc;
   if (p.do_bias) {
@@ -174,19 +240,26 @@
     if (P > p.F1) return;
   }
   cand.filtersc[c] = filtersc;
-  atomicAdd(&ctr->n_past_bias, 1ull); atomicAdd(&ctr->pos_past_bias, (unsigned long long)L * 3ull);
+  tally_add(tally, F1_N_BIAS, 1ull); tally_add(tally, F1_POS_BIAS, (unsigned long long)L * 3ull);
   cand.stage[c] = 2;
-  if (P > p.F2) { cand.flags[c] |= FLAG_VIT_RUN; todo_vit[atomicAdd(&ctr->todo_vit, 1)] = c; atomicAdd(&ctr->res_vit, (unsigned long long)L); }
-  else todo_ssvb[atomicAdd(&ctr->todo_ssvb, 1)] = c;
-}
-
-__global__ void f1_bias_kernel(Cand cand, int cand_cap, Counters *__restrict__ ctr, Params p, const uint8_t *__restrict__ pool, int M, F1Tables t,
-                               int32_t *__restrict__ todo_vit, int32_t *__restrict__ todo_ssvb) {
+  if (P > p.F2) { cand.flags[c] |= FLAG_VIT_RUN; tally_push(tally, F1_TODO_VIT, c); tally_add(tally, F1_RES_VIT, (unsigned long long)L); }
+  else tally_push(tally, F1_TODO_SSVB, c);
+}
+
+__global__ __launch_bounds__(256) void f1_bias_kernel(Cand cand, int cand_cap, Counters *__restrict__ ctr, Params p, const uint8_t *__restrict__ pool, int M, F1Tables t,
+                                                      int32_t *__restrict__ todo_vit, int32_t *__restrict__ todo_ssvb) {
   __shared__ float s_eo[kKp * 2];
+  __shared__ BlockTally<F1_NL, F1_NS, 512> tally;
   for (int i = threadIdx.x; i < kKp * 2; i += blockDim.x) s_eo[i] = t.eo[i];
-  __syncthreads();
+  tally_reset(tally);
+  const TallyOut<F1_NL, F1_NS> out = f1_tally_out(ctr, todo_vit, todo_ssvb);
   const int ncand = min(ctr->cand_count, cand_cap);
-  for (int c = blockIdx.x * blockDim.x + threadIdx.x; c < ncand; c += gridDim.x * blockDim.x) cand_f1_bias(cand, c, ctr, p, pool, M, s_eo, t, todo_vit, todo_ssvb);
+  for (int c0 = blockIdx.x * blockDim.x; c0 < ncand; c0 += gridDim.x * blockDim.x) {
+    if (tally_lists_full(tally)) tally_write_lists(tally, out);
+    const int c = c0 + threadIdx.x;
+    if (c < ncand) cand_f1_bias(cand, c, tally, p, pool, M, s_eo, t);
+  }
+  tally_finish(tally, out);
 }
 
 template <int NR>
@@ -196,6 +269,7 @@
                                                            F1Tables t, int32_t *__restrict__ todo_vit, int32_t *__restrict__ todo_ssvb) {
   extern __shared__ __attribute__((aligned(16))) char lds[];
   __shared__ float s_eo[kKp * 2];
+  __shared__ BlockTally<F1_NL, F1_NS, 256> tally;
   const int ncand = min(ctr->cand_count, cand_cap);
   if ((int64_t)blockIdx.x * blockDim.x >= ncand) return;
   {
@@ -205,7 +279,7 @@
     for (int i = threadIdx.x; i < n32; i += blockDim.x) dst[i] = src[i];
     for (int i = threadIdx.x; i < kKp * 2; i += blockDim.x) s_eo[i] = t.eo[i];
   }
-  __syncthreads();
+  tally_reset(tally);
   const int64_t job = (int64_t)blockIdx.x * blockDim.x + threadIdx.x;
   const bool live = job < ncand;
   const int c = live ? (int)job : 0;
@@ -220,7 +294,8 @@
     if (overflow) { cand.usc[c] = INFINITY; cand.msv_status[c] = BATH_ERANGE; }
     else { cand.usc[c] = msv_lane_score(xJ, tjb, mc); cand.msv_status[c] = BATH_OK; }
   }
-  if (live) cand_f1_bias(cand, c, ctr, p, pool, M, s_eo, t, todo_vit, todo_ssvb);
+  if (live) cand_f1_bias(cand, c, tally, p, pool, M, s_eo, t);
+  tally_finish(tally, f1_tally_out(ctr, todo_vit, todo_ssvb));
 }
 
 template <int C>
@@ -351,32 +426,44 @@
   }
 }
 
-__global__ void post_vit_kernel(Cand cand, int cand_cap, Counters *__restrict__ ctr, Params p, int32_t *__restrict__ todo_lb, int32_t *__restrict__ todo_fwd) {
+enum { PV_TODO_LB = 0, PV_TODO_FWD = 1, PV_NL = 2 };
+enum { PV_N_VIT = 0, PV_POS_VIT, PV_RES_FWD, PV_NS };
+__global__ __launch_bounds__(256) void post_vit_kernel(Cand cand, int cand_cap, Counters *__restrict__ ctr, Params p, int32_t *__restrict__ todo_lb, int32_t *__restrict__ todo_fwd) {
+  __shared__ BlockTally<PV_NL, PV_NS, 512> tally;
+  tally_reset(tally);
+  const TallyOut<PV_NL, PV_NS> out{{todo_lb, todo_fwd}, {&ctr->todo_lb, &ctr->todo_fwd}, {&ctr->n_past_vit, &ctr->pos_past_vit, &ctr->res_fwd}};
   const int ncand = min(ctr->cand_count, cand_cap);
-  for (int c = blockIdx.x * blockDim.x + threadIdx.x; c < ncand; c += gridDim.x * blockDim.x) {
-    if (cand.stage[c] != 2) continue;
-    const int L = cand.len[c];
-    if (cand.flags[c] & FLAG_VIT_RUN) {
+  for (int c0 = blockIdx.x * blockDim.x; c0 < ncand; c0 += gridDim.x * blockDim.x) {
+    if (tally_lists_full(tally)) tally_write_lists(tally, out);
+    const int c = c0 + threadIdx.x;
+    bool past = c < ncand && cand.stage[c] == 2;
+    if (past && (cand.flags[c] & FLAG_VIT_RUN)) {
       const float seqsc = (float)((double)(cand.vfsc[c] - cand.filtersc[c]) / kLog2);
       const double P = d_gumbel_surv(seqsc, p.evparam[2], p.evparam[3]);
       cand.P[c] = P;
-      if (P > p.F2) { cand.kminmax[2 * c] = 1 << 30; cand.kminmax[2 * c + 1] = 0; continue; }
-    }
-    atomicAdd(&ctr->n_past_vit, 1ull); atomicAdd(&ctr->pos_past_vit, (unsigned long long)L * 3ull);
+      if (P > p.F2) { cand.kminmax[2 * c] = 1 << 30; cand.kminmax[2 * c + 1] = 0; past = false; }
+    }
+    if (!past) continue;
+    const int L = cand.len[c];
+    tally_add(tally, PV_N_VIT, 1ull); tally_add(tally, PV_POS_VIT, (unsigned long long)L * 3ull);
     if (p.do_bias && cand.kminmax[2 * c] <= cand.kminmax[2 * c + 1]) {
       cand.flags[c] |= FLAG_HAS_WIN;
-      todo_lb[atomicAdd(&ctr->todo_lb, 1)] = c;
+      tally_push(tally, PV_TODO_LB, c);
       continue;
     }
     cand.stage[c] = 3;
-    todo_fwd[atomicAdd(&ctr->todo_fwd, 1)] = c; atomicAdd(&ctr->res_fwd, (unsigned long long)L);
-  }
-}
-
+    tally_push(tally, PV_TODO_FWD, c); tally_add(tally, PV_RES_FWD, (unsigned long long)L);
+  }
+  tally_finish(tally, out);
+}
+
+__host__ __device__ __forceinline__ float compo_term(float bg, int base_b, int sc, float scale_b) {
+  const float lo = ((float)base_b - (float)sc) / scale_b;
+  return bg * expf(lo);
+}
 __global__ void compo_terms_kernel(const float *__restrict__ bgf, int base_b, float scale_b, float *__restrict__ terms ) {
   const int x = blockIdx.x, sc = threadIdx.x;
-  const float lo = ((float)base_b - (float)sc) / scale_b;
-  terms[x * 256 + sc] = bgf[x] * expf(lo);
+  terms[x * 256 + sc] = compo_term(bgf[x], base_b, sc, scale_b);
 }
 
 __global__ __launch_bounds__(64) void local_compo_kernel(Cand cand, const Counters *__restrict__ ctr, int M, const uint8_t *__restrict__ ssv_scores,
@@ -403,8 +490,14 @@
                                                             const float *__restrict__ p1_tab, const float *__restrict__ lt1_tab, const float *__restrict__ lt2_tab,
                                                             const int32_t *__restrict__ todo_lb, int32_t *__restrict__ todo_vit2, int32_t *__restrict__ todo_fwd) {
   __shared__ float s_eo[64][kKp * 2 + 1];
+  __shared__ BlockTally<2, 2, 128> tally;
+  tally_reset(tally);
+  const TallyOut<2, 2> out{{todo_vit2, todo_fwd}, {&ctr->todo_vit2, &ctr->todo_fwd}, {&ctr->res_vit, &ctr->res_fwd}};
   const int ntodo = ctr->todo_lb;
-  for (int job = blockIdx.x * blockDim.x + threadIdx.x; job < ntodo; job += gridDim.x * blockDim.x) {
+  for (int job0 = blockIdx.x * blockDim.x; job0 < ntodo; job0 += gridDim.x * blockDim.x) {
+    if (tally_lists_full(tally)) tally_write_lists(tally, out);
+    const int job = job0 + threadIdx.x;
+    if (job >= ntodo) continue;
     const int c = todo_lb[job];
     const int L = cand.len[c];
     const float usc = cand.usc[c];
@@ -424,7 +517,7 @@
         const float seqsc = (float)((double)(usc - filtersc) / kLog2);
         const double P = d_gumbel_surv(seqsc, p.evparam[0], p.evparam[1]);
         cand.P[c] = P;
-        if (P > p.F2) { cand.stage[c] = 5; todo_vit2[atomicAdd(&ctr->todo_vit2, 1)] = c; atomicAdd(&ctr->res_vit, (unsigned long long)L); to_fwd = false; }
+        if (P > p.F2) { cand.stage[c] = 5; tally_push(tally, 0, c); tally_add(tally, 0, (unsigned long long)L); to_fwd = false; }
       } else {
         const float seqsc = (float)((double)(vfsc - filtersc) / kLog2);
         const double P = d_gumbel_surv(seqsc, p.evparam[2], p.evparam[3]);
@@ -432,24 +525,35 @@
         if (P > p.F2) to_fwd = false;
       }
     }
-    if (to_fwd) { cand.stage[c] = 3; todo_fwd[atomicAdd(&ctr->todo_fwd, 1)] = c; atomicAdd(&ctr->res_fwd, (unsigned long long)L); }
-  }
-}
-
-__global__ void post_vit2_kernel(Cand cand, Counters *__restrict__ ctr, Params p, const int32_t *__restrict__ todo_vit2, int32_t *__restrict__ todo_fwd) {
+    if (to_fwd) { cand.stage[c] = 3; tally_push(tally, 1, c); tally_add(tally, 1, (unsigned long long)L); }
+  }
+  tally_finish(tally, out);
+}
+
+__global__ __launch_bounds__(256) void post_vit2_kernel(Cand cand, Counters *__restrict__ ctr, Params p, const int32_t *__restrict__ todo_vit2, int32_t *__restrict__ todo_fwd) {
+  __shared__ BlockTally<1, 1, 512> tally;
+  tally_reset(tally);
+  const TallyOut<1, 1> out{{todo_fwd}, {&ctr->todo_fwd}, {&ctr->res_fwd}};
   const int ntodo = ctr->todo_vit2;
-  for (int job = blockIdx.x * blockDim.x + threadIdx.x; job < ntodo; job += gridDim.x * blockDim.x) {
+  for (int job0 = blockIdx.x * blockDim.x; job0 < ntodo; job0 += gridDim.x * blockDim.x) {
+    if (tally_lists_full(tally)) tally_write_lists(tally, out);
+    const int job = job0 + threadIdx.x;
+    if (job >= ntodo) continue;
     const int c = todo_vit2[job];
     const float seqsc = (float)((double)(cand.vfsc[c] - cand.filtersc[c]) / kLog2);
     const double P = d_gumbel_surv(seqsc, p.evparam[2], p.evparam[3]);
     cand.P[c] = P;
     if (P > p.F2) { cand.stage[c] = 2; continue; }
     cand.stage[c] = 3;
-    todo_fwd[atomicAdd(&ctr->todo_fwd, 1)] = c; atomicAdd(&ctr->res_fwd, (unsigned long long)cand.len[c]);
-  }
-}
-
-__global__ void final_kernel(Cand cand, Counters *__restrict__ ctr, Params p, const int32_t *__restrict__ todo_fwd) {
+    tally_push(tally, 0, c); tally_add(tally, 0, (unsigned long long)cand.len[c]);
+  }
+  tally_finish(tally, out);
+}
+
+__global__ __launch_bounds__(256) void final_kernel(Cand cand, Counters *__restrict__ ctr, Params p, const int32_t *__restrict__ todo_fwd) {
+  __shared__ BlockTally<0, 2, 1> tally;
+  tally_reset(tally);
+  const TallyOut<0, 2> out{{nullptr}, {nullptr}, {&ctr->n_past_fwd, &ctr->pos_past_fwd}};
   const int ntodo = ctr->todo_fwd;
   for (int job = blockIdx.x * blockDim.x + threadIdx.x; job < ntodo; job += gridDim.x * blockDim.x) {
     const int c = todo_fwd[job];
@@ -458,9 +562,10 @@
     cand.P[c] = P;
     if (P > (p.fs_pipe ? p.F4 : p.F3)) continue;
     cand.stage[c] = 4;
-    atomicAdd(&ctr->n_past_fwd, 1ull);
-    if (!p.fs_pipe) atomicAdd(&ctr->pos_past_fwd, (unsigned long long)cand.len[c] * 3ull);
-  }
+    tally_add(tally, 0, 1ull);
+    if (!p.fs_pipe) tally_add(tally, 1, (unsigned long long)cand.len[c] * 3ull);
+  }
+  tally_finish(tally, out);
 }
 
 __global__ void copy_count_kernel(const int *src, int64_t *dst) { *dst = *src; }
@@ -517,6 +622,16 @@
   return BATH_OK;
 }
 
+int build_compo_terms(bath_hip_ctx *ctx, bath_hip_oprofile *om) {
+  BATH_HIP_TRY(ctx, hipMalloc((void **)&om->d_compo_terms, (size_t)(20 * 256 + 20) * sizeof(float) + 64));
+  float *d_bgf = om->d_compo_terms + 20 * 256;
+  BATH_HIP_TRY(ctx, hipMemcpyAsync(d_bgf, kAminoBg, 20 * sizeof(float), hipMemcpyHostToDevice, ctx->stream));
+  hipLaunchKernelGGL(compo_terms_kernel, dim3(20), dim3(256), 0, ctx->stream, d_bgf, (int)om->base_b, om->scale_b, om->d_compo_terms);
+  BATH_HIP_TRY(ctx, hipGetLastError());
+  BATH_HIP_TRY(ctx, hipStreamSynchronize(ctx->stream));
+  return BATH_OK;
+}
+
 static int wave_grid_blocks(bath_hip_ctx *ctx) { return ctx->prop.multiProcessorCount * 8; }
 
 struct PipelineWork {
@@ -560,6 +675,13 @@
   return (size_t)(p - base);
 }
 
+}
+
+extern "C" int bath_selftest_compo_terms(int base_b, float scale_b, float *terms) {
+  if (!terms || !(scale_b > 0.f)) return BATH_EINVAL;
+  for (int x = 0; x < 20; x++)
+    for (int sc = 0; sc < 256; sc++) terms[x * 256 + sc] = bath::compo_term(kAminoBg[x], base_b, sc, scale_b);
+  return BATH_OK;
 }
 
 extern "C" void bath_pipeline_params_default(bath_pipeline_params *p, int fs_pipe) {
@@ -781,10 +903,9 @@
     hipLaunchKernelGGL(post_vit_kernel, dim3(dec_blocks), dim3(256), 0, ctx->stream, W.cand, W.cand_cap, W.ctr, P, W.todo_msv , W.todo_fwd);
     if (P.do_bias) {
       DevBuf &b_compo = ctx->scratch[36];
-      BATH_HIP_TRY(ctx, b_compo.reserve((size_t)20 * 256 * 4 + (size_t)W.cand_cap * 20 * 4 + 256));
-      float *d_terms = b_compo.as<float>(), *d_compo = d_terms + 20 * 256;
-      hipLaunchKernelGGL(compo_terms_kernel, dim3(20), dim3(256), 0, ctx->stream, d_bgf, (int)om->base_b, om->scale_b, d_terms);
-      hipLaunchKernelGGL(local_compo_kernel, dim3(16384), dim3(64), 0, ctx->stream, W.cand, W.ctr, M, d_ssvsc, d_terms, W.todo_msv, d_compo);
+      BATH_HIP_TRY(ctx, b_compo.reserve((size_t)W.cand_cap * 20 * 4 + 256));
+      float *d_compo = b_compo.as<float>();
+      hipLaunchKernelGGL(local_compo_kernel, dim3(16384), dim3(64), 0, ctx->stream, W.cand, W.ctr, M, d_ssvsc, om->d_compo_terms, W.todo_msv, d_compo);
       hipLaunchKernelGGL(post_vit_local_kernel, dim3(std::max(1, dec_blocks)), dim3(64), 0, ctx->stream, W.cand, W.ctr, P, W.pool, M, d_bgf, d_compo,
                          om->lt.d_p1, om->lt.d_lt1, om->lt.d_lt2, W.todo_msv, W.todo_vit2, W.todo_fwd);
     }
diff --git a/bath_amd/csrc/bath_profile.hip b/bath_amd/csrc/bath_profile.hip
--- a/bath_amd/csrc/bath_profile.hip
+++ b/bath_amd/csrc/bath_profile.hip
@@ -270,11 +270,13 @@
   return BATH_OK;
 }
 
+extern "C" int bath_selftest_compute_units(const bath_hip_ctx *ctx) { return ctx ? ctx->prop.multiProcessorCount : 0; }
+
 
 extern "C" void bath_hip_oprofile_destroy(bath_hip_oprofile *om) {
   if (!om) return;
   for (void *p : {(void *)om->d_emit, (void *)om->d_ssv, (void *)om->d_msv, (void *)om->d_rb, (void *)om->d_rw, (void *)om->d_tw, (void *)om->d_rf, (void *)om->d_tf,
-                  (void *)om->d_bias_eo, (void *)om->d_vit_rw, (void *)om->d_vit_tw2, (void *)om->d_vit_rank, (void *)om->lt.d_tjb, (void *)om->lt.d_xwmove, (void *)om->lt.d_pmove,
+                  (void *)om->d_bias_eo, (void *)om->d_compo_terms, (void *)om->d_vit_rw, (void *)om->d_vit_tw2, (void *)om->d_vit_rank, (void *)om->lt.d_tjb, (void *)om->lt.d_xwmove, (void *)om->lt.d_pmove,
                   (void *)om->lt.d_nullsc, (void *)om->lt.d_lt1, (void *)om->lt.d_lt2, (void *)om->lt.d_p1, (void *)om->d_cons, (void *)om->d_msc, (void *)om->d_tsc, (void *)om->d_rfb, (void *)om->d_tfb})
     if (p) (void)hipFree(p);
   for (void *p : om->retired) (void)hipFree(p);
@@ -461,7 +463,8 @@
     BATH_HIP_TRY(ctx, upload(&om->d_bias_eo, &eo[0][0], (size_t)kKp * 2, ctx->stream));
   }
   BATH_HIP_TRY(ctx, hipStreamSynchronize(ctx->stream));
-  int st = om->ensure_len_tables(4096);
+  int st = bath::build_compo_terms(ctx, om);
+  if (st == BATH_OK) st = om->ensure_len_tables(4096);
   if (st != BATH_OK) { bath_hip_oprofile_destroy(om); return st; }
   *ret = om;
   return BATH_OK;
diff --git a/bath_amd/csrc/bath_viterbi.hip b/bath_amd/csrc/bath_viterbi.hip
--- a/bath_amd/csrc/bath_viterbi.hip
+++ b/bath_amd/csrc/bath_viterbi.hip
@@ -201,16 +201,23 @@
   __syncthreads();
   for (int i = threadIdx.x; i < kLenBins; i += blockDim.x) if (s_cnt[i]) atomicAdd(&hist[i], s_cnt[i]);
 }
-__global__ void len_scan_kernel(int *__restrict__ hist ) {
-  __shared__ int tmp[kLenBins];
-  for (int i = threadIdx.x; i < kLenBins; i += blockDim.x) tmp[i] = hist[i];
-  __syncthreads();
-  if (threadIdx.x == 0) {
-    int run = 0;
-    for (int b = kLenBins - 1; b >= 0; b--) { const int cnt = tmp[b]; tmp[b] = run; run += cnt; }
-  }
-  __syncthreads();
-  for (int i = threadIdx.x; i < kLenBins; i += blockDim.x) hist[i] = tmp[i];
+__global__ __launch_bounds__(256) void len_scan_kernel(int *__restrict__ hist ) {
+  constexpr int kPer = kLenBins / 256;
+  __shared__ int s_wsum[4];
+  const int tid = threadIdx.x, lane = tid & 63, wv = tid >> 6;
+  int c[kPer], sum = 0;
+#pragma unroll
+  for (int k = 0; k < kPer; k++) { c[k] = hist[kLenBins - 1 - (kPer * tid + k)]; sum += c[k]; }
+  int x = sum;
+#pragma unroll
+  for (int d = 1; d < 64; d <<= 1) { const int y = __shfl_up(x, d, 64); if (lane >= d) x += y; }
+  if (lane == 63) s_wsum[wv] = x;
+  __syncthreads();
+  int run = x - sum;
+#pragma unroll
+  for (int u = 0; u < 4; u++) run += u < wv ? s_wsum[u] : 0;
+#pragma unroll
+  for (int k = 0; k < kPer; k++) { hist[kLenBins - 1 - (kPer * tid + k)] = run; run += c[k]; }
 }
 __global__ __launch_bounds__(256) void len_scatter_kernel(const int32_t *__restrict__ todo, const int *__restrict__ ntodo_dev, const int32_t *__restrict__ len,
                                                           int *__restrict__ cursor, int32_t *__restrict__ sorted) {
@@ -240,6 +247,28 @@
   hipLaunchKernelGGL(len_scatter_kernel, dim3(256), dim3(256), 0, ctx->stream, d_todo, d_ntodo, d_len, d_bins, d_sorted);
   BATH_HIP_TRY(ctx, hipGetLastError());
   return BATH_OK;
+}
+
+extern "C" int bath_selftest_len_sort(bath_hip_ctx *ctx, int n, const int32_t *lens, int T, int32_t *sorted, int32_t *n_longer) {
+  if (!ctx || n < 0 || (n > 0 && (!lens || !sorted)) || !n_longer) return BATH_EINVAL;
+  BATH_HIP_TRY(ctx, hipSetDevice(ctx->device));
+  const size_t m = (size_t)std::max(n, 1);
+  int32_t *d = nullptr;
+  BATH_HIP_TRY(ctx, hipMalloc((void **)&d, (3 * m + kLenBins + 1) * sizeof(int32_t)));
+  int32_t *d_len = d, *d_todo = d + m, *d_sorted = d + 2 * m, *d_bins = d + 3 * m, *d_n = d_bins + kLenBins;
+  std::vector<int32_t> todo(m);
+  for (size_t i = 0; i < m; i++) todo[i] = (int32_t)i;
+  hipError_t e = hipSuccess;
+  if (n > 0) e = hipMemcpy(d_len, lens, (size_t)n * sizeof(int32_t), hipMemcpyHostToDevice);
+  if (e == hipSuccess) e = hipMemcpy(d_todo, todo.data(), m * sizeof(int32_t), hipMemcpyHostToDevice);
+  if (e == hipSuccess) e = hipMemcpy(d_n, &n, sizeof(int32_t), hipMemcpyHostToDevice);
+  int st = e == hipSuccess ? launch_len_sort(ctx, d_todo, d_n, d_len, d_bins, d_sorted) : BATH_EFAIL;
+  if (st == BATH_OK) e = hipStreamSynchronize(ctx->stream);
+  if (st == BATH_OK && e == hipSuccess && n > 0) e = hipMemcpy(sorted, d_sorted, (size_t)n * sizeof(int32_t), hipMemcpyDeviceToHost);
+  if (st == BATH_OK && e == hipSuccess) e = hipMemcpy(n_longer, len_sort_count_longer(d_bins, T), sizeof(int32_t), hipMemcpyDeviceToHost);
+  (void)hipFree(d);
+  if (st == BATH_OK && e != hipSuccess) { ctx->set_error(std::string("bath_selftest_len_sort: ") + hipGetErrorString(e)); st = BATH_EFAIL; }
+  return st;
 }
 
 int launch_vit_lane(bath_hip_ctx *ctx, const bath_hip_oprofile *om, SeqView v, const int32_t *d_todo, int64_t ntodo, const int *ntodo_dev,
diff --git a/include/bath_hip.h b/include/bath_hip.h
--- a/include/bath_hip.h
+++ b/include/bath_hip.h
@@ -470,7 +470,10 @@
 int bath_selftest_std_ens_walk(int M, const float *tf, float pmove, float tEL, float tEM, int Lr, const float *fwd, const float *fx, uint32_t rng_state,
                                int32_t *status, int32_t *seg, int max_seg, int32_t *n_seg);
 int bath_selftest_rng_jump(uint32_t seed, uint64_t n, uint32_t *state);
-int bath_selftest_ens_explog(int n, const float *x, float *e, float *l);
+int bath_selftest_compo_terms(int base_b, float scale_b, float *terms );
+int bath_selftest_len_sort(bath_hip_ctx *ctx, int n, const int32_t *lens, int T, int32_t *sorted, int32_t *n_longer);
+int bath_selftest_compute_units(const bath_hip_ctx *ctx);
+int bath_selftest_ens_explog(int n,const float *x, float *e, float *l);
 
 #ifdef __cplusplus
 }
```

Measured after the change: 210.5 billion (median of 6 runs). +4.7%, better.
